# anindex/motion_planning_baselines

Measured on AMD Instinct MI355X. Metric: stomp_trajectory_update_iters_per_sec, higher is better.
Workload: dtype f32

## Files before the change

include/mpb.h:

```cpp
#ifndef MPB_H
#define MPB_H

#include <stddef.h>
#include <stdint.h>

#include "mpb_geom_layout.h"
#include "mpb_rrt_layout.h"
#include "mpb_self_layout.h"
#include "mpb_sdf_layout.h"

#ifdef __cplusplus
extern "C" {
#endif

#define MPB_OK 0
#define MPB_E_INVALID 1
#define MPB_E_UNSUPPORTED 2
#define MPB_E_HIP 3

#define MPB_MAX_H 256

#define MPB_ABI_VERSION 7
#define MPB_VERSION_TUNING_BUILD 0x40000000
int mpb_version(void);
const char *mpb_last_error(void);

int mpb_geom_check(const float *geom_host, int n_words);
int mpb_geom_flags(const float *geom_host, int n_words, int *flags);

int mpb_cost_collision_eval(const float *trajs, const float *geom, float *out, float *per_waypoint,
                            int B, int H, int d, int h_begin, float k_sigma, float weight, void *stream);
int mpb_cost_collision_grad(const float *trajs, const float *geom, int geom_flags, float *out, float *grad,
                            int B, int H, int d, int h_begin, float k_sigma, float weight, void *stream);

#define MPB_TERM_GP 1u
#define MPB_TERM_START 2u
#define MPB_TERM_GOAL 4u
#define MPB_TERM_SMOOTH 8u
#define MPB_TERM_JLIM 16u
#define MPB_TERM_VEL_FD 32u
#define MPB_TERM_ALL 63u
int mpb_cost_terms_eval(const float *trajs, float *out, double *jl_total, const float *start_state,
                        const float *goal_states, const float *q_min, const float *q_max,
                        int B, int H, int d, int n_dof, int trajs_per_goal, uint32_t flags, float dt,
                        float k_gp, float k_start, float k_goal, float k_smooth, float k_jlim, float jl_eps,
                        int accumulate, int broadcast_jlim, void *stream);
int mpb_cost_terms_grad(float *trajs, const float *grad_in, float *grad_out, const float *R,
                        const float *start_state, const float *goal_states, const float *q_min, const float *q_max,
                        int B, int H, int d, int n_dof, int trajs_per_goal, uint32_t flags, float dt,
                        float k_gp, float k_start, float k_goal, float k_smooth, float k_jlim, float jl_eps,
                        float jl_scale, float prior_bw, float lr, float grad_clip, int apply, void *stream);

int mpb_traj_resample(const float *paths, const int *lengths, float *out, int N, int Lmax, int H, int D, float dt,
                      void *stream);
int mpb_traj_interpolate(const float *trajs, float *out, int B, int H, int d, int n_interp, void *stream);
int mpb_gp_factor_error(const float *x, float *out, int B, int H, int D, float dt, void *stream);
int mpb_traj_finite_difference(const float *pos, float *out, int B, int H, int D, float dt, void *stream);

int mpb_fk_collision_points(const float *q, const float *geom, float *pts, int B, int H, int d, void *stream);
int mpb_fk_collision_points_vjp(const float *q, const float *geom, const float *grad_pts, float *grad_q,
                                int B, int H, int d, void *stream);
int mpb_field_cost_points(const float *pts, const float *geom, float *cost, int B, int H, void *stream);
int mpb_field_cost_points_vjp(const float *pts, const float *geom, const float *grad_cost, float *grad_pts,
                              int B, int H, void *stream);

int mpb_stomp_step(float *means, const float *eps, float *samples, float *costs, float *weights,
                   const float *L, const float *Sigma, const float *geom, int geom_flags,
                   int P, int S, int H, int d, int D,
                   float k_sigma, float weight, float lr, float temperature,
                   int n_iters, uint64_t seed, uint32_t iter0, uint32_t particle_offset, void *stream);
int mpb_stomp_step_profile(float *means, float *samples, float *costs, float *weights,
                           const float *L, const float *Sigma, const float *geom, int geom_flags,
                           int P, int S, int H, int d, int D,
                           float k_sigma, float weight, float lr, float temperature,
                           int n_iters, uint64_t seed, uint32_t iter0, uint32_t particle_offset, void *stream,
                           float *sample_kernel_ms, float *update_kernel_ms);
#define MPB_STOMP_WS_HEADER_BYTES 1280
#define MPB_STOMP_PATH_TWO_KERNEL 0
#define MPB_STOMP_PATH_PERSISTENT_EXCHANGE 1
#define MPB_STOMP_PATH_PERSISTENT 2
size_t mpb_stomp_workspace_bytes(int P, int S, int H, int d);
int mpb_stomp_workspace_init(float *workspace, size_t workspace_bytes, void *stream);
int mpb_stomp_run_path(int geom_flags, size_t workspace_bytes, int P, int S, int H, int d);
int mpb_stomp_run(float *means, const float *eps, float *samples, float *costs, float *weights,
                  const float *L, const float *Sigma, const float *geom, int geom_flags,
                  float *workspace, size_t workspace_bytes,
                  int P, int S, int H, int d, int D,
                  float k_sigma, float weight, float lr, float temperature,
                  int n_iters, uint64_t seed, uint32_t iter0, uint32_t particle_offset, void *stream);
int mpb_stomp_run_checked(float *means, const float *eps, float *samples, float *costs, float *weights,
                          const float *L, const float *Sigma, const float *geom, int geom_flags,
                          float *workspace, size_t workspace_bytes,
                          int P, int S, int H, int d, int D,
                          float k_sigma, float weight, float lr, float temperature,
                          int n_iters, uint64_t seed, uint32_t iter0, uint32_t particle_offset,
                          uint32_t *status, uint32_t *tag_out, float *means_copy, void *stream);
int mpb_stomp_run_status(const float *workspace, void *stream, int *timed_out);
int mpb_stomp_run_timed(float *means, const float *eps, float *samples, float *costs, float *weights,
                        const float *L, const float *Sigma, const float *geom, int geom_flags,
                        float *workspace, size_t workspace_bytes,
                        int P, int S, int H, int d, int D,
                        float k_sigma, float weight, float lr, float temperature,
                        int n_iters, uint64_t seed, uint32_t iter0, uint32_t particle_offset,
                        uint32_t *status, uint32_t *tag_out, float *means_copy, void *stream, float *kernel_ms);
typedef struct mpb_stomp_plan_s mpb_stomp_plan;
int mpb_stomp_plan_create(mpb_stomp_plan **plan, float *means, float *samples, float *costs, float *weights,
                          const float *L, const float *Sigma, const float *geom, int geom_flags,
                          float *workspace, size_t workspace_bytes, int P, int S, int H, int d, int D,
                          float k_sigma, float weight, float lr, float temperature, uint64_t seed, uint32_t particle_offset,
                          uint32_t *status);
int mpb_stomp_plan_launch(mpb_stomp_plan *plan, int n_iters, uint32_t iter0, float *means_copy, void *stream, uint32_t *tag_out);
int mpb_stomp_plan_destroy(mpb_stomp_plan *plan);

int mpb_stomp_sample(const float *means, const float *eps, float *samples, const float *L,
                     const float *geom, int geom_flags, float *costs,
                     int P, int S, int H, int d, float k_sigma, float weight,
                     uint64_t seed, uint32_t iter, uint32_t particle_offset, void *stream);
int mpb_stomp_update(float *means, const float *samples, const float *costs, float *weights,
                     const float *Sigma, int P, int S, int H, int d, float lr, float temperature,
                     void *stream);

int mpb_chomp_step(float *means, const float *R, const float *geom, int geom_flags, float *costs_out,
                   int B_local, int B_global, int H, int d, int D,
                   float k_sigma, float weight, float w_prior, float lr, float grad_clip,
                   int n_iters, void *stream);

size_t mpb_gpmp2_workspace_bytes(int B, int H, int D);
int mpb_gpmp2_linearize(const float *x, const float *geom, int geom_flags, void *workspace, int B, int H, int D,
                        int n_interp, void *stream);
int mpb_gpmp2_diag(void *workspace, double *diag_sum_out, int B, int H, int D, int n_fields, float dt,
                   float sigma_start, float sigma_gp, float sigma_goal, float sigma_coll, void *stream);
int mpb_gpmp2_solve(float *x, const float *start, const float *goal, const double *diag_mean, void *workspace,
                    float *costs_out, int B, int H, int D, int n_fields, float dt,
                    float sigma_start, float sigma_gp, float sigma_goal, float sigma_coll,
                    float delta, int trust_region, float step_size, void *stream);
int mpb_gpmp2_step(float *x, const float *start, const float *goal, const float *geom, int geom_flags, void *workspace,
                   float *costs_out, int B, int H, int D, float dt,
                   float sigma_start, float sigma_gp, float sigma_goal, float sigma_coll,
                   float delta, int trust_region, float step_size, int n_iters, int n_interp, int n_fields,
                   void *stream);

int mpb_mppi_step(float *mean, const float *eps, const float *scale_tril, const float *cov_inv,
                  const float *state0, const float *goal, const float *ctrl_min, const float *ctrl_max,
                  const float *discount, const float *c_weights, const float *geom, int geom_flags,
                  float *controls, float *states, float *costs, float *weights,
                  float *best_cost, float *best_states,
                  int NP, int S, int T, int c, int control_type, float dt,
                  float k_sigma, float weight, float temp, float step_size,
                  int n_iters, uint64_t seed, uint32_t iter0, void *stream);
#define MPB_MPPI_NOISE_GLOBAL 0
#define MPB_MPPI_NOISE_LDS 1
#define MPB_MPPI_NOISE_MATRIX 2
int mpb_mppi_plan(int geom_flags, int has_geom, int NP, int S, int T, int c, int has_eps, int n_cu, int *plan);
int mpb_point_dynamics(const float *x, const float *u, const float *ctrl_min, const float *ctrl_max, const float *dyn_std,
                       const float *noise, float *x_next, size_t n, int dim, float dt, void *stream);
int mpb_point_traj_cost(const float *X, const float *U, const float *goal, const float *discount, float w_pos, float w_vel,
                        float w_ctrl, float w_pos_T, float energy, float *costs, int T, int B, int state_dim, int ctrl_dim,
                        void *stream);


int mpb_stoch_gpmp_costs(const float *samples, const float *means, const float *start, const float *goal,
                         const float *geom, float *costs, int P, int S, int H, int D, float dt,
                         float sigma_start, float sigma_gp, float sigma_goal, float sigma_coll,
                         float sigma_start_sample, float sigma_gp_sample, float sigma_goal_sample,
                         float temperature, void *stream);

int mpb_stoch_gpmp_step(float *means, double *means64, float *samples, float *costs, float *weights,
                        const double *Udiag, const double *Uoff, const double *scale_tril,
                        const float *start, const float *goal, const float *geom,
                        int P, int S, int H, int D, float dt,
                        float sigma_start, float sigma_gp, float sigma_goal, float sigma_coll,
                        float sigma_start_sample, float sigma_gp_sample, float sigma_goal_sample,
                        float temperature, float step_size, int n_iters, uint64_t seed, void *stream);

int mpb_gp_prior_sample(float *out, const double *means, const double *eps, const double *Udiag,
                        const double *Uoff, int G, int n, int H, int D, uint64_t seed, void *stream);
int mpb_gp_prior_sample_dense(float *out, const double *means, const double *eps, const double *scale_tril,
                              int G, int n, int H, int D, uint64_t seed, void *stream);
int mpb_mvn_sample_dense(float *out, const double *means, const double *eps, const double *tril_t,
                         int G, int n, int M, uint64_t seed, void *stream);

int mpb_mt19937_normals(float *out, int n, int n_calls, const uint32_t *state_in, int pos, int final_idx, uint32_t *state_out,
                        const uint16_t *jump_idx, const int *jump_cnt, int jump_stride, const int *segs, int n_segs,
                        uint32_t *work, void *stream);

int mpb_collision_check(const float *q, const float *geom, int geom_flags, unsigned char *in_collision, float *gap,
                        int N, int D, void *stream);

int mpb_traj_collision_stats(const float *trajs, size_t row_stride, const float *geom, int geom_flags, int n_interp,
                             int *n_in_collision, int *first_in_collision, float *max_gap, unsigned char *point_in_collision,
                             int N, int H, int D, void *stream);

int mpb_self_check(const float *self_host, int n_words);
int mpb_self_invalidate(const float *self);
int mpb_self_collision_eval(const float *trajs, const float *self, float *out, float *per_waypoint,
                            int B, int H, int d, int h_begin, float k_sigma, float weight, int accumulate, void *stream);
int mpb_self_collision_grad(const float *trajs, const float *self, float *out, float *grad,
                            int B, int H, int d, int h_begin, float k_sigma, float weight, int accumulate, void *stream);
int mpb_self_collision_check(const float *q, const float *self, unsigned char *in_collision, float *gap,
                             int N, int D, int or_into, void *stream);

int mpb_sdf_grid_check(const float *sdf_host, int n_words);
int mpb_sdf_grid_invalidate(const float *sdf);
int mpb_sdf_grid_build(const float *geom, float *sdf, void *stream);
int mpb_sdf_grid_build_occupancy(const unsigned char *occupancy, float *sdf, void *stream);
int mpb_sdf_grid_sample(const float *points, const float *sdf, float *s, float *grad, int N, void *stream);
int mpb_sdf_grid_eval(const float *trajs, const float *sdf, float *out, float *per_waypoint,
                      int B, int H, int d, int h_begin, float k_sigma, float weight, int accumulate, void *stream);
int mpb_sdf_grid_grad(const float *trajs, const float *sdf, float *out, float *grad,
                      int B, int H, int d, int h_begin, float k_sigma, float weight, int accumulate, void *stream);
int mpb_sdf_grid_collision_check(const float *q, const float *sdf, unsigned char *in_collision, float *gap,
                                 int N, int D, int or_into, void *stream);

#define MPB_IK_MAX_ITERS 1024
#define MPB_IK_MIN_DAMPING 1e-2f
int mpb_fk_ee_pose(const float *q, const float *geom, float *pose, float *jac, int N, int D, void *stream);
int mpb_ik_solve(const float *target, const float *q_seed, const float *geom, const float *q_min, const float *q_max,
                 float *q_out, float *pos_err, float *rot_err, unsigned char *converged, int *iters_used,
                 int N, int S, int D, int n_iters, float damping, float pos_tol, float rot_tol, int position_only, void *stream);

int mpb_ee_cost_eval(const float *trajs, const float *geom, const float *target, float *out, float *per_waypoint,
                     int B, int H, int d, int D, int h_begin, int h_end, int group, int stride_g, int stride_h,
                     float k_pos, float k_rot, int use_axis, float ax, float ay, float az, float weight, int accumulate, void *stream);
int mpb_ee_cost_grad(const float *trajs, const float *geom, const float *target, float *out, float *grad,
                     int B, int H, int d, int D, int h_begin, int h_end, int group, int stride_g, int stride_h,
                     float k_pos, float k_rot, int use_axis, float ax, float ay, float az, float weight, int accumulate, void *stream);

size_t mpb_rrt_connect_workspace_bytes(int B, int max_nodes, int n_pre, int D);
int mpb_rrt_connect_init(void *workspace, size_t workspace_bytes, const float *start, const float *goal,
                         const float *geom, int geom_flags, int B, int max_nodes, int n_pre, int D, void *stream);
int mpb_rrt_connect_run(void *workspace, size_t workspace_bytes, const float *geom, int geom_flags,
                        const float *pre_samples, size_t pre_stride, const int *sample_idx, float *paths,
                        int *lengths, int *status, int B, int max_nodes, int n_pre, int D, int Lmax, int iter0,
                        int n_iters, int total_iters, float step_size, float n_radius, uint64_t seed,
                        uint32_t problem_offset, void *stream);

size_t mpb_rrt_star_workspace_bytes(int B, int max_nodes, int n_pre, int D);
int mpb_rrt_star_init(void *workspace, size_t workspace_bytes, const float *start, const float *goal,
                      const float *geom, int geom_flags, int B, int max_nodes, int n_pre, int D, void *stream);
int mpb_rrt_star_run(void *workspace, size_t workspace_bytes, const float *geom, int geom_flags,
                     const float *pre_samples, size_t pre_stride, const int *sample_idx, const int *goal_draw,
                     float *paths, int *lengths, float *costs, int *status, int B, int max_nodes, int n_pre, int D,
                     int Lmax, int iter0, int n_iters, int total_iters, int max_best_cost_iters,
                     int n_iters_after_success, int informed, float step_size, float n_radius, float goal_prob,
                     float cost_eps, float eps, uint64_t seed, uint32_t problem_offset, void *stream);

#ifdef __cplusplus
}
#endif
#endif
```

include/mpb_debug.h:

```cpp
#ifndef MPB_DEBUG_H
#define MPB_DEBUG_H

#include <stddef.h>
#include <stdint.h>

#ifdef __cplusplus
extern "C" {
#endif

const char *mpb_debug_last_error(void);
int mpb_debug_occupy(int n_blocks, uint64_t usec, uint32_t *sink, void *stream);
int mpb_debug_philox(const uint32_t *ctr, const uint32_t *key, uint32_t *out, int n, int rounds, void *stream);
int mpb_debug_stomp_normals(float *out, int P, int S, int d, int n_iters, uint64_t seed, uint32_t iter0,
                            uint32_t particle_offset, void *stream);
int mpb_debug_stomp_normals_h(float *out, int P, int S, int d, int H, int n_iters, uint64_t seed, uint32_t iter0,
                              uint32_t particle_offset, void *stream);
int mpb_debug_mppi_normals(float *out, int NP, int S, int T, int c, int n_iters, uint64_t seed, uint32_t iter0, void *stream);

int mpb_debug_mt19937_uniforms(float *out, int n, int n_calls, const uint32_t *state_in, int pos, int final_idx,
                               uint32_t *state_out, const uint16_t *jump_idx, const int *jump_cnt, int jump_stride,
                               const int *segs, int n_segs, uint32_t *work, void *stream);
int mpb_debug_mt19937_normals_timed(float *out, int n, int n_calls, const uint32_t *state_in, int pos, int final_idx,
                                    uint32_t *state_out, const uint16_t *jump_idx, const int *jump_cnt, int jump_stride,
                                    const int *segs, int n_segs, uint32_t *work, void *events, void *stream);

#ifdef __cplusplus
}
#endif
#endif
```

motion_planning_baselines_amd/_lib.py:

```python
import ctypes
import os

import numpy as np

_HERE = os.path.dirname(os.path.abspath(__file__))
LIB_PATH = os.environ.get('MPB_LIB_PATH') or os.path.join(_HERE, 'csrc', 'libmpb_hip.so')

_f = ctypes.c_float
_i = ctypes.c_int
_p = ctypes.c_void_p
_u64 = ctypes.c_uint64
_u32 = ctypes.c_uint32

SIGNATURES = {
    'mpb_version': [],
    'mpb_last_error': [],
    'mpb_geom_check': [_p, _i],
    'mpb_geom_flags': [_p, _i, _p],
    'mpb_cost_collision_eval': [_p, _p, _p, _p, _i, _i, _i, _i, _f, _f, _p],
    'mpb_cost_collision_grad': [_p, _p, _i, _p, _p, _i, _i, _i, _i, _f, _f, _p],
    'mpb_cost_terms_eval': [_p] * 7 + [_i] * 5 + [_u32] + [_f] * 7 + [_i, _i, _p],
    'mpb_cost_terms_grad': [_p] * 8 + [_i] * 5 + [_u32] + [_f] * 11 + [_i, _p],
    'mpb_traj_resample': [_p, _p, _p, _i, _i, _i, _i, _f, _p],
    'mpb_gp_factor_error': [_p, _p, _i, _i, _i, _f, _p],
    'mpb_traj_interpolate': [_p, _p, _i, _i, _i, _i, _p],
    'mpb_traj_finite_difference': [_p, _p, _i, _i, _i, _f, _p],
    'mpb_fk_collision_points': [_p, _p, _p, _i, _i, _i, _p],
    'mpb_fk_collision_points_vjp': [_p, _p, _p, _p, _i, _i, _i, _p],
    'mpb_field_cost_points': [_p, _p, _p, _i, _i, _p],
    'mpb_field_cost_points_vjp': [_p, _p, _p, _p, _i, _i, _p],
    'mpb_stomp_step': [_p, _p, _p, _p, _p, _p, _p, _p, _i, _i, _i, _i, _i, _i, _f, _f, _f, _f, _i, _u64, _u32, _u32, _p],
    'mpb_stomp_workspace_bytes': [_i, _i, _i, _i],
    'mpb_stomp_run': [_p, _p, _p, _p, _p, _p, _p, _p, _i, _p, ctypes.c_size_t, _i, _i, _i, _i, _i, _f, _f, _f, _f, _i, _u64, _u32, _u32, _p],
    'mpb_stomp_run_checked': [_p, _p, _p, _p, _p, _p, _p, _p, _i, _p, ctypes.c_size_t, _i, _i, _i, _i, _i, _f, _f, _f, _f, _i, _u64, _u32, _u32, _p, _p, _p, _p],
    'mpb_stomp_run_status': [_p, _p, _p],
    'mpb_stomp_run_timed': [_p, _p, _p, _p, _p, _p, _p, _p, _i, _p, ctypes.c_size_t, _i, _i, _i, _i, _i, _f, _f, _f, _f, _i, _u64, _u32, _u32, _p, _p, _p, _p, _p],
    'mpb_stomp_workspace_init': [_p, ctypes.c_size_t, _p],
    'mpb_stomp_run_path': [_i, ctypes.c_size_t, _i, _i, _i, _i],
    'mpb_stomp_step_profile': [_p, _p, _p, _p, _p, _p, _p, _i, _i, _i, _i, _i, _i, _f, _f, _f, _f, _i, _u64, _u32, _u32, _p, _p, _p],
    'mpb_stomp_sample': [_p, _p, _p, _p, _p, _i, _p, _i, _i, _i, _i, _f, _f, _u64, _u32, _u32, _p],
    'mpb_stomp_update': [_p, _p, _p, _p, _p, _i, _i, _i, _i, _f, _f, _p],
    'mpb_chomp_step': [_p, _p, _p, _i, _p, _i, _i, _i, _i, _i, _f, _f, _f, _f, _f, _i, _p],
    'mpb_gpmp2_workspace_bytes': [_i, _i, _i],
    'mpb_gpmp2_linearize': [_p, _p, _i, _p, _i, _i, _i, _i, _p],
    'mpb_gpmp2_diag': [_p, _p, _i, _i, _i, _i, _f, _f, _f, _f, _f, _p],
    'mpb_gpmp2_solve': [_p, _p, _p, _p, _p, _p, _i, _i, _i, _i, _f, _f, _f, _f, _f, _f, _i, _f, _p],
    'mpb_gpmp2_step': [_p, _p, _p, _p, _i, _p, _p, _i, _i, _i, _f, _f, _f, _f, _f, _f, _i, _f, _i, _i, _i, _p],
    'mpb_stoch_gpmp_costs': [_p, _p, _p, _p, _p, _p, _i, _i, _i, _i] + [_f] * 9 + [_p],
    'mpb_stoch_gpmp_step': [_p] * 11 + [_i] * 4 + [_f] * 10 + [_i, _u64, _p],
    'mpb_gp_prior_sample': [_p, _p, _p, _p, _p, _i, _i, _i, _i, _u64, _p],
    'mpb_gp_prior_sample_dense': [_p, _p, _p, _p, _i, _i, _i, _i, _u64, _p],
    'mpb_mvn_sample_dense': [_p, _p, _p, _p, _i, _i, _i, _u64, _p],
    'mpb_stomp_plan_create': [_p] * 8 + [_i, _p, ctypes.c_size_t, _i, _i, _i, _i, _i, _f, _f, _f, _f, _u64, _u32, _p],
    'mpb_stomp_plan_launch': [_p, _i, _u32, _p, _p, _p],
    'mpb_stomp_plan_destroy': [_p],
    'mpb_point_dynamics': [_p, _p, _p, _p, _p, _p, _p, ctypes.c_size_t, _i, _f, _p],
    'mpb_point_traj_cost': [_p, _p, _p, _p, _f, _f, _f, _f, _f, _p, _i, _i, _i, _i, _p],
    'mpb_mppi_step': [_p] * 11 + [_i] + [_p] * 6 + [_i, _i, _i, _i, _i, _f, _f, _f, _f, _f, _i, _u64, _u32, _p],
    'mpb_mppi_plan': [_i, _i, _i, _i, _i, _i, _i, _i, _p],
    'mpb_mt19937_normals': [_p, _i, _i, _p, _i, _i, _p, _p, _p, _i, _p, _i, _p, _p],
    'mpb_collision_check': [_p, _p, _i, _p, _p, _i, _i, _p],
    'mpb_traj_collision_stats': [_p, ctypes.c_size_t, _p, _i, _i, _p, _p, _p, _p, _i, _i, _i, _p],
    'mpb_self_check': [_p, _i],
    'mpb_self_invalidate': [_p],
    'mpb_self_collision_eval': [_p, _p, _p, _p, _i, _i, _i, _i, _f, _f, _i, _p],
    'mpb_self_collision_grad': [_p, _p, _p, _p, _i, _i, _i, _i, _f, _f, _i, _p],
    'mpb_self_collision_check': [_p, _p, _p, _p, _i, _i, _i, _p],
    'mpb_sdf_grid_check': [_p, _i],
    'mpb_sdf_grid_invalidate': [_p],
    'mpb_sdf_grid_build': [_p, _p, _p],
    'mpb_sdf_grid_build_occupancy': [_p, _p, _p],
    'mpb_sdf_grid_sample': [_p, _p, _p, _p, _i, _p],
    'mpb_sdf_grid_eval': [_p, _p, _p, _p, _i, _i, _i, _i, _f, _f, _i, _p],
    'mpb_sdf_grid_grad': [_p, _p, _p, _p, _i, _i, _i, _i, _f, _f, _i, _p],
    'mpb_sdf_grid_collision_check': [_p, _p, _p, _p, _i, _i, _i, _p],
    'mpb_fk_ee_pose': [_p, _p, _p, _p, _i, _i, _p],
    'mpb_ik_solve': [_p] * 10 + [_i] * 4 + [_f] * 3 + [_i, _p],
    'mpb_ee_cost_eval': [_p] * 5 + [_i] * 9 + [_f, _f, _i] + [_f] * 4 + [_i, _p],
    'mpb_ee_cost_grad': [_p] * 5 + [_i] * 9 + [_f, _f, _i] + [_f] * 4 + [_i, _p],
    'mpb_rrt_connect_workspace_bytes': [_i, _i, _i, _i],
    'mpb_rrt_connect_init': [_p, ctypes.c_size_t, _p, _p, _p, _i, _i, _i, _i, _i, _p],
    'mpb_rrt_connect_run': [_p, ctypes.c_size_t, _p, _i, _p, ctypes.c_size_t, _p, _p, _p, _p] + [_i] * 8 + [_f, _f, _u64, _u32, _p],
    'mpb_rrt_star_workspace_bytes': [_i, _i, _i, _i],
    'mpb_rrt_star_init': [_p, ctypes.c_size_t, _p, _p, _p, _i, _i, _i, _i, _i, _p],
    'mpb_rrt_star_run': [_p, ctypes.c_size_t, _p, _i, _p, ctypes.c_size_t] + [_p] * 6 + [_i] * 11 + [_f] * 5 + [_u64, _u32, _p],
}

DEBUG_SIGNATURES = {
    'mpb_debug_last_error': [],
    'mpb_debug_occupy': [_i, _u64, _p, _p],
    'mpb_debug_philox': [_p, _p, _p, _i, _i, _p],
    'mpb_debug_stomp_normals': [_p, _i, _i, _i, _i, _u64, _u32, _u32, _p],
    'mpb_debug_stomp_normals_h': [_p, _i, _i, _i, _i, _i, _u64, _u32, _u32, _p],
    'mpb_debug_mppi_normals': [_p, _i, _i, _i, _i, _i, _u64, _u32, _p],
    'mpb_debug_mt19937_uniforms': [_p, _i, _i, _p, _i, _i, _p, _p, _p, _i, _p, _i, _p, _p],
    'mpb_debug_mt19937_normals_timed': [_p, _i, _i, _p, _i, _i, _p, _p, _p, _i, _p, _i, _p, _p, _p],
}
ABI_VERSION = 7

_lib = None
_debug_lib = None


class MPBError(RuntimeError):
    pass


def lib():
    global _lib
    if _lib is not None:
        return _lib
    if not os.path.exists(LIB_PATH):
        raise MPBError(
            f'{LIB_PATH} not found: the HIP extension is not built. Run '
            f'`python -c "import __graft_entry__ as g; g.build()"` (or motion_planning_baselines_amd/build.py). '
            f'There is no CPU fallback.')
    import torch
    h = ctypes.CDLL(LIB_PATH)
    for name, argtypes in SIGNATURES.items():
        try:
            fn = getattr(h, name)
        except AttributeError as e:
            raise MPBError(f'{LIB_PATH} does not export {name} (declared in include/mpb.h)') from e
        fn.argtypes = argtypes
        fn.restype = (ctypes.c_char_p if name == 'mpb_last_error' else
                      ctypes.c_size_t if name in ('mpb_gpmp2_workspace_bytes', 'mpb_stomp_workspace_bytes', 'mpb_rrt_connect_workspace_bytes',
                                                         'mpb_rrt_star_workspace_bytes') else ctypes.c_int)
    if (h.mpb_version() & 0xFFFF) != ABI_VERSION:
        raise MPBError(f'{LIB_PATH} reports ABI version {h.mpb_version() & 0xFFFF}, this binding is written for {ABI_VERSION} '
                       f'(include/mpb.h MPB_ABI_VERSION); rebuild with motion_planning_baselines_amd.build.build(force=True)')
    if (h.mpb_version() & 0x40000000) and not os.environ.get('MPB_LIB_PATH'):
        raise MPBError(f'{LIB_PATH} is a tuning build (compiled with wrong-result timing switches); rebuild with '
                       f'motion_planning_baselines_amd.build.build(force=True)')
    _lib = h
    return h


def debug_lib():
    global _debug_lib
    if _debug_lib is not None:
        return _debug_lib
    path = os.path.join(_HERE, 'csrc', 'libmpb_hip_debug.so')
    if not os.path.exists(path):
        raise MPBError(f'{path} not found: run motion_planning_baselines_amd.build.build()')
    lib()
    h = ctypes.CDLL(path)
    for name, argtypes in DEBUG_SIGNATURES.items():
        fn = getattr(h, name)
        fn.argtypes = argtypes
        fn.restype = ctypes.c_char_p if name == 'mpb_debug_last_error' else ctypes.c_int
    _debug_lib = h
    return h


def debug_check(code, what=''):
    if code != 0:
        msg = debug_lib().mpb_debug_last_error()
        raise MPBError(f'{what} failed with code {code}: {msg.decode() if msg else "?"}')


def check(code, what=''):
    if code != 0:
        msg = lib().mpb_last_error()
        raise MPBError(f'{what} failed with code {code}: {msg.decode() if msg else "?"}')


def geom_check(buf):
    buf = np.ascontiguousarray(buf, dtype=np.float32)
    check(lib().mpb_geom_check(buf.ctypes.data_as(ctypes.c_void_p), int(buf.size)), 'mpb_geom_check')


def self_check(buf):
    buf = np.ascontiguousarray(buf, dtype=np.float32)
    check(lib().mpb_self_check(buf.ctypes.data_as(ctypes.c_void_p), int(buf.size)), 'mpb_self_check')


def sdf_grid_check(buf, n_words=None):
    buf = np.ascontiguousarray(buf, dtype=np.float32)
    check(lib().mpb_sdf_grid_check(buf.ctypes.data_as(ctypes.c_void_p), int(buf.size if n_words is None else n_words)), 'mpb_sdf_grid_check')


def geom_flags(buf):
    buf = np.ascontiguousarray(buf, dtype=np.float32)
    out = ctypes.c_int(0)
    check(lib().mpb_geom_flags(buf.ctypes.data_as(ctypes.c_void_p), int(buf.size), ctypes.cast(ctypes.pointer(out), ctypes.c_void_p)),
          'mpb_geom_flags')
    return int(out.value)
```

motion_planning_baselines_amd/build.py:

```python
import os
import subprocess
import sys
import tempfile

HERE = os.path.dirname(os.path.abspath(__file__))
CSRC = os.path.join(HERE, 'csrc')
SOURCES = ['mpb_lib.hip', 'mpb_stomp_api.hip', 'mpb_kernels.hip', 'mpb_stomp_fused.hip', 'mpb_stomp_fused_hx.hip', 'mpb_chomp.hip', 'mpb_gpmp2.hip', 'mpb_gpmp2_lr.hip', 'mpb_mppi.hip', 'mpb_prior.hip', 'mpb_stoch_gpmp.hip', 'mpb_costs.hip', 'mpb_points.hip', 'mpb_mt19937.hip', 'mpb_rrt_connect.hip', 'mpb_rrt_star.hip', 'mpb_traj_validate.hip', 'mpb_self_collision.hip', 'mpb_sdf_grid.hip', 'mpb_ik.hip', 'mpb_ee_cost.hip']
DEBUG_SOURCES = ['mpb_debug.hip']
MAX_ILP = ['-mllvm', '-amdgpu-sched-strategy=max-ilp']
EXTRA = {'mpb_chomp.hip': MAX_ILP, 'mpb_gpmp2.hip': MAX_ILP, 'mpb_gpmp2_lr.hip': MAX_ILP, 'mpb_mppi.hip': MAX_ILP,
         'mpb_kernels.hip': ['-mllvm', '-amdgpu-sched-strategy=iterative-ilp'],
         'mpb_stomp_fused.hip': ['-mllvm', '-amdgpu-sched-strategy=iterative-ilp'],
         'mpb_stomp_fused_hx.hip': ['-mllvm', '-amdgpu-sched-strategy=iterative-ilp']}
OUT = os.path.join(CSRC, 'libmpb_hip.so')
DEBUG_OUT = os.path.join(CSRC, 'libmpb_hip_debug.so')
FLAGS = ['--offload-arch=gfx950', '-O3', '-std=c++17', '-fPIC', '-Wall', '-Wno-unused-function',
         '-ffinite-math-only', '-fno-signed-zeros', '-fno-slp-vectorize']
RESOURCES = os.path.join(CSRC, 'kernel_resources.json')
REMARKS = ['-Rpass-analysis=kernel-resource-usage']


def parse_resource_remarks(text):
    import re
    out, cur = {}, None
    keys = {'VGPRs': 'vgprs', 'AGPRs': 'agprs', 'ScratchSize [bytes/lane]': 'scratch', 'Occupancy [waves/SIMD]': 'occupancy',
            'SGPRs Spill': 'sgpr_spill', 'VGPRs Spill': 'vgpr_spill', 'LDS Size [bytes/block]': 'lds', 'TotalSGPRs': 'sgprs'}
    for line in text.splitlines():
        m = re.search(r'remark: Function Name: (\S+)', line)
        if m:
            cur = out.setdefault(m.group(1), {})
            continue
        m = re.search(r'remark:\s+([A-Za-z \[\]/]+): (\d+) \[-Rpass-analysis', line)
        if m and cur is not None and m.group(1).strip() in keys:
            cur[keys[m.group(1).strip()]] = int(m.group(2))
    return out


_LAYOUT = '../../include/mpb_geom_layout.h'
PMC_SOURCES = {
    'stomp': ['mpb_stomp_fused.hip', 'mpb_stomp_fused.h', 'mpb_stomp_noise.h', 'mpb_geom.h', _LAYOUT, 'mpb_common.h', 'mpb_model_panda.h'],
    'stomp_c5': ['mpb_stomp_fused.hip', 'mpb_stomp_fused.h', 'mpb_stomp_noise.h', 'mpb_geom.h', _LAYOUT, 'mpb_common.h', 'mpb_model_panda.h'],
    'stomp_h128': ['mpb_stomp_fused_hx.hip', 'mpb_stomp_fused.h', 'mpb_stomp_noise.h', 'mpb_geom.h', _LAYOUT, 'mpb_common.h', 'mpb_model_panda.h'],
    'kernelA': ['mpb_kernels.hip', 'mpb_stomp_noise.h', 'mpb_geom.h', _LAYOUT, 'mpb_common.h', 'mpb_model_panda.h'],
    'solve': ['mpb_gpmp2.hip', 'mpb_gpmp2_lr.hip', 'mpb_gpmp2.h', 'mpb_geom.h', _LAYOUT, 'mpb_common.h'],
    'chomp': ['mpb_chomp.hip', 'mpb_geom.h', _LAYOUT, 'mpb_common.h', 'mpb_model_panda.h'],
    'mppi': ['mpb_mppi.hip', 'mpb_geom.h', _LAYOUT, 'mpb_common.h'],
}


def sources_sha1(files):
    import hashlib
    h = hashlib.sha1()
    for f in files:
        h.update(f.encode())
        with open(os.path.join(CSRC, f), 'rb') as fh:
            h.update(fh.read())
    return h.hexdigest()


def pmc_fingerprint(kind):
    files = PMC_SOURCES[kind]
    return {'sources': files, 'sources_sha1': sources_sha1(files), 'flags': FLAGS + EXTRA.get(files[0], [])}


def _stale():
    if not os.path.exists(OUT) or not os.path.exists(DEBUG_OUT) or not os.path.exists(RESOURCES):
        return True
    t = min(os.path.getmtime(OUT), os.path.getmtime(DEBUG_OUT))
    deps = [os.path.join(CSRC, f) for f in os.listdir(CSRC) if f.endswith(('.hip', '.h'))]
    deps += [os.path.join(os.path.dirname(HERE), 'include', h) for h in ('mpb.h', 'mpb_geom_layout.h', 'mpb_rrt_layout.h', 'mpb_self_layout.h', 'mpb_sdf_layout.h', 'mpb_debug.h')]
    return any(os.path.getmtime(d) > t for d in deps)


def build_variant(out, extra_flags, verbose=False):
    if os.path.abspath(out) == os.path.abspath(OUT):
        raise ValueError('build_variant must not overwrite the product library')
    extra_flags = list(extra_flags)
    if any('_T_' in f for f in extra_flags) and '-DMPB_TUNING_BUILD' not in extra_flags:
        extra_flags.append('-DMPB_TUNING_BUILD')
    hipcc = os.environ.get('HIPCC', '/opt/rocm/bin/hipcc')
    objs = []
    tmp = out + '.objs'
    os.makedirs(tmp, exist_ok=True)
    for src in SOURCES:
        obj = os.path.join(tmp, src.replace('.hip', '.o'))
        cmd = [hipcc, *FLAGS, *EXTRA.get(src, []), *extra_flags, '-c', os.path.join(CSRC, src), '-o', obj]
        if verbose:
            print(' '.join(cmd), flush=True)
        subprocess.check_call(cmd)
        objs.append(obj)
    subprocess.check_call([hipcc, '--offload-arch=gfx950', '-shared', '-fPIC', *objs, '-o', out])
    return out


def build(force=False, verbose=True):
    from . import model_gen
    stale = force or _stale() or bool(model_gen.stale_headers())
    if not stale:
        return OUT
    for path in model_gen.write_headers():
        if verbose:
            print('regenerated', path, flush=True)
    if any('MPB_TUNING_BUILD' in f or '_T_' in f for f in FLAGS + [x for v in EXTRA.values() for x in v]):
        raise RuntimeError('the product build must not carry tuning switches')
    hipcc = os.environ.get('HIPCC', '/opt/rocm/bin/hipcc')
    objs = []
    procs = []
    for src in SOURCES + DEBUG_SOURCES:
        obj = os.path.join(CSRC, src.replace('.hip', '.o'))
        objs.append(obj)
        cmd = [hipcc, *FLAGS, *EXTRA.get(src, []), *REMARKS, '-c', os.path.join(CSRC, src), '-o', obj]
        if verbose:
            print(' '.join(cmd), flush=True)
        log = tempfile.TemporaryFile(mode='w+')
        procs.append((cmd, subprocess.Popen(cmd, stderr=log, text=True), log))
    resources = {}
    for cmd, p, log in procs:
        p.wait()
        log.seek(0)
        err = log.read()
        log.close()
        rest = '\n'.join(l for l in err.splitlines() if 'kernel-resource-usage' not in l and not l.lstrip().startswith(('|', '^')) and l.strip()
                         and not __import__('re').match(r'^\s*\d+ \|', l))
        if p.returncode != 0:
            raise RuntimeError('hipcc failed: ' + ' '.join(cmd) + '\n' + err[-4000:])
        if verbose and rest:
            print(rest, file=sys.stderr, flush=True)
        resources.update(parse_resource_remarks(err))
    import json
    with open(RESOURCES, 'w') as fh:
        json.dump(resources, fh, indent=0, sort_keys=True)
    n = len(SOURCES)
    for out, o in ((OUT, objs[:n]), (DEBUG_OUT, objs[n:])):
        cmd = [hipcc, '--offload-arch=gfx950', '-shared', '-fPIC', *o, '-o', out]
        if verbose:
            print(' '.join(cmd), flush=True)
        subprocess.check_call(cmd)
    return OUT


if __name__ == '__main__':
    build(force='--force' in sys.argv)
```

motion_planning_baselines_amd/csrc/mpb_debug.hip:

```cpp
#include <hip/hip_runtime.h>

#include "mpb_common.h"
#include "mpb_host.h"
#include "mpb_stomp_noise.h"
#include "mpb_mt19937.h"
#include "../../include/mpb_debug.h"

static thread_local char g_debug_err[512] = "";
char* mpb_err_buf() { return g_debug_err; }
extern "C" const char* mpb_debug_last_error(void) { return g_debug_err; }

__global__ void debug_philox_kernel(const uint32_t* __restrict__ ctr, const uint32_t* __restrict__ key, uint32_t* __restrict__ out,
                                    int n, int rounds) {
    const int i = blockIdx.x * blockDim.x + threadIdx.x;
    if (i >= n) return;
    const uint4 c = make_uint4(ctr[4 * i], ctr[4 * i + 1], ctr[4 * i + 2], ctr[4 * i + 3]);
    const uint2 k = make_uint2(key[2 * i], key[2 * i + 1]);
    const uint4 r = (rounds == 7) ? philox4x32<7>(c, k) : philox4x32<10>(c, k);
    out[4 * i] = r.x; out[4 * i + 1] = r.y; out[4 * i + 2] = r.z; out[4 * i + 3] = r.w;
}

extern "C" int mpb_debug_philox(const uint32_t* ctr, const uint32_t* key, uint32_t* out, int n, int rounds, void* stream) {
    if (!ctr || !key || !out || n < 1) return mpb_fail(MPB_E_INVALID, "mpb_debug_philox: bad argument");
    if (rounds != 7 && rounds != 10) return mpb_fail(MPB_E_INVALID, "mpb_debug_philox: rounds must be 7 or 10");
    hipLaunchKernelGGL(debug_philox_kernel, dim3((n + 255) / 256), dim3(256), 0, (hipStream_t)stream, ctr, key, out, n, rounds);
    return mpb_check_launch("mpb_debug_philox");
}

#ifdef MPB_DEBUG_RAW_NORMALS
#define DBGQ(x) (x)
#else
#define DBGQ(x) stomp_eps_quantise(x)
#endif
__global__ void debug_stomp_normals_kernel(float* __restrict__ out, int P, int S, int d, int HC, int n_iters, uint32_t seed_lo,
                                           uint32_t seed_hi, uint32_t iter0, uint32_t particle_offset) {
    const size_t n = (size_t)n_iters * P * S * d * HC * 4;
    const size_t i = (size_t)blockIdx.x * blockDim.x + threadIdx.x;
    if (i >= n) return;
    const uint32_t g = i & 3;
    size_t r = i >> 2;
    const uint32_t kc = r % HC; r /= HC;
    const uint32_t j = r % d; r /= d;
    const uint32_t s = r % S; r /= S;
    const uint32_t p = r % P; r /= P;
    const uint32_t it = (uint32_t)r;
    float lo[8], hi[8];
    uint32_t carry[2];
    stomp_normals_lo<STOMP_PRIO_NONE>(particle_offset + p, s, j, g, kc << 4, iter0 + it, seed_lo, seed_hi, lo, carry);
    stomp_normals_hi<STOMP_PRIO_NONE>(particle_offset + p, s, j, g, kc << 4, iter0 + it, seed_lo, seed_hi, carry, hi);
    float* o = out + (((((size_t)it * P + p) * S + s) * d + j) * HC + kc) * 64;
#pragma unroll
    for (int u = 0; u < 8; ++u) {
        o[stomp_eps_column((int)g, u >> 2, u & 3)] = DBGQ(lo[u]);
        o[stomp_eps_column((int)g, 2 + (u >> 2), u & 3)] = DBGQ(hi[u]);
    }
}

extern "C" int mpb_debug_stomp_normals_h(float* out, int P, int S, int d, int H, int n_iters, uint64_t seed, uint32_t iter0,
                                         uint32_t particle_offset, void* stream) {
    if (!out || P < 1 || S < 1 || d < 1 || d > 16 || n_iters < 1 || H < 1 || H > 256)
        return mpb_fail(MPB_E_INVALID, "mpb_debug_stomp_normals: bad argument");
    const int HC = (H + 63) / 64;
    const size_t n = (size_t)n_iters * P * S * d * HC * 4;
    if (n > 0x7FFFFFFFull * 256ull) return mpb_fail(MPB_E_INVALID, "mpb_debug_stomp_normals: too many draws for one launch");
    hipLaunchKernelGGL(debug_stomp_normals_kernel, dim3((unsigned)((n + 255) / 256)), dim3(256), 0, (hipStream_t)stream, out, P, S,
                       d, HC, n_iters, (uint32_t)seed, (uint32_t)(seed >> 32), iter0, particle_offset);
    return mpb_check_launch("mpb_debug_stomp_normals");
}
extern "C" int mpb_debug_stomp_normals(float* out, int P, int S, int d, int n_iters, uint64_t seed, uint32_t iter0,
                                       uint32_t particle_offset, void* stream) {
    return mpb_debug_stomp_normals_h(out, P, S, d, 64, n_iters, seed, iter0, particle_offset, stream);
}

__global__ void debug_mppi_normals_kernel(float* __restrict__ out, int NP, int S, int T, int c, int n_iters, uint32_t seed_lo,
                                          uint32_t seed_hi, uint32_t iter0) {
    const int G4 = (T + 3) >> 2;
    const size_t n = (size_t)n_iters * NP * c * S * G4;
    const size_t idx = (size_t)blockIdx.x * blockDim.x + threadIdx.x;
    if (idx >= n) return;
    size_t r = idx;
    const uint32_t g4 = r % G4; r /= G4;
    const uint32_t s = r % S; r /= S;
    const uint32_t i = r % c; r /= c;
    const uint32_t prob = r % NP; r /= NP;
    const uint32_t it = (uint32_t)r;
    const uint4 w = philox4x32<7>(make_uint4(prob, s, g4 | (i << 16), iter0 + it), make_uint2(seed_lo, seed_hi));
    float nrm[4];
    box_muller_m23(w.x, w.y, nrm[0], nrm[1]);
    box_muller_m23(w.z, w.w, nrm[2], nrm[3]);
    float* o = out + ((((size_t)it * NP + prob) * c + i) * S + s) * T;
#pragma unroll
    for (int q = 0; q < 4; ++q)
        if ((int)(4 * g4 + q) < T) o[4 * g4 + q] = nrm[q];
}

extern "C" int mpb_debug_mppi_normals(float* out, int NP, int S, int T, int c, int n_iters, uint64_t seed, uint32_t iter0, void* stream) {
    if (!out || NP < 1 || S < 1 || T < 1 || c < 1 || n_iters < 1) return mpb_fail(MPB_E_INVALID, "mpb_debug_mppi_normals: bad argument");
    const size_t n = (size_t)n_iters * NP * c * S * ((T + 3) >> 2);
    if (n > 0x7FFFFFFFull * 256ull) return mpb_fail(MPB_E_INVALID, "mpb_debug_mppi_normals: too many draws for one launch");
    hipLaunchKernelGGL(debug_mppi_normals_kernel, dim3((unsigned)((n + 255) / 256)), dim3(256), 0, (hipStream_t)stream, out, NP, S, T, c,
                       n_iters, (uint32_t)seed, (uint32_t)(seed >> 32), iter0);
    return mpb_check_launch("mpb_debug_mppi_normals");
}

__global__ __launch_bounds__(64) void occupy_kernel(unsigned long long ticks, unsigned* sink) {
    __shared__ unsigned pad[150 * 256];
    pad[threadIdx.x] = threadIdx.x;
    const unsigned long long t0 = __builtin_amdgcn_s_memrealtime();
    while (__builtin_amdgcn_s_memrealtime() - t0 < ticks) __builtin_amdgcn_s_sleep(32);
    if (pad[(threadIdx.x + 1) & 63] == 0xFFFFFFFFu) sink[0] = 1u;
}

extern "C" int mpb_debug_occupy(int n_blocks, uint64_t usec, uint32_t* sink, void* stream) {
    if (n_blocks < 1 || !sink) return mpb_fail(MPB_E_INVALID, "mpb_debug_occupy: bad argument");
    hipLaunchKernelGGL(occupy_kernel, dim3(n_blocks), dim3(64), 0, (hipStream_t)stream, usec * 100ull, sink);
    return mpb_check_launch("mpb_debug_occupy");
}

extern "C" int mpb_debug_mt19937_uniforms(float* out, int n, int n_calls, const uint32_t* state_in, int pos, int final_idx,
                                          uint32_t* state_out, const uint16_t* jump_idx, const int* jump_cnt, int jump_stride,
                                          const int* segs, int n_segs, uint32_t* work, void* stream) {
    if (!out || !state_in || !state_out || !jump_idx || !jump_cnt || !segs || !work)
        return mpb_fail(MPB_E_INVALID, "mpb_debug_mt19937_uniforms: null pointer");
    if (const char* why = mt19937_bad_args(n, n_calls, pos, final_idx, jump_stride, n_segs)) return mpb_fail(MPB_E_INVALID, why);
    if (((uintptr_t)jump_idx & 15u) || ((uintptr_t)work & 15u)) return mpb_fail(MPB_E_INVALID, "mpb_debug_mt19937_uniforms: misaligned");
    if (mt19937_launch<true>(out, n, state_in, pos, final_idx, state_out, jump_idx, jump_cnt, jump_stride, segs, n_segs, work, nullptr,
                             (hipStream_t)stream) != hipSuccess)
        return mpb_fail(MPB_E_HIP, "mpb_debug_mt19937_uniforms: HIP launch failed");
    return MPB_OK;
}

extern "C" int mpb_debug_mt19937_normals_timed(float* out, int n, int n_calls, const uint32_t* state_in, int pos, int final_idx,
                                               uint32_t* state_out, const uint16_t* jump_idx, const int* jump_cnt, int jump_stride,
                                               const int* segs, int n_segs, uint32_t* work, void* events, void* stream) {
    if (!out || !state_in || !state_out || !jump_idx || !jump_cnt || !segs || !work || !events)
        return mpb_fail(MPB_E_INVALID, "mpb_debug_mt19937_normals_timed: null pointer");
    if (const char* why = mt19937_bad_args(n, n_calls, pos, final_idx, jump_stride, n_segs)) return mpb_fail(MPB_E_INVALID, why);
    if (((uintptr_t)jump_idx & 15u) || ((uintptr_t)work & 15u)) return mpb_fail(MPB_E_INVALID, "mpb_debug_mt19937_normals_timed: misaligned");
    if (mt19937_launch<false>(out, n, state_in, pos, final_idx, state_out, jump_idx, jump_cnt, jump_stride, segs, n_segs, work,
                              (hipEvent_t*)events, (hipStream_t)stream) != hipSuccess)
        return mpb_fail(MPB_E_HIP, "mpb_debug_mt19937_normals_timed: HIP launch failed");
    return MPB_OK;
}
```

motion_planning_baselines_amd/csrc/mpb_stomp_api.hip:

```cpp
#include <hip/hip_runtime.h>
#include <stdlib.h>

#include <atomic>
#include <chrono>

#include "mpb_stomp_host.h"
#include "mpb_stomp_fused.h"

struct StompCheck {
    const char* who;
    int n_iters;
    bool two_kernel;
    bool profile;
    const char* aligned;
    const void *extra0 = nullptr, *extra1 = nullptr;
};

static int stomp_check(const StompCall& c, const StompCheck& k) {
    if (!c.means || !c.samples || !c.costs || !c.weights || !c.L || !c.Sigma || !c.geom) return mpb_failf(MPB_E_INVALID, "%s: null pointer", k.who);
    bool bad = c.P < (k.profile ? 1 : 0) || c.S < 1 || !(c.d == c.D || c.d == 2 * c.D) || k.n_iters < (k.profile ? 1 : 0) || (k.profile && k.n_iters > 1024);
    if (k.two_kernel) bad = bad || c.H < 3 || c.H > MPB_MAX_H || c.D < 1 || c.D > MPB_MAX_DOF;
    if (bad) return mpb_failf(MPB_E_INVALID, "%s: bad shape", k.who);
    if (!(c.temperature > 0.f)) return mpb_failf(MPB_E_INVALID, "%s: temperature must be > 0", k.who);
    if (k.aligned && (mpb_misaligned16(c.means, c.eps, c.samples, c.L, c.Sigma, c.geom) || mpb_misaligned16(k.extra0, k.extra1)))
        return mpb_failf(MPB_E_INVALID, "%s: %s must be 16-byte aligned", k.who, k.aligned);
    return k.two_kernel ? mpb_update_envelope(c.S, c.H, c.d, k.who) : MPB_OK;
}

extern "C" int mpb_stomp_sample(const float* means, const float* eps, float* samples, const float* L,
                                const float* geom, int geom_flags, float* costs, int P, int S, int H, int d, float k_sigma,
                                float weight, uint64_t seed, uint32_t iter, uint32_t particle_offset, void* stream) {
    if (P == 0) return MPB_OK;
    if (!means || !samples || !L) return mpb_failf(MPB_E_INVALID, "%s: null pointer", __func__);
    if ((geom == nullptr) != (costs == nullptr)) return mpb_failf(MPB_E_INVALID, "%s: geom and costs must be given together", __func__);
    if (P < 0 || S < 1 || H < 3 || H > MPB_MAX_H || d < 1 || d > MPB_MAX_D) return mpb_failf(MPB_E_INVALID, "%s: bad shape", __func__);
    if (mpb_misaligned16(means, eps, samples, L, geom)) return mpb_failf(MPB_E_INVALID, "%s: means / eps / samples / L / geom must be 16-byte aligned", __func__);
    StompCall c = {};
    c.means = const_cast<float*>(means); c.eps = eps; c.samples = samples; c.costs = costs; c.L = L; c.geom = geom;
    c.P = P; c.S = S; c.H = H; c.d = d; c.seed = seed; c.particle_offset = particle_offset;
    if (geom) { c.geom_flags = geom_flags; c.k_sigma = k_sigma; c.weight = weight; }
    mpb_stomp_launch_sample(c, eps, iter, (hipStream_t)stream, nullptr);
    return mpb_check_launch(__func__);
}

extern "C" int mpb_stomp_update(float* means, const float* samples, const float* costs, float* weights,
                                const float* Sigma, int P, int S, int H, int d, float lr, float temperature,
                                void* stream) {
    if (P == 0) return MPB_OK;
    if (!means || !samples || !costs || !weights) return mpb_failf(MPB_E_INVALID, "%s: null pointer", __func__);
    if (P < 0) return mpb_failf(MPB_E_INVALID, "%s: bad shape", __func__);
    if (const int rc = mpb_update_envelope(S, H, d, __func__)) return rc;
    if (!(temperature > 0.f)) return mpb_failf(MPB_E_INVALID, "%s: temperature must be > 0", __func__);
    if (mpb_misaligned16(means, samples, Sigma)) return mpb_failf(MPB_E_INVALID, "%s: means / samples / Sigma must be 16-byte aligned", __func__);
    StompCall c = {};
    c.means = means; c.samples = const_cast<float*>(samples); c.costs = const_cast<float*>(costs); c.weights = weights; c.Sigma = Sigma;
    c.P = P; c.S = S; c.H = H; c.d = d; c.lr = lr; c.temperature = temperature;
    mpb_stomp_launch_update(c, (hipStream_t)stream, nullptr);
    return mpb_check_launch(__func__);
}

static int stomp_step(const StompCall& c, const StompLaunch& l) {
    if (c.P == 0) return MPB_OK;
    if (const int rc = stomp_check(c, {"mpb_stomp_step", l.n_iters, true, false, "means / eps / samples / L / Sigma / geom"})) return rc;
    const size_t eps_stride = (size_t)c.S * c.d * c.P * c.H;
    constexpr int MPB_CHUNK = 128;
    hipEvent_t ev[2] = {nullptr, nullptr};
    hipStreamCaptureStatus cap = hipStreamCaptureStatusNone;
    const bool throttle = l.n_iters > 2 * MPB_CHUNK &&
                          hipStreamIsCapturing(l.stream, &cap) == hipSuccess && cap == hipStreamCaptureStatusNone;
    for (int it = 0; it < l.n_iters; ++it) {
        if (throttle && it % MPB_CHUNK == 0) {
            const int k = (it / MPB_CHUNK) & 1;
            if (ev[k]) (void)hipEventSynchronize(ev[k]);
            else (void)hipEventCreateWithFlags(&ev[k], hipEventDisableTiming);
        }
        mpb_stomp_launch_sample(c, c.eps ? c.eps + (size_t)it * eps_stride : nullptr, l.iter0 + (uint32_t)it, l.stream, nullptr);
        mpb_stomp_launch_update(c, l.stream, nullptr);
        if (throttle && it % MPB_CHUNK == MPB_CHUNK - 1) (void)hipEventRecord(ev[(it / MPB_CHUNK) & 1], l.stream);
    }
    for (int k = 0; k < 2; ++k)
        if (ev[k]) (void)hipEventDestroy(ev[k]);
    return mpb_check_launch("mpb_stomp_step");
}

extern "C" int mpb_stomp_step(float* means, const float* eps, float* samples, float* costs, float* weights,
                              const float* L, const float* Sigma, const float* geom, int geom_flags, int P, int S, int H, int d, int D,
                              float k_sigma, float weight, float lr, float temperature, int n_iters, uint64_t seed,
                              uint32_t iter0, uint32_t particle_offset, void* stream) {
    const StompCall c = {means, eps, samples, costs, weights, L, Sigma, geom, geom_flags, P, S, H, d, D,
                         k_sigma, weight, lr, temperature, seed, particle_offset};
    return stomp_step(c, {n_iters, iter0, nullptr, (hipStream_t)stream, nullptr});
}

extern "C" int mpb_stomp_step_profile(float* means, float* samples, float* costs, float* weights, const float* L,
                                      const float* Sigma, const float* geom, int geom_flags, int P, int S, int H, int d, int D,
                                      float k_sigma, float weight, float lr, float temperature, int n_iters, uint64_t seed,
                                      uint32_t iter0, uint32_t particle_offset, void* stream, float* sample_kernel_ms,
                                      float* update_kernel_ms) {
    const StompCall c = {means, nullptr, samples, costs, weights, L, Sigma, geom, geom_flags, P, S, H, d, D,
                         k_sigma, weight, lr, temperature, seed, particle_offset};
    if (!sample_kernel_ms || !update_kernel_ms) return mpb_failf(MPB_E_INVALID, "%s: null pointer", __func__);
    if (const int rc = stomp_check(c, {__func__, n_iters, true, true, nullptr})) return rc;
    hipStream_t st = (hipStream_t)stream;
    StompEvents* ev = new StompEvents[2 * (size_t)n_iters]();
    int rc = MPB_OK;
    for (int i = 0; i < 2 * n_iters && rc == MPB_OK; ++i)
        if (hipEventCreate(&ev[i].start) != hipSuccess || hipEventCreate(&ev[i].stop) != hipSuccess)
            rc = mpb_failf(MPB_E_HIP, "%s: hipEventCreate failed", __func__);
    if (rc == MPB_OK) {
        for (int it = 0; it < n_iters; ++it) {
            mpb_stomp_launch_sample(c, nullptr, iter0 + (uint32_t)it, st, &ev[2 * it]);
            mpb_stomp_launch_update(c, st, &ev[2 * it + 1]);
        }
        rc = mpb_check_launch(__func__);
    }
    if (rc == MPB_OK && hipStreamSynchronize(st) != hipSuccess) rc = mpb_failf(MPB_E_HIP, "%s: synchronize failed", __func__);
    double sa = 0.0, sb = 0.0;
    for (int it = 0; it < n_iters && rc == MPB_OK; ++it) {
        float ma = 0.f, mb = 0.f;
        if (hipEventElapsedTime(&ma, ev[2 * it].start, ev[2 * it].stop) != hipSuccess ||
            hipEventElapsedTime(&mb, ev[2 * it + 1].start, ev[2 * it + 1].stop) != hipSuccess)
            rc = mpb_failf(MPB_E_HIP, "%s: hipEventElapsedTime failed", __func__);
        sa += ma;
        sb += mb;
    }
    for (int i = 0; i < 2 * n_iters; ++i) {
        if (ev[i].start) (void)hipEventDestroy(ev[i].start);
        if (ev[i].stop) (void)hipEventDestroy(ev[i].stop);
    }
    delete[] ev;
    if (rc != MPB_OK) return rc;
    *sample_kernel_ms = (float)(sa / n_iters);
    *update_kernel_ms = (float)(sb / n_iters);
    return MPB_OK;
}

struct FusedPlan {
    int path;
    int nc;
    bool hx;
    int nb;
    size_t ws_bytes;
};
static FusedPlan fused_plan(int geom_flags, int P, int S, int H, int d) {
    FusedPlan f = {MPB_STOMP_PATH_TWO_KERNEL, 1, false, 1, 0};
    if (P < 1 || S < 1) return f;
    const int n_cu = mpb_device_cu_count();
    const char* hx_env = getenv("MPB_STOMP_HX");
    const int force_hx = hx_env ? atoi(hx_env) : 0;
    const bool v1 = !force_hx && H == 64 && S <= FUSED_WAVES * FUSED_MAX_CHUNKS && mpb_flags_all_grids(geom_flags) &&
                    (d == 2 || d == 3 || d == 4 || d == 6 || d == 7 || d == 14);
    if (!v1) {
        if (!mpb_fused_hx_plan(geom_flags, n_cu, P, S, H, d, &f.nc, &f.nb, &f.ws_bytes)) return f;
        f.hx = true;
        f.path = f.nc > 1 ? MPB_STOMP_PATH_PERSISTENT_EXCHANGE : MPB_STOMP_PATH_PERSISTENT;
        return f;
    }
    f.nc = (S + FUSED_WAVES - 1) / FUSED_WAVES;
    static const int force_nb = [] { const char* e = getenv("MPB_STOMP_BATCHES"); return e ? atoi(e) : 0; }();
    const long r1 = (2L * P + n_cu - 1) / n_cu, r2 = ((long)P + n_cu - 1) / n_cu;
    const bool two_batches = f.nc == 2 && force_nb != 1 && (force_nb == 2 || 188 * r2 < 100 * r1);
    f.nb = two_batches ? 2 : 1;
    const bool exchange = f.nc > 1 && !two_batches;
    f.path = exchange ? MPB_STOMP_PATH_PERSISTENT_EXCHANGE : MPB_STOMP_PATH_PERSISTENT;
    f.ws_bytes = (exchange ? mpb_fused_ws_floats(P, f.nc) : FUSED_HDR_WORDS) * sizeof(float);
    return f;
}

extern "C" size_t mpb_stomp_workspace_bytes(int P, int S, int H, int d) {
    if (P < 1 || S < 1) return 0;
    const FusedPlan f = fused_plan(MPB_GEOM_FLAG_ALL_GRIDS, P, S, H, d);
    const FusedPlan fl = fused_plan(MPB_GEOM_FLAG_ALL_LISTS, P, S, H, d);
    size_t b = f.path == MPB_STOMP_PATH_TWO_KERNEL ? FUSED_HDR_WORDS * sizeof(float) : f.ws_bytes;
    if (fl.path != MPB_STOMP_PATH_TWO_KERNEL && fl.ws_bytes > b) b = fl.ws_bytes;
    return b;
}

extern "C" int mpb_stomp_workspace_init(float* workspace, size_t workspace_bytes, void* stream) {
    if (!workspace || workspace_bytes < FUSED_HDR_WORDS * sizeof(float)) return mpb_fail(MPB_E_INVALID, "mpb_stomp_workspace_init: workspace too small");
    if (hipMemsetAsync(workspace, 0, FUSED_HDR_WORDS * sizeof(float), (hipStream_t)stream) != hipSuccess) return mpb_fail(MPB_E_HIP, "mpb_stomp_workspace_init: memset failed");
    return MPB_OK;
}

extern "C" int mpb_stomp_run_path(int geom_flags, size_t workspace_bytes, int P, int S, int H, int d) {
    const FusedPlan f = fused_plan(geom_flags, P, S, H, d);
    return (f.path != MPB_STOMP_PATH_TWO_KERNEL && workspace_bytes >= f.ws_bytes) ? f.path : MPB_STOMP_PATH_TWO_KERNEL;
}

static int stomp_run(const StompCall& c, float* workspace, size_t workspace_bytes, uint32_t* status, const StompLaunch& l, uint32_t* tag_out) {
    if (tag_out) *tag_out = 0u;
    if (c.P == 0) return MPB_OK;
    const FusedPlan f = fused_plan(c.geom_flags, c.P, c.S, c.H, c.d);
    if (l.n_iters == 0 || !workspace || f.path == MPB_STOMP_PATH_TWO_KERNEL || workspace_bytes < f.ws_bytes) {
        const int rc = l.n_iters == 0 ? MPB_OK : stomp_step(c, l);
        if (rc == MPB_OK && l.means_copy && c.means &&
            hipMemcpyAsync(l.means_copy, c.means, sizeof(float) * (size_t)c.P * c.H * c.d, hipMemcpyDeviceToDevice, l.stream) != hipSuccess)
            return mpb_fail(MPB_E_HIP, "mpb_stomp_run: copy of the means failed");
        return rc;
    }
    if (const int rc = stomp_check(c, {"mpb_stomp_run", l.n_iters, false, false, "means / eps / samples / L / Sigma / geom / workspace / means_copy",
                                       workspace, l.means_copy}))
        return rc;
    StompFusedGrid g = {workspace, f.nc, f.nb, 0u, 0ull, nullptr};
    if (status) {
        static thread_local uint32_t* seen_host = nullptr;
        static thread_local unsigned* seen_dev = nullptr;
        if (status != seen_host) {
            unsigned* dp = nullptr;
            if (hipHostGetDevicePointer(reinterpret_cast<void**>(&dp), status, 0) != hipSuccess) {
                (void)hipGetLastError();
                return mpb_fail(MPB_E_INVALID, "mpb_stomp_run: status is not pinned, device-mapped host memory");
            }
            seen_host = status;
            seen_dev = dp;
        }
        g.status_dev = seen_dev;
    }
    static std::atomic<uint32_t> epoch{(uint32_t)std::chrono::steady_clock::now().time_since_epoch().count()};
    g.tag0 = (epoch.fetch_add(1u) + 1u) * 0x9E3779B9u;
    if (g.tag0 == 0u) g.tag0 = 0x9E3779B9u;
    if (tag_out) *tag_out = g.tag0;
    g.timeout = FUSED_TIMEOUT_TICKS + FUSED_TIMEOUT_PER_ITER * (unsigned long long)l.n_iters;
    if (const char* e = getenv("MPB_STOMP_TIMEOUT_US")) { const long long us = atoll(e); if (us > 0) g.timeout = 100ull * (unsigned long long)us; }
    return f.hx ? mpb_fused_hx_launch(c, l, g) : mpb_fused_launch(c, l, g);
}

extern "C" int mpb_stomp_run_checked(float* means, const float* eps, float* samples, float* costs, float* weights,
                                     const float* L, const float* Sigma, const float* geom, int geom_flags, float* workspace,
                                     size_t workspace_bytes, int P, int S, int H, int d, int D, float k_sigma, float weight, float lr,
                                     float temperature, int n_iters, uint64_t seed, uint32_t iter0, uint32_t particle_offset,
                                     uint32_t* status, uint32_t* tag_out, float* means_copy, void* stream) {
    const StompCall c = {means, eps, samples, costs, weights, L, Sigma, geom, geom_flags, P, S, H, d, D,
                         k_sigma, weight, lr, temperature, seed, particle_offset};
    return stomp_run(c, workspace, workspace_bytes, status, {n_iters, iter0, means_copy, (hipStream_t)stream, nullptr}, tag_out);
}

extern "C" int mpb_stomp_run(float* means, const float* eps, float* samples, float* costs, float* weights,
                             const float* L, const float* Sigma, const float* geom, int geom_flags, float* workspace,
                             size_t workspace_bytes, int P, int S, int H, int d, int D, float k_sigma, float weight, float lr,
                             float temperature, int n_iters, uint64_t seed, uint32_t iter0, uint32_t particle_offset,
                             void* stream) {
    const StompCall c = {means, eps, samples, costs, weights, L, Sigma, geom, geom_flags, P, S, H, d, D,
                         k_sigma, weight, lr, temperature, seed, particle_offset};
    return stomp_run(c, workspace, workspace_bytes, nullptr, {n_iters, iter0, nullptr, (hipStream_t)stream, nullptr}, nullptr);
}

struct mpb_stomp_plan_s {
    StompCall call;
    float* workspace;
    size_t workspace_bytes;
    uint32_t* status;
};

extern "C" int mpb_stomp_plan_create(mpb_stomp_plan** plan, float* means, float* samples, float* costs, float* weights, const float* L,
                                     const float* Sigma, const float* geom, int geom_flags, float* workspace, size_t workspace_bytes,
                                     int P, int S, int H, int d, int D, float k_sigma, float weight, float lr, float temperature,
                                     uint64_t seed, uint32_t particle_offset, uint32_t* status) {
    if (!plan) return mpb_failf(MPB_E_INVALID, "%s: null pointer", __func__);
    *plan = nullptr;
    const StompCall c = {means, nullptr, samples, costs, weights, L, Sigma, geom, geom_flags, P, S, H, d, D,
                         k_sigma, weight, lr, temperature, seed, particle_offset};
    if (const int rc = stomp_check(c, {__func__, 0, false, false, "means / samples / L / Sigma / geom / workspace", workspace})) return rc;
    mpb_stomp_plan_s* q = static_cast<mpb_stomp_plan_s*>(malloc(sizeof(mpb_stomp_plan_s)));
    if (!q) return mpb_failf(MPB_E_HIP, "%s: out of host memory", __func__);
    *q = mpb_stomp_plan_s{c, workspace, workspace_bytes, status};
    *plan = q;
    return MPB_OK;
}

extern "C" int mpb_stomp_plan_launch(mpb_stomp_plan* plan, int n_iters, uint32_t iter0, float* means_copy, void* stream, uint32_t* tag_out) {
    if (!plan) return mpb_fail(MPB_E_INVALID, "mpb_stomp_plan_launch: null plan");
    return stomp_run(plan->call, plan->workspace, plan->workspace_bytes, plan->status, {n_iters, iter0, means_copy, (hipStream_t)stream, nullptr}, tag_out);
}

extern "C" int mpb_stomp_plan_destroy(mpb_stomp_plan* plan) {
    free(plan);
    return MPB_OK;
}

extern "C" int mpb_stomp_run_timed(float* means, const float* eps, float* samples, float* costs, float* weights,
                                   const float* L, const float* Sigma, const float* geom, int geom_flags, float* workspace,
                                   size_t workspace_bytes, int P, int S, int H, int d, int D, float k_sigma, float weight, float lr,
                                   float temperature, int n_iters, uint64_t seed, uint32_t iter0, uint32_t particle_offset,
                                   uint32_t* status, uint32_t* tag_out, float* means_copy, void* stream, float* kernel_ms) {
    if (!kernel_ms) return mpb_failf(MPB_E_INVALID, "%s: null pointer", __func__);
    *kernel_ms = 0.f;
    StompEvents ev = {nullptr, nullptr};
    if (hipEventCreate(&ev.start) != hipSuccess || hipEventCreate(&ev.stop) != hipSuccess) {
        if (ev.start) (void)hipEventDestroy(ev.start);
        return mpb_failf(MPB_E_HIP, "%s: hipEventCreate failed", __func__);
    }
    const StompCall c = {means, eps, samples, costs, weights, L, Sigma, geom, geom_flags, P, S, H, d, D,
                         k_sigma, weight, lr, temperature, seed, particle_offset};
    uint32_t tag = 0;
    int rc = stomp_run(c, workspace, workspace_bytes, status, {n_iters, iter0, means_copy, (hipStream_t)stream, &ev}, &tag);
    if (tag_out) *tag_out = tag;
    if (rc == MPB_OK && hipStreamSynchronize((hipStream_t)stream) != hipSuccess) rc = mpb_failf(MPB_E_HIP, "%s: synchronize failed", __func__);
    if (rc == MPB_OK && tag != 0u && hipEventElapsedTime(kernel_ms, ev.start, ev.stop) != hipSuccess) {
        (void)hipGetLastError();
        rc = mpb_failf(MPB_E_HIP, "%s: hipEventElapsedTime failed", __func__);
    }
    (void)hipEventDestroy(ev.start);
    (void)hipEventDestroy(ev.stop);
    return rc;
}

extern "C" int mpb_stomp_run_status(const float* workspace, void* stream, int* timed_out) {
    if (!workspace || !timed_out) return mpb_failf(MPB_E_INVALID, "%s: null pointer", __func__);
    uint32_t w[4] = {0u};
    if (hipMemcpyAsync(w, workspace, sizeof(w), hipMemcpyDeviceToHost, (hipStream_t)stream) != hipSuccess ||
        hipStreamSynchronize((hipStream_t)stream) != hipSuccess)
        return mpb_failf(MPB_E_HIP, "%s: copy failed", __func__);
    *timed_out = (w[FUSED_HDR_ERR] == w[FUSED_HDR_TAG] && w[FUSED_HDR_TAG] != 0u) ? (w[FUSED_HDR_WHY] == 2u ? 2 : 1) : 0;
    return MPB_OK;
}
```

motion_planning_baselines_amd/csrc/mpb_stomp_fused.hip:

```cpp
#include <hip/hip_runtime.h>

#include <type_traits>

#include "mpb_common.h"
#include "mpb_stomp_host.h"
#include "mpb_geom.h"
#include "mpb_stomp_noise.h"
#include "mpb_stomp_fused.h"

static inline size_t fused_ws_floats(int P, int nc) { return FUSED_HDR_WORDS + 2 * 2 * (size_t)P * nc * FUSED_XCHG; }

#ifdef MPB_STAMPS
__device__ unsigned long long g_fstamps[256 * FUSED_WAVES * 12];
#define FSTAMP(k)                                                                                   \
    do {                                                                                            \
        if (it == 2 && blockIdx.x < 256) {                                                          \
            __builtin_amdgcn_sched_barrier(0);                                                      \
            unsigned long long t_;                                                                  \
            asm volatile("s_memtime %0\n\ts_waitcnt lgkmcnt(0)" : "=s"(t_)::"memory");           \
            __builtin_amdgcn_sched_barrier(0);                                                      \
            if ((k) == 0) {           \
                unsigned hw_;                                                                       \
                asm volatile("s_getreg_b32 %0, hwreg(HW_REG_HW_ID, 4, 2)" : "=s"(hw_));             \
                t_ = (t_ & 0x00FFFFFFFFFFFFFFull) | ((unsigned long long)hw_ << 56);                \
            }                                                                                       \
            if ((threadIdx.x & 63) == 0) g_fstamps[(blockIdx.x * FUSED_WAVES + (threadIdx.x >> 6)) * 12 + (k)] = t_; \
        }                                                                                           \
    } while (0)
extern "C" int mpb_debug_read_fstamps(unsigned long long* dst, int n) {
    return hipMemcpyFromSymbol(dst, HIP_SYMBOL(g_fstamps), sizeof(unsigned long long) * n) == hipSuccess ? 0 : 3;
}
__device__ unsigned long long g_lstamps[1024 * 8];
#define LSTAMP(k)                                                                                   \
    do {                                                                                            \
        if (blockIdx.x < 1024 && threadIdx.x == 0) g_lstamps[blockIdx.x * 8 + (k)] = __builtin_amdgcn_s_memrealtime(); \
    } while (0)
extern "C" int mpb_debug_read_lstamps(unsigned long long* dst, int n) {
    return hipMemcpyFromSymbol(dst, HIP_SYMBOL(g_lstamps), sizeof(unsigned long long) * n) == hipSuccess ? 0 : 3;
}
#else
#define FSTAMP(k)
#define LSTAMP(k)
#endif

#ifdef FUSED_T_PRE_STATS
__device__ unsigned g_pre_miss[FUSED_WAVES];
extern "C" int mpb_debug_read_pre_miss(unsigned* dst) {
    if (hipMemcpyFromSymbol(dst, HIP_SYMBOL(g_pre_miss), sizeof(unsigned) * FUSED_WAVES) != hipSuccess) return 3;
    unsigned z[FUSED_WAVES] = {};
    return hipMemcpyToSymbol(HIP_SYMBOL(g_pre_miss), z, sizeof(z)) == hipSuccess ? 0 : 3;
}
#endif
template <int DCH, bool PRE>
struct FusedSmem {
    float4 otab[MPB_GRID_MAX_SPH + 1];
    unsigned gridw[MPB_GRID_MAX_CELLS];
    unsigned Limg[STOMP_LIMG_WORDS];
    float sig_l[64 * FUSED_LD];
    float mean_l[64 * DCH];
    float delta[DCH * FUSED_LD];
    float cst[FUSED_WAVES];
    int s_abort;
    unsigned s_ticket;
    unsigned pad_[2];
    float tiles[FUSED_WAVES * 64 * NT_STRIDE];
    __attribute__((aligned(16))) granule_t pre[PRE ? FUSED_WAVES * 128 : 2];
    __attribute__((aligned(16))) granule_t premz[PRE ? FUSED_WAVES * 4 : 2];
};

template <int DCH, int MODEL, int NB, bool INJ, bool CHAIN>
__global__ __launch_bounds__(FUSED_THREADS, 4) void stomp_fused_kernel(
    float* __restrict__ means, const float* __restrict__ eps, float* __restrict__ samples, float* __restrict__ costs,
    float* __restrict__ weights, const float* __restrict__ Lmat, const float* __restrict__ Sigma,
    const float* __restrict__ geom, float* __restrict__ ws, int P, int S, int nc, float k_sigma, float weight, float lr,
    float temperature, int n_iters, uint32_t seed_lo, uint32_t seed_hi, uint32_t iter0, uint32_t particle_offset,
    uint32_t tag0, unsigned long long timeout_ticks, unsigned* __restrict__ status_host, float* __restrict__ means_copy) {
    constexpr int H = 64;
    constexpr int N = H * DCH;
    static_assert(N <= FUSED_THREADS && N + 2 <= FUSED_XCHG, "one thread per trajectory element");
    if (!INJ) eps = nullptr;
#ifdef FUSED_NO_PRE
    constexpr bool PRE = false;
#else
    constexpr bool PRE = NB == 1 && 2 * DCH > 16 && MODEL != 0 && !INJ;
#endif
    __shared__ __attribute__((aligned(16))) FusedSmem<DCH, PRE> sm;
    float4 (&otab)[MPB_GRID_MAX_SPH + 1] = sm.otab;
    unsigned (&gridw)[MPB_GRID_MAX_CELLS] = sm.gridw;
    unsigned (&Limg)[STOMP_LIMG_WORDS] = sm.Limg;
    float (&sig_l)[64 * FUSED_LD] = sm.sig_l;
    float (&mean_l)[64 * DCH] = sm.mean_l;
    float (&delta)[DCH * FUSED_LD] = sm.delta;
    float (&cst)[FUSED_WAVES] = sm.cst;
    float (&tiles)[FUSED_WAVES * 64 * NT_STRIDE] = sm.tiles;
    int& s_abort = sm.s_abort;
    unsigned& s_ticket = sm.s_ticket;

    const int tid = threadIdx.x, lane = tid & 63, wave = __builtin_amdgcn_readfirstlane(tid >> 6);
    LSTAMP(0);
    unsigned* wsu = reinterpret_cast<unsigned*>(ws);
    const bool exchange = NB == 1 && nc > 1;
    if (tid == 0) {
        s_abort = 0;
        fused_stamp_begin(wsu, status_host);
        unsigned u = blockIdx.x;
        if (exchange) {
            int why;
            u = fused_draw_unit(wsu, P, nc, tag0, why);
            s_abort = why;
        }
        s_ticket = u;
    }
    LSTAMP(1);
    const int j = lane & 15, g = lane >> 4;
    granule_t* xch = reinterpret_cast<granule_t*>(ws + FUSED_HDR_WORDS);

    GeomView G0 = geom_view(geom);
    if (!CHAIN && G0.next != 0) G0.model = 0;
    {
        const int g_rounds = (G0.n_cells + 4 * FUSED_THREADS - 1) / (4 * FUSED_THREADS);
        const uint4* g4 = reinterpret_cast<const uint4*>(G0.grid);
        const int n_pad16 = (G0.n_cells + MPB_GRID_PAD - 1) / MPB_GRID_PAD * (MPB_GRID_PAD / 4);
        for (int u = 0; u < (MPB_GRID_MAX_CELLS / 4 + FUSED_THREADS - 1) / FUSED_THREADS; ++u) {
            const int i = tid + FUSED_THREADS * u;
            if (u < g_rounds && i < n_pad16) {
                const uint4 gw = g4[i];
                const unsigned ns = (unsigned)G0.n_sph;
                reinterpret_cast<uint4*>(gridw)[i] = make_uint4(grid_offset_word(gw.x, ns), grid_offset_word(gw.y, ns),
                                                                grid_offset_word(gw.z, ns), grid_offset_word(gw.w, ns));
            }
        }
        for (int i = tid; i <= G0.n_sph && i <= MPB_GRID_MAX_SPH; i += FUSED_THREADS)
            otab[i] = (i < G0.n_sph) ? reinterpret_cast<const float4*>(G0.sph)[i] : make_float4(-1.0e9f, -1.0e9f, -1.0e9f, 0.f);
        const f32x4 lv = reinterpret_cast<const f32x4*>(Lmat)[tid];
        const f32x4 sv = reinterpret_cast<const f32x4*>(Sigma)[tid];
        const int row = tid >> 4, col0 = (tid & 15) << 2;
        const bool edge_row = row == 0 || row == H - 1;
        stomp_l_image_store(Limg, row, col0, edge_row ? f32x4{0.f, 0.f, 0.f, 0.f} : lv);
        *reinterpret_cast<f32x4*>(sig_l + row * FUSED_LD + col0) = sv;
    }
    __syncthreads();
    const int ticket = __builtin_amdgcn_readfirstlane((int)s_ticket);
    const int p = exchange ? ticket / nc : ticket;
    const int chunk = exchange ? ticket - p * nc : 0;
    int s = chunk * FUSED_WAVES + wave;
    bool live = s < S;
    float mean_reg = 0.f;
    if (NB == 1) mean_reg = (tid < N) ? means[(size_t)p * N + tid] : 0.f;
    else if (tid < N) mean_l[tid] = means[(size_t)p * N + tid];
    if (ticket == 0 && tid == 0) st_agent_u(wsu + FUSED_HDR_TAG, tag0);
    LSTAMP(2);

    const size_t eps_stride = (size_t)S * DCH * P * H;
    const float inv_temperature = 1.0f / temperature;

#ifdef FUSED_NO_PAIR
    constexpr bool PAIRED = false;
#else
    constexpr bool PAIRED = 2 * DCH <= 16;
#endif
    constexpr int PAIR_STRIDE = FUSED_WAVES / 2;
    float* nt = tiles + wave * (H * NT_STRIDE);
    if constexpr (PAIRED) {
        if (wave < PAIR_STRIDE) {
            f32x4 acc[4];
            stomp_noise_bf16_pair<DCH>(Limg, acc, eps, P, S, p, j, g, particle_offset + (uint32_t)p, (uint32_t)s, (uint32_t)(s + PAIR_STRIDE),
                                       iter0, seed_lo, seed_hi);
            stomp_noise_to_tile_pair<DCH>(nt, nt + PAIR_STRIDE * (H * NT_STRIDE), acc, lane);
        }
    } else {
        f32x4 acc[4];
        stomp_noise_bf16<DCH>(Limg, acc, eps ? eps + (size_t)(live ? s : 0) * DCH * P * H : nullptr, P, p, j, g,
                              particle_offset + (uint32_t)p, (uint32_t)s, iter0, seed_lo, seed_hi);
        stomp_noise_to_tile(nt, acc, lane);
    }
    if (NB == 1 && tid < N) mean_l[tid] = mean_reg;
    __syncthreads();

    LSTAMP(3);
    const int n_run = s_abort ? 0 : n_iters;
#ifdef FUSED_T_PRE_STATS
    int pre_miss_ = 0;
#endif
    float w_out = 0.f;
    for (int it = 0; it < n_run; ++it) {
        const bool last_it = it + 1 == n_run;
        float pm0 = -3.0e38f, pz0 = 0.f, pe0 = 0.f, pm1 = -3.0e38f, pz1 = 0.f, pe1 = 0.f;
        f32x4 sd0 = {0.f, 0.f, 0.f, 0.f}, sd1 = {0.f, 0.f, 0.f, 0.f};
        float mb = 0.f, zb = 0.f, ex = 0.f, dpart = 0.f;
        int tq = 0, hh = 0, cc = 0, sl = 0;
        auto sigma_times_delta = [&](int li, int lg) {
            const float* arow = sig_l + (16 * wave + li) * FUSED_LD + 16 * lg;
            const float* brow = delta + (li < DCH ? li : 0) * FUSED_LD + 16 * lg;
            f32x4 acc = {0.f, 0.f, 0.f, 0.f};
#pragma unroll
            for (int q = 0; q < 4; ++q) {
                const f32x4 av = *reinterpret_cast<const f32x4*>(arow + 4 * q);
                f32x4 bv = *reinterpret_cast<const f32x4*>(brow + 4 * q);
                if (li >= DCH) bv = f32x4{0.f, 0.f, 0.f, 0.f};
#pragma unroll
                for (int e = 0; e < 4; ++e) acc = __builtin_amdgcn_mfma_f32_16x16x4f32(av[e], bv[e], acc, 0, 0, 0);
            }
            return acc;
        };
#pragma nounroll
        for (int bt = 0; bt < NB; ++bt) {
        if (NB > 1) { s = bt * FUSED_WAVES + wave; live = s < S; }
        FSTAMP(0);
        float nz[16];
        stomp_noise_row<DCH>(nt, lane, nz);
        const int h = lane;
        float x[DCH];
        if (DCH % 2 == 0) {
#pragma unroll
            for (int c = 0; c < DCH; c += 2) {
#ifdef FUSED_T_A_NOMEAN
                const float2 mv = make_float2(0.f, 0.f);
#else
                const float2 mv = *reinterpret_cast<const float2*>(mean_l + h * DCH + c);
#endif
                x[c] = mv.x + nz[c];
                x[c + 1] = mv.y + nz[c + 1];
            }
#pragma unroll
            for (int c = 0; c < DCH; c += 2) *reinterpret_cast<float2*>(nt + h * DCH + c) = make_float2(x[c], x[c + 1]);
        } else {
#pragma unroll
            for (int c = 0; c < DCH; ++c) x[c] = mean_l[h * DCH + c] + nz[c];
#pragma unroll
            for (int c = 0; c < DCH; ++c) nt[h * DCH + c] = x[c];
        }
        __builtin_amdgcn_wave_barrier();
        if (NB > 1 && last_it && live) {
            const f32x4* pk4 = reinterpret_cast<const f32x4*>(nt);
            f32x4* out4 = reinterpret_cast<f32x4*>(samples + ((size_t)p * S + s) * N);
#pragma unroll
            for (int k = 0; k < (16 * DCH + 63) / 64; ++k) {
                const unsigned idx = (unsigned)lane + 64u * k;
                if (idx < 16u * DCH) out4[idx] = pk4[idx];
            }
        }
        FSTAMP(1);
        {
            float q[MPB_MAX_DOF];
            constexpr int DQ_ = (DCH > MPB_MAX_DOF) ? DCH / 2 : DCH;
#pragma unroll
            for (int i = 0; i < MPB_MAX_DOF; ++i) q[i] = (i < DQ_) ? x[i < DQ_ ? i : 0] : 0.f;
            float c = 0.f;
            bool bad = false;
            GeomView G = G0;
            for (const float* gp = geom;;) {
                if (gp != geom) {
                    __syncthreads();
                    grid_stage_offsets(G, gridw, otab, tid, FUSED_THREADS);
                    __syncthreads();
                }
#ifdef FUSED_T_SKIP_COST
                if (false) {
#else
                if (live && h >= 1) {
#endif
                    if (MODEL == PandaModel::ID) {
                        if (G.model == PandaModel::ID) c = fmaf(G.fscale, waypoint_cost_grid_model<PandaModel, true, false, !CHAIN>(G, gridw, otab, q), c);
                    } else {
                        c = fmaf(G.fscale, waypoint_cost_grid<true>(G, gridw, otab, q), c);
                    }
                }
                if (MODEL != 0 && G.model != MODEL) bad = true;
                if (!CHAIN) break;
                if (G.next == 0) break;
                gp += G.next;
                G = geom_view(gp);
            }
            if (CHAIN && G0.next != 0) {
                __syncthreads();
                int tid_o = tid;
                asm volatile("" : "+v"(tid_o));
                grid_stage_offsets(G0, gridw, otab, tid_o, FUSED_THREADS);
            }
            const double csum = wave_sum_f64((double)c);
            const float cw = weight * (k_sigma * (float)csum);
            if (lane == 0) {
                cst[wave] = cw;
                if (NB > 1 && last_it && live) {
                    if (bad) reinterpret_cast<unsigned*>(costs)[(size_t)p * S + s] = 0x7FC00000u;
                    else costs[(size_t)p * S + s] = cw;
                }
            }
        }
        FSTAMP(2);
        __syncthreads();
        FSTAMP(3);
        tq = tid;
        asm volatile("" : "+v"(tq));
        const int lq = tq & 63;
        hh = (tq < N) ? tq / DCH : 0; cc = (tq < N) ? tq - hh * DCH : 0;
        sl = (NB > 1 ? bt : chunk) * FUSED_WAVES + (lq & 15);
        const float xs = (sl < S) ? -cst[lq & 15] * inv_temperature : -3.0e38f;
        mb = row_max_f32(xs);
        ex = (sl < S) ? fast_expf(xs - mb) : 0.f;
        zb = row_sum_f32(ex);
        dpart = 0.f;
        if (tq < N) {
            const float mu = mean_l[tq];
            float df[FUSED_WAVES];
#pragma unroll
            for (int w = 0; w < FUSED_WAVES; ++w) df[w] = tiles[w * (H * NT_STRIDE) + tq] - mu;
            fmac_row_bcast_seq(dpart, ex, df);
        }
        if (NB > 1) {
            if (bt == 0) { pm0 = mb; pz0 = zb; pe0 = ex; } else { pm1 = mb; pz1 = zb; pe1 = ex; }
        }
        FSTAMP(4);
        const unsigned tag = tag0 + (unsigned)it;
        if (NB == 1 && nc > 1 && tq == 0) {
            granule_t* mine = xch + ((size_t)(it & 1) * P * nc + (size_t)p * nc + chunk) * FUSED_XCHG;
            st_granule(mine + 0, mb, tag);
            st_granule(mine + 1, zb, tag);
        }
        if (tq < N) delta[cc * FUSED_LD + hh] = dpart;
        __syncthreads();
        if (wave < 4) {
#ifndef FUSED_NO_PUBPRIO
            if (NB == 1) __builtin_amdgcn_s_setprio(3);
#endif
            const int li = tq & 15, lg = (tq >> 4) & 3;
            const f32x4 sd = sigma_times_delta(li, lg);
            if (NB == 1 && nc > 1) {
                granule_t* mine = xch + ((size_t)(it & 1) * P * nc + (size_t)p * nc + chunk) * FUSED_XCHG;
                if (li < DCH) {
#pragma unroll
                    for (int r = 0; r < 4; ++r) st_granule(mine + 2 + (16 * wave + 4 * lg + r) * DCH + li, sd[r], tag);
                }
            } else if (NB > 1 && bt > 0) {
                sd1 = sd;
            } else {
                sd0 = sd;
            }
        }
        FSTAMP(5);
        const bool more_batches = NB > 1 && bt + 1 < NB;
        const int it_n = more_batches ? it : it + 1;
        const int s_n = NB > 1 ? (more_batches ? bt + 1 : 0) * FUSED_WAVES + wave : s;
#ifdef FUSED_T_SKIP_NOISE
        if (false) {
#else
        if (it_n < n_run) {
#endif
            f32x4 acc[4];
            int jv = j, gv = g;
            asm volatile("" : "+v"(jv), "+v"(gv));
            uint32_t slo = seed_lo, shi = seed_hi;
            asm volatile("" : "+s"(slo), "+s"(shi));
            uint32_t pg = particle_offset + (uint32_t)p;
            if (NB > 1) asm volatile("" : "+s"(pg));
#ifndef FUSED_NOISE_PRIO
#define FUSED_NOISE_PRIO STOMP_PRIO_PROGRESS
#endif
            int lane_w = lane;
            asm volatile("" : "+v"(lane_w));
            if constexpr (PAIRED) {
                if (wave < PAIR_STRIDE) {
                    stomp_noise_bf16_pair<DCH, FUSED_NOISE_PRIO>(Limg, acc, eps ? eps + (size_t)it_n * eps_stride : nullptr, P, S, p, jv, gv,
                                                                 pg, (uint32_t)s_n, (uint32_t)(s_n + PAIR_STRIDE),
                                                                 iter0 + (uint32_t)it_n, slo, shi, 3 - (wave >> 1));
                    stomp_noise_to_tile_pair<DCH>(nt, nt + PAIR_STRIDE * (H * NT_STRIDE), acc, lane_w);
                }
            } else {
                auto prefetch = [&]() {
                    if (PRE && nc == 2) {
                        int lp = lane;
                        asm volatile("" : "+v"(lp));
                        const granule_t* slot0 = xch + ((size_t)(it & 1) * P * nc + (size_t)p * nc) * FUSED_XCHG;
                        const int wv = wave < DCH ? wave : DCH - 1;
                        const granule_t* gsrc = slot0 + (size_t)(lp >> 5) * FUSED_XCHG + 2 + 64 * wv + 2 * (lp & 31);
                        __builtin_amdgcn_global_load_lds((const __attribute__((address_space(1))) void*)gsrc,
                                                         (__attribute__((address_space(3))) void*)(sm.pre + wave * 128), 16, 0, 16);
                        if (lp < 2)
                            __builtin_amdgcn_global_load_lds((const __attribute__((address_space(1))) void*)(slot0 + (size_t)lp * FUSED_XCHG),
                                                             (__attribute__((address_space(3))) void*)(sm.premz + wave * 4), 16, 0, 16);
                    }
                };
                if constexpr (PRE)
                    stomp_noise_bf16<DCH, FUSED_NOISE_PRIO>(Limg, acc, eps ? eps + (size_t)it_n * eps_stride + (size_t)(s_n < S ? s_n : 0) * DCH * P * H : nullptr,
                                                            P, p, jv, gv, pg, (uint32_t)s_n, iter0 + (uint32_t)it_n,
                                                            slo, shi, 3 - (wave >> 2), prefetch);
                else
                    stomp_noise_bf16<DCH, FUSED_NOISE_PRIO>(Limg, acc, eps ? eps + (size_t)it_n * eps_stride + (size_t)(s_n < S ? s_n : 0) * DCH * P * H : nullptr,
                                                            P, p, jv, gv, pg, (uint32_t)s_n, iter0 + (uint32_t)it_n,
                                                            slo, shi, 3 - (wave >> 2));
                stomp_noise_to_tile(nt, acc, lane_w);
            }
            if (FUSED_NOISE_PRIO == STOMP_PRIO_STAGGER) __builtin_amdgcn_s_setprio(0);
        }
        if (PAIRED && more_batches) __syncthreads();
        }
        float m_all = mb, z_all = zb, f_own = 1.f, f_own0 = 1.f, f_sd0 = 1.f, f_sd1 = 0.f;
        const unsigned tag = tag0 + (unsigned)it;
        float dsum = 0.f;
        FSTAMP(6);
        if (NB > 1) {
            m_all = fmaxf(pm0, pm1);
            const float f0 = fast_expf(pm0 - m_all), f1 = fast_expf(pm1 - m_all);
            z_all = fmaf(f1, pz1, fmaf(f0, pz0, 0.f));
            f_own0 = f0;
            f_own = f1;
            f_sd0 = f0;
            f_sd1 = f1;
        }
        if (NB == 1 && nc > 1) {
            float mk[FUSED_MAX_CHUNKS], zk[FUSED_MAX_CHUNKS], dk[FUSED_MAX_CHUNKS];
            const granule_t* slot0 = xch + ((size_t)(it & 1) * P * nc + (size_t)p * nc) * FUSED_XCHG;
            bool have = false;
            if (PRE && nc == 2 && it + 1 < n_run) {
                asm volatile("s_waitcnt vmcnt(0)" ::: "memory");
                const granule_t* mine = sm.pre + wave * 128;
                const granule_t* mz = sm.premz + wave * 4;
                const granule_t g0 = mine[tq & 63], g1 = mine[64 + (tq & 63)];
                const granule_t gm0 = mz[0], gz0 = mz[1], gm1 = mz[2], gz1 = mz[3];
                have = (unsigned)(g0 >> 32) == tag && (unsigned)(g1 >> 32) == tag && (unsigned)(gm0 >> 32) == tag && (unsigned)(gz0 >> 32) == tag &&
                       (unsigned)(gm1 >> 32) == tag && (unsigned)(gz1 >> 32) == tag;
#pragma unroll
                for (int k = 2; k < FUSED_MAX_CHUNKS; ++k) { mk[k] = -3.0e38f; zk[k] = 0.f; dk[k] = 0.f; }
                mk[0] = __uint_as_float((unsigned)gm0); zk[0] = __uint_as_float((unsigned)gz0);
                mk[1] = __uint_as_float((unsigned)gm1); zk[1] = __uint_as_float((unsigned)gz1);
                dk[0] = (tq < N) ? __uint_as_float((unsigned)g0) : 0.f;
                dk[1] = (tq < N) ? __uint_as_float((unsigned)g1) : 0.f;
            }
#ifdef FUSED_T_PRE_STATS
            if (!have) ++pre_miss_;
#endif
            const unsigned long long t0 = __builtin_amdgcn_s_memrealtime();
            for (;;) {
                if (have) break;
                bool ok = true;
                auto poll_chunk = [&](auto kc) {
                    constexpr int k = decltype(kc)::value;
                    mk[k] = -3.0e38f; zk[k] = 0.f; dk[k] = 0.f;
                    if (k < nc) {
                        const granule_t* theirs = slot0 + (size_t)k * FUSED_XCHG;
                        const granule_t gm = ld_granule(theirs + 0), gz = ld_granule(theirs + 1);
                        const granule_t gd = ld_granule(theirs + 2 + (tq < N ? tq : 0));
                        ok = ok && (unsigned)(gm >> 32) == tag && (unsigned)(gz >> 32) == tag && (unsigned)(gd >> 32) == tag;
                        mk[k] = __uint_as_float((unsigned)gm);
                        zk[k] = __uint_as_float((unsigned)gz);
                        dk[k] = (tq < N) ? __uint_as_float((unsigned)gd) : 0.f;
                    }
                };
                static_assert(FUSED_MAX_CHUNKS == 4, "poll_chunk is called once per chunk");
                poll_chunk(std::integral_constant<int, 0>{});
                poll_chunk(std::integral_constant<int, 1>{});
                poll_chunk(std::integral_constant<int, 2>{});
                poll_chunk(std::integral_constant<int, 3>{});
                if (ok) break;
                __builtin_amdgcn_s_sleep(2);
                if (__builtin_amdgcn_s_memrealtime() - t0 > timeout_ticks) { s_abort = 1; break; }
            }
            FSTAMP(7);
            m_all = mk[0];
#pragma unroll
            for (int k = 1; k < FUSED_MAX_CHUNKS; ++k) m_all = fmaxf(m_all, mk[k]);
            z_all = 0.f;
            dsum = 0.f;
#pragma unroll
            for (int k = 0; k < FUSED_MAX_CHUNKS; ++k) {
                if (k < nc) {
                    const float f = fast_expf(mk[k] - m_all);
                    z_all = fmaf(f, zk[k], z_all);
                    dsum = fmaf(f, dk[k], dsum);
                }
            }
            f_own = fast_expf(mb - m_all);
        }
        FSTAMP(8);
        const float rz = fast_rcpf(z_all);
        if (NB > 1) {
            const int sl0 = tq & 15;
            if (last_it && tq < FUSED_WAVES && sl0 < S) weights[(size_t)p * S + sl0] = pe0 * f_own0 * rz;
            if (last_it && tq < FUSED_WAVES && sl < S) weights[(size_t)p * S + sl] = pe1 * f_own * rz;
        } else {
            w_out = ex * f_own * rz;
        }
        if (NB == 1 && nc > 1) {
            if (tq < N) mean_l[tq] += lr * (dsum * rz);
        } else if (wave < 4) {
            const int li = tq & 15, lg = (tq >> 4) & 3;
            if (li < DCH) {
#pragma unroll
                for (int r = 0; r < 4; ++r) {
                    float ds = fmaf(f_sd0, sd0[r], 0.f);
                    if (NB > 1) ds = fmaf(f_sd1, sd1[r], ds);
                    mean_l[(16 * wave + 4 * lg + r) * DCH + li] += lr * (ds * rz);
                }
            }
        }
        FSTAMP(9);
        FSTAMP(10);
        __syncthreads();
        FSTAMP(11);
        if (s_abort) break;
        if (it < 3) LSTAMP(4 + it);
    }
#ifdef FUSED_T_PRE_STATS
    if (pre_miss_ > 1) atomicAdd(&g_pre_miss[wave], (unsigned)(pre_miss_ - 1));
#endif
    const int aborted = s_abort;
    if (NB == 1 && !aborted && n_run > 0) {
        if (live) {
            const f32x4* pk4 = reinterpret_cast<const f32x4*>(nt);
            f32x4* out4 = reinterpret_cast<f32x4*>(samples + ((size_t)p * S + s) * N);
#pragma unroll
            for (int k = 0; k < (16 * DCH + 63) / 64; ++k) {
                const unsigned idx = (unsigned)lane + 64u * k;
                if (idx < 16u * DCH) out4[idx] = pk4[idx];
            }
            if (lane == 0) {
                bool bad = false;
                if (MODEL != 0) {
                    for (const float* gp = geom;;) {
                        const GeomView G = geom_view(gp);
                        if (G.model != MODEL || (!CHAIN && G.next != 0)) bad = true;
                        if (!CHAIN || G.next == 0) break;
                        gp += G.next;
                    }
                }
                if (bad) reinterpret_cast<unsigned*>(costs)[(size_t)p * S + s] = 0x7FC00000u;
                else costs[(size_t)p * S + s] = cst[wave];
            }
        }
        const int sl = chunk * FUSED_WAVES + (tid & 15);
        if (tid < FUSED_WAVES && sl < S) weights[(size_t)p * S + sl] = w_out;
    }
    if (!aborted && chunk == 0 && tid < N) {
        const float m = mean_l[tid];
        means[(size_t)p * N + tid] = m;
        if (means_copy) means_copy[(size_t)p * N + tid] = m;
    }
    if (aborted == 1 && chunk == 0 && tid < N && means_copy) means_copy[(size_t)p * N + tid] = means[(size_t)p * N + tid];
    if (aborted == 2 && (int)blockIdx.x < P && tid < N && means_copy) means_copy[(size_t)blockIdx.x * N + tid] = means[(size_t)blockIdx.x * N + tid];
    asm volatile("s_waitcnt vmcnt(0)" ::: "memory");
    __syncthreads();
    if (tid == 0) {
        LSTAMP(7);
        fused_leave(wsu, status_host, tag0, aborted);
    }
}

size_t mpb_fused_ws_floats(int P, int nc) { return fused_ws_floats(P, nc); }

int mpb_fused_launch(const StompCall& c, const StompLaunch& l, const StompFusedGrid& g) {
    const bool two_batches = g.nb == 2;
    const dim3 grid(two_batches ? c.P : c.P * g.nc), block(FUSED_THREADS);
    const int nc_k = two_batches ? 1 : g.nc;
    const int model = mpb_flags_model_on_grids(c.geom_flags, PandaModel::ID) ? PandaModel::ID : 0, d = c.d;
    const uint32_t lo = (uint32_t)c.seed, hi = (uint32_t)(c.seed >> 32);
#define MPB_F_LAUNCH_(DCH, MODEL, NB, INJ, CHAIN)                                                                                       \
    MPB_LAUNCH(l.events, (stomp_fused_kernel<DCH, MODEL, NB, INJ, CHAIN>), grid, block, 0, l.stream, c.means, c.eps, c.samples, c.costs, \
               c.weights, c.L, c.Sigma, c.geom, g.workspace, c.P, c.S, nc_k, c.k_sigma, c.weight, c.lr, c.temperature, l.n_iters, lo,   \
               hi, l.iter0, c.particle_offset, g.tag0, g.timeout, g.status_dev, l.means_copy)
    const bool one_field = mpb_flags_one_field(c.geom_flags);
#define MPB_F_LAUNCH(DCH, MODEL, NB, INJ)                                              \
    do {                                                                               \
        if ((MODEL) != 0 && one_field) MPB_F_LAUNCH_(DCH, MODEL, NB, INJ, (MODEL) == 0); \
        else MPB_F_LAUNCH_(DCH, MODEL, NB, INJ, true);                                 \
    } while (0)
#define MPB_F_CASE(DCH, MODEL)                                             \
    do {                                                                   \
        if (two_batches && c.eps) MPB_F_LAUNCH(DCH, MODEL, 2, true);       \
        else if (two_batches) MPB_F_LAUNCH(DCH, MODEL, 2, false);          \
        else if (c.eps) MPB_F_LAUNCH(DCH, MODEL, 1, true);                 \
        else MPB_F_LAUNCH(DCH, MODEL, 1, false);                           \
    } while (0)
    if (model == PandaModel::ID && d == 7) MPB_F_CASE(7, PandaModel::ID);
    else if (model == PandaModel::ID && d == 14) MPB_F_CASE(14, PandaModel::ID);
    else if (d == 2) MPB_F_CASE(2, 0);
    else if (d == 3) MPB_F_CASE(3, 0);
    else if (d == 4) MPB_F_CASE(4, 0);
    else if (d == 6) MPB_F_CASE(6, 0);
    else if (d == 7) MPB_F_CASE(7, 0);
    else MPB_F_CASE(14, 0);
#undef MPB_F_CASE
#undef MPB_F_LAUNCH
#undef MPB_F_LAUNCH_
    return mpb_check_launch("mpb_stomp_run");
}
```

motion_planning_baselines_amd/csrc/mpb_stomp_host.h:

```cpp
#pragma once
#include <hip/hip_runtime.h>
#include <hip/hip_ext.h>
#include <stdint.h>

#include "mpb_host.h"

#define MPB_MAX_D 16

struct StompCall {
    float* means;
    const float* eps;
    float *samples, *costs, *weights;
    const float *L, *Sigma, *geom;
    int geom_flags;
    int P, S, H, d, D;
    float k_sigma, weight, lr, temperature;
    uint64_t seed;
    uint32_t particle_offset;
};

struct StompEvents { hipEvent_t start, stop; };
#define MPB_LAUNCH(ev, kernel, grid, block, lds, st, ...)                                                                   \
    do {                                                                                                                    \
        if ((ev) != nullptr) hipExtLaunchKernelGGL(kernel, grid, block, lds, st, (ev)->start, (ev)->stop, 0, __VA_ARGS__);  \
        else hipLaunchKernelGGL(kernel, grid, block, lds, st, __VA_ARGS__);                                                 \
    } while (0)

struct StompLaunch {
    int n_iters;
    uint32_t iter0;
    float* means_copy;
    hipStream_t stream;
    const StompEvents* events;
};

struct StompFusedGrid {
    float* workspace;
    int nc;
    int nb;
    uint32_t tag0;
    unsigned long long timeout;
    unsigned* status_dev;
};

void mpb_stomp_launch_sample(const StompCall& c, const float* eps_it, uint32_t iter, hipStream_t st, const StompEvents* ev);
bool mpb_stomp_launch_update(const StompCall& c, hipStream_t st, const StompEvents* ev);
size_t mpb_fused_ws_floats(int P, int nc);
int mpb_fused_launch(const StompCall& c, const StompLaunch& l, const StompFusedGrid& g);
bool mpb_fused_hx_plan(int geom_flags, int n_cu, int P, int S, int H, int d, int* nc_out, int* nb_out, size_t* ws_bytes);
int mpb_fused_hx_launch(const StompCall& c, const StompLaunch& l, const StompFusedGrid& g);
```

motion_planning_baselines_amd/ops.py:

```python
import collections
import ctypes
import functools
import math
import warnings

import numpy as np
import torch

from . import _lib, rrt_layout
from .geometry import KIND_CHAIN, MAX_FIELDS, CollisionField, count_fields, occupancy_bytes, pack_geometry, pack_sdf_grid, pack_self_collision
from .geometry import header as geometry_header


_raw_stream = getattr(torch._C, '_cuda_getCurrentRawStream', None)


def raw_stream(device_index):
    if _raw_stream is not None:
        return _raw_stream(device_index)
    return torch.cuda.current_stream(device_index).cuda_stream


def _stream():
    return ctypes.c_void_p(torch.cuda.current_stream().cuda_stream)
# ... 262 lines not shown
        gap = torch.empty(N, device=q.device, dtype=torch.float32) if with_gap else None
    _lib.check(_lib.lib().mpb_sdf_grid_collision_check(_ptr(q), _ptr(sdf.buf), _ptr(flag), _ptr(gap), N, D, int(or_into), _stream()),
               'mpb_sdf_grid_collision_check')
    return (flag, gap) if (with_gap or gap is not None) else flag


@_on_tensor_device
def cost_collision_eval(trajs, geom, k_sigma, weight=1.0, h_begin=1, per_waypoint=False):
    B, H, d = trajs.shape
    _chk(trajs, (B, H, d), 'trajs')
    out = torch.empty(B, device=trajs.device, dtype=torch.float32)
    pw = torch.empty(B, H, device=trajs.device, dtype=torch.float32) if per_waypoint else None
    _lib.check(_lib.lib().mpb_cost_collision_eval(_ptr(trajs), _ptr(geom.buf), _ptr(out), _ptr(pw), B, H, d, h_begin,
                                                 float(k_sigma), float(weight), _stream()), 'mpb_cost_collision_eval')
    return (out, pw) if per_waypoint else out


@_on_tensor_device
def cost_collision_grad(trajs, geom, k_sigma, weight=1.0, h_begin=1, grad=None):
    B, H, d = trajs.shape
    _chk(trajs, (B, H, d), 'trajs')
    out = torch.empty(B, device=trajs.device, dtype=torch.float32)
    if grad is None:
        grad = torch.empty_like(trajs)
    else:
        _chk(grad, (B, H, d), 'grad')
    _lib.check(_lib.lib().mpb_cost_collision_grad(_ptr(trajs), _ptr(geom.buf), int(geom.flags), _ptr(out), _ptr(grad), B, H, d, h_begin,
                                                 float(k_sigma), float(weight), _stream()), 'mpb_cost_collision_grad')
    return out, grad


TERM_GP, TERM_START, TERM_GOAL, TERM_SMOOTH, TERM_JLIM, TERM_VEL_FD = 1, 2, 4, 8, 16, 32


def _term_flags(terms, B, n_dof, vel_fd, start_state, goal_states, trajs_per_goal, q_min, q_max):
    terms = set(terms or ())
    unknown = terms - {'gp', 'start', 'goal', 'smooth', 'jlim'}
    if unknown:
        raise ValueError(f'unknown cost terms {sorted(unknown)}')
    flags = 0
    if 'gp' in terms:
        flags |= TERM_GP | (TERM_VEL_FD if vel_fd else 0)
    if 'start' in terms:
        flags |= TERM_START
        _chk(start_state, (2 * n_dof,), 'start_state')
    if 'goal' in terms:
        flags |= TERM_GOAL
        if goal_states is None or goal_states.ndim != 2:
            raise ValueError('goal_states (G, 2*n_dof) is required')
        _chk(goal_states, (goal_states.shape[0], 2 * n_dof), 'goal_states')
        if trajs_per_goal < 1 or goal_states.shape[0] * trajs_per_goal < B:
            raise ValueError(f'{goal_states.shape[0]} goals x {trajs_per_goal} trajectories do not cover B={B}')
    if 'smooth' in terms:
        flags |= TERM_SMOOTH
    if 'jlim' in terms:
        flags |= TERM_JLIM
        _chk(q_min, (n_dof,), 'q_min')
        _chk(q_max, (n_dof,), 'q_max')
    return flags


@_on_tensor_device
def cost_terms_eval(trajs, n_dof, dt=0.0, k_gp=0.0, vel_fd=False, k_start=0.0, start_state=None, k_goal=0.0,
                    goal_states=None, trajs_per_goal=1, k_smooth=0.0, k_jlim=0.0, q_min=None, q_max=None, jl_eps=0.0,
                    out=None, accumulate=False, broadcast_jlim=True, terms=None):
    B, H, d = trajs.shape
    _chk(trajs, (B, H, d), 'trajs')
    flags = _term_flags(terms, B, n_dof, vel_fd, start_state, goal_states, trajs_per_goal, q_min, q_max)
    jl_total = torch.zeros((), device=trajs.device, dtype=torch.float64) if flags & TERM_JLIM else None
    if out is None:
        if accumulate:
            raise ValueError('accumulate needs an existing out buffer')
        out = torch.empty(B, device=trajs.device, dtype=torch.float32)
    else:
        if out.numel() != B:
            raise ValueError(f'out has {out.numel()} elements, expected {B}')
        _chk(out, out.shape, 'out')
    _lib.check(_lib.lib().mpb_cost_terms_eval(
        _ptr(trajs), _ptr(out), _ptr(jl_total), _ptr(start_state), _ptr(goal_states), _ptr(q_min), _ptr(q_max),
        B, H, d, int(n_dof), int(trajs_per_goal), flags, float(dt), float(k_gp), float(k_start), float(k_goal),
        float(k_smooth), float(k_jlim), float(jl_eps), int(bool(accumulate)), int(bool(broadcast_jlim)), _stream()),
        'mpb_cost_terms_eval')
    return out, jl_total


def _need_all_links(geom):
    if not getattr(geom, 'all_links', True):
        raise ValueError('this geometry leaves out collision spheres that cannot reach an obstacle; the per-sphere entry '
                         'points need DeviceGeometry(..., keep_all_links=True)')


@_on_tensor_device
def fk_collision_points(q, geom):
    B, H, d = q.shape
    _chk(q, (B, H, d), 'q')
    _need_all_links(geom)
    L = geom.n_links
    pts = torch.empty(B, H, L, 3, device=q.device, dtype=torch.float32)
    _lib.check(_lib.lib().mpb_fk_collision_points(_ptr(q), _ptr(geom.buf), _ptr(pts), B, H, d, _stream()), 'mpb_fk_collision_points')
    return pts


@_on_tensor_device
def fk_collision_points_vjp(q, geom, grad_pts):
    B, H, d = q.shape
    _need_all_links(geom)
    L = geom.n_links
    _chk(q, (B, H, d), 'q')
    _chk(grad_pts, (B, H, L, 3), 'grad_pts')
    gq = torch.empty(B, H, geom.n_dof, device=q.device, dtype=torch.float32)
    _lib.check(_lib.lib().mpb_fk_collision_points_vjp(_ptr(q), _ptr(geom.buf), _ptr(grad_pts), _ptr(gq), B, H, d, _stream()),
               'mpb_fk_collision_points_vjp')
    return gq


@_on_tensor_device
def field_cost_points(pts, geom):
    B, H, L, _ = pts.shape
    _need_all_links(geom)
    _chk(pts, (B, H, geom.n_links, 3), 'pts')
    cost = torch.empty(B, H, device=pts.device, dtype=torch.float32)
    _lib.check(_lib.lib().mpb_field_cost_points(_ptr(pts), _ptr(geom.buf), _ptr(cost), B, H, _stream()), 'mpb_field_cost_points')
    return cost


@_on_tensor_device
def field_cost_points_vjp(pts, geom, grad_cost):
    B, H, L, _ = pts.shape
    _need_all_links(geom)
    _chk(pts, (B, H, geom.n_links, 3), 'pts')
    _chk(grad_cost, (B, H), 'grad_cost')
    gp = torch.empty_like(pts)
    _lib.check(_lib.lib().mpb_field_cost_points_vjp(_ptr(pts), _ptr(geom.buf), _ptr(grad_cost), _ptr(gp), B, H, _stream()),
               'mpb_field_cost_points_vjp')
    return gp


@_on_tensor_device
def gp_factor_error(x, D, dt):
    B, H, dim = x.shape
    _chk(x, (B, H, 2 * D), 'x')
    out = torch.empty(B, H - 1, dim, device=x.device, dtype=torch.float32)
    _lib.check(_lib.lib().mpb_gp_factor_error(_ptr(x), _ptr(out), B, H, D, float(dt), _stream()), 'mpb_gp_factor_error')
    return out


@_on_tensor_device
def cost_terms_grad(trajs, n_dof, grad_in=None, grad_out=None, apply=False, R=None, prior_bw=0.0, lr=0.0, grad_clip=0.0,
                    jl_scale=1.0, dt=0.0, k_gp=0.0, vel_fd=False, k_start=0.0, start_state=None, k_goal=0.0,
                    goal_states=None, trajs_per_goal=1, k_smooth=0.0, k_jlim=0.0, q_min=None, q_max=None, jl_eps=0.0,
                    terms=None):
    B, H, d = trajs.shape
    _chk(trajs, (B, H, d), 'trajs')
    flags = _term_flags(terms, B, n_dof, vel_fd, start_state, goal_states, trajs_per_goal, q_min, q_max)
    if grad_in is not None:
        _chk(grad_in, (B, H, d), 'grad_in')
    if not apply:
        if grad_out is None:
            grad_out = torch.empty(B, H, d, device=trajs.device, dtype=torch.float32)
        _chk(grad_out, (B, H, d), 'grad_out')
    if prior_bw != 0.0:
        _chk(R, (H, H), 'R')
    _lib.check(_lib.lib().mpb_cost_terms_grad(
        _ptr(trajs), _ptr(grad_in), _ptr(grad_out), _ptr(R), _ptr(start_state), _ptr(goal_states), _ptr(q_min), _ptr(q_max),
        B, H, d, int(n_dof), int(trajs_per_goal), flags, float(dt), float(k_gp), float(k_start), float(k_goal),
        float(k_smooth), float(k_jlim), float(jl_eps), float(jl_scale), float(prior_bw), float(lr), float(grad_clip),
        int(bool(apply)), _stream()), 'mpb_cost_terms_grad')
    return grad_out


@_on_tensor_device
def traj_interpolate(trajs, n_interp):
    B, H, d = trajs.shape
    _chk(trajs, (B, H, d), 'trajs')
    n = int(n_interp)
    out = torch.empty(B, (H - 1) * (n + 1) + 1, d, device=trajs.device, dtype=torch.float32)
    _lib.check(_lib.lib().mpb_traj_interpolate(_ptr(trajs), _ptr(out), B, H, d, n, _stream()), 'mpb_traj_interpolate')
    return out


@_on_tensor_device
def traj_resample(paths, lengths, H, dt):
    N, Lmax, D = paths.shape
    _chk(paths, (N, Lmax, D), 'paths')
    if not (lengths.is_cuda and lengths.dtype == torch.int32 and lengths.is_contiguous() and tuple(lengths.shape) == (N,)):
        raise ValueError('lengths must be a contiguous int32 GPU tensor of shape (N,)')
    out = torch.empty(N, H, 2 * D, device=paths.device, dtype=torch.float32)
    _lib.check(_lib.lib().mpb_traj_resample(_ptr(paths), _ptr(lengths), _ptr(out), N, Lmax, int(H), D, float(dt), _stream()),
               'mpb_traj_resample')
    return out


@_on_tensor_device
def traj_finite_difference(pos, dt):
    B, H, D = pos.shape
    _chk(pos, (B, H, D), 'pos')
    out = torch.empty(B, H, 2 * D, device=pos.device, dtype=torch.float32)
    _lib.check(_lib.lib().mpb_traj_finite_difference(_ptr(pos), _ptr(out), B, H, D, float(dt), _stream()),
               'mpb_traj_finite_difference')
    return out


def _stomp_shapes(means, samples, costs, weights, L, Sigma, S):
    P, H, d = means.shape
    _chk(means, (P, H, d), 'means')
    _chk(samples, (P, S, H, d), 'samples')
    _chk(costs, (P, S), 'costs')
    _chk(weights, (P, S), 'weights')
    _chk(L, (H, H), 'L')
    _chk(Sigma, (H, H), 'Sigma')
    return P, H, d


def _stomp_head(eps, means, samples, costs, weights, L, Sigma, geom, S, D, k_sigma, weight, lr, temperature, workspace=False):
    P, H, d = means.shape
    bufs = (means,) + (() if eps is False else (eps,)) + (samples, costs, weights, L, Sigma, geom.buf)
    ws = () if workspace is False else (_ptr(workspace), 0 if workspace is None else workspace.numel() * 4)
    return (*map(_ptr, bufs), int(geom.flags), *ws, P, S, H, d, D, float(k_sigma), float(weight), float(lr), float(temperature))


@_on_tensor_device
def stomp_step(means, eps, samples, costs, weights, L, Sigma, geom, S, D, k_sigma, weight, lr, temperature,
               n_iters=1, seed=0, iter0=0, particle_offset=0):
    P, H, d = _stomp_shapes(means, samples, costs, weights, L, Sigma, S)
    if eps is not None:
        _chk(eps, (n_iters, S, d, P, H), 'eps')
    _lib.check(_lib.lib().mpb_stomp_step(
        *_stomp_head(eps, means, samples, costs, weights, L, Sigma, geom, S, D, k_sigma, weight, lr, temperature),
        int(n_iters), _seed64(seed), int(iter0), int(particle_offset), _stream()), 'mpb_stomp_step')


def stomp_workspace(P, S, H, d, device):
    n = int(_lib.lib().mpb_stomp_workspace_bytes(int(P), int(S), int(H), int(d)))
    ws = torch.empty((n + 3) // 4, device=device, dtype=torch.float32)
    with torch.cuda.device(ws.device):
        _lib.check(_lib.lib().mpb_stomp_workspace_init(_ptr(ws), ws.numel() * 4, _stream()), 'mpb_stomp_workspace_init')
    return ws


STOMP_PATH_TWO_KERNEL, STOMP_PATH_PERSISTENT_EXCHANGE, STOMP_PATH_PERSISTENT = 0, 1, 2


def stomp_run_path(geom, workspace, P, S, H, d):
    nbytes = 0 if workspace is None else workspace.numel() * 4
    with torch.cuda.device(geom.buf.device):
        return int(_lib.lib().mpb_stomp_run_path(int(geom.flags), nbytes, int(P), int(S), int(H), int(d)))


class StompRunStatus:

    def __init__(self):
        self.buf = torch.zeros(8, dtype=torch.int32).pin_memory()
        self._view = self.buf.numpy().view(np.uint32)
        self.issued = []
        self.tag_c = ctypes.c_uint32(0)

    def ptr(self):
        return ctypes.c_void_p(self.buf.data_ptr())

    def note_launch(self):
        tag = int(self.tag_c.value)
        if tag:
            self.issued.append(tag)
        return tag

    def lost(self):
        lost, done = int(self._view[1]), int(self._view[0])
        if lost and lost in self.issued:
            return lost, int(self._view[2])
        if done in self.issued:
            del self.issued[:self.issued.index(done) + 1]
        return None

    def device_span_ms(self):
        v = self._view
        if int(v[0]) == 0:
            return None
        t0, t1 = int(v[4]) | (int(v[5]) << 32), int(v[6]) | (int(v[7]) << 32)
        return (t1 - t0) * 1e-5 if t1 > t0 else None

    def acknowledge(self, tag):
        if tag in self.issued:
            del self.issued[:self.issued.index(tag) + 1]


@_on_tensor_device
def stomp_run(means, eps, samples, costs, weights, L, Sigma, geom, S, D, k_sigma, weight, lr, temperature, workspace,
              n_iters=1, seed=0, iter0=0, particle_offset=0, status=None, means_copy=None):
    P, H, d = _stomp_shapes(means, samples, costs, weights, L, Sigma, S)
    if eps is not None:
        _chk(eps, (n_iters, S, d, P, H), 'eps')
    if workspace is not None:
        _chk(workspace, tuple(workspace.shape), 'workspace')
    if means_copy is not None:
        _chk(means_copy, (P, H, d), 'means_copy')
    _lib.check(_lib.lib().mpb_stomp_run_checked(
        *_stomp_head(eps, means, samples, costs, weights, L, Sigma, geom, S, D, k_sigma, weight, lr, temperature, workspace),
        int(n_iters), _seed64(seed), int(iter0), int(particle_offset),
        None if status is None else status.ptr(), None if status is None else ctypes.byref(status.tag_c), _ptr(means_copy),
        _stream()), 'mpb_stomp_run')
    return 0 if status is None else status.note_launch()


class StompRunPlan:

    def __init__(self, means, samples, costs, weights, L, Sigma, geom, S, D, k_sigma, weight, lr, temperature, workspace,
                 seed, particle_offset, status):
        P, H, d = _stomp_shapes(means, samples, costs, weights, L, Sigma, S)
        _chk(workspace, tuple(workspace.shape), 'workspace')
        devs = {t.device for t in (means, samples, costs, weights, L, Sigma, geom.buf, workspace)}
        if len(devs) != 1:
            raise ValueError(f'StompRunPlan: tensors live on different devices ({devs})')
        self.device = means.device
        self.shape = (P, H, d)
        self.key = (means.data_ptr(), samples.data_ptr(), costs.data_ptr(), weights.data_ptr(), L.data_ptr(),
                    Sigma.data_ptr(), geom.buf.data_ptr(), workspace.data_ptr(), S, D, float(k_sigma), float(weight),
                    float(lr), float(temperature), int(seed), int(particle_offset))
        self._call = (means, samples, costs, weights, L, Sigma, geom, S, D, k_sigma, weight, lr, temperature, workspace)
        self._seed, self._poff = _seed64(seed), int(particle_offset)
        self._status = status
        self._status_ptr = status.ptr()
        self._tag_ref = ctypes.byref(status.tag_c)
        h = ctypes.c_void_p(0)
        _lib.check(_lib.lib().mpb_stomp_plan_create(
            ctypes.byref(h), *_stomp_head(False, *self._call), self._seed, self._poff, self._status_ptr),
            'mpb_stomp_plan_create')
        self._handle = h
        self._launch = _lib.lib().mpb_stomp_plan_launch
        self._destroy = _lib.lib().mpb_stomp_plan_destroy

    def __del__(self):
        h = getattr(self, '_handle', None)
        if h is not None and h.value:
            self._destroy(h)
            self._handle = None

    def launch_timed(self, n_iters, iter0, means_copy=None):
        ms = ctypes.c_float(0.0)
        rc = _lib.lib().mpb_stomp_run_timed(*_stomp_head(None, *self._call), int(n_iters), self._seed,
                                            int(iter0), self._poff, self._status_ptr,
                                            self._tag_ref, None if means_copy is None else means_copy.data_ptr(),
                                            torch.cuda.current_stream(self.device).cuda_stream, ctypes.byref(ms))
        if rc != 0:
            _lib.check(rc, 'mpb_stomp_run_timed')
        self._status.note_launch()
        return float(ms.value)

    def launch(self, n_iters, iter0, means_copy=None):
        rc = self._launch(self._handle, n_iters, iter0, None if means_copy is None else means_copy.data_ptr(),
                          raw_stream(self.device.index), self._tag_ref)
        if rc != 0:
            _lib.check(rc, 'mpb_stomp_run')
        return self._status.note_launch()


def stomp_run_state(workspace):
    out = ctypes.c_int(0)
    with torch.cuda.device(workspace.device):
        _lib.check(_lib.lib().mpb_stomp_run_status(_ptr(workspace), _stream(), ctypes.cast(ctypes.pointer(out), ctypes.c_void_p)),
                   'mpb_stomp_run_status')
    return int(out.value)


def stomp_run_timed_out(workspace):
    return stomp_run_state(workspace) != 0


def debug_philox(ctr, key, rounds):
    ctr = np.ascontiguousarray(np.asarray(ctr, dtype=np.uint32).reshape(-1, 4))
    key = np.ascontiguousarray(np.asarray(key, dtype=np.uint32).reshape(-1, 2))
    n = ctr.shape[0]
    dev = torch.device('cuda', torch.cuda.current_device())
    c = torch.from_numpy(ctr.view(np.int32)).to(dev)
    k = torch.from_numpy(key.view(np.int32)).to(dev)
    out = torch.empty(n, 4, dtype=torch.int32, device=dev)
    _lib.debug_check(_lib.debug_lib().mpb_debug_philox(_ptr(c), _ptr(k), _ptr(out), n, int(rounds), _stream()), 'mpb_debug_philox')
    return out.cpu().numpy().view(np.uint32)


def debug_stomp_normals(P, S, d, n_iters, device, seed=0, iter0=0, particle_offset=0, H=64):
    Hp = 64 * ((int(H) + 63) // 64)
    out = torch.empty(n_iters, P, S, d, Hp, device=device, dtype=torch.float32)
    with torch.cuda.device(out.device):
        _lib.debug_check(_lib.debug_lib().mpb_debug_stomp_normals_h(_ptr(out), int(P), int(S), int(d), int(H), int(n_iters),
                                                                    _seed64(seed), int(iter0), int(particle_offset), _stream()),
                         'mpb_debug_stomp_normals_h')
    return out


def debug_mppi_normals(NP, S, T, c, n_iters, device, seed=0, iter0=0):
    out = torch.empty(n_iters, NP, c, S, T, device=device, dtype=torch.float32)
    with torch.cuda.device(out.device):
        _lib.debug_check(_lib.debug_lib().mpb_debug_mppi_normals(_ptr(out), int(NP), int(S), int(T), int(c), int(n_iters),
                                                                 _seed64(seed), int(iter0), _stream()), 'mpb_debug_mppi_normals')
    return out


def debug_occupy(n_blocks, usec, device):
    sink = torch.zeros(1, dtype=torch.int32, device=device)
    with torch.cuda.device(sink.device):
        _lib.debug_check(_lib.debug_lib().mpb_debug_occupy(int(n_blocks), int(usec), _ptr(sink), _stream()), 'mpb_debug_occupy')
    return sink


@_on_tensor_device
def stomp_step_profile(means, samples, costs, weights, L, Sigma, geom, S, D, k_sigma, weight, lr, temperature,
                       n_iters=50, seed=0, iter0=0, particle_offset=0):
    _stomp_shapes(means, samples, costs, weights, L, Sigma, S)
    ka, kb = ctypes.c_float(0.0), ctypes.c_float(0.0)
    _lib.check(_lib.lib().mpb_stomp_step_profile(
        *_stomp_head(False, means, samples, costs, weights, L, Sigma, geom, S, D, k_sigma, weight, lr, temperature),
        int(n_iters), _seed64(seed), int(iter0), int(particle_offset), _stream(),
        ctypes.cast(ctypes.pointer(ka), ctypes.c_void_p), ctypes.cast(ctypes.pointer(kb), ctypes.c_void_p)),
        'mpb_stomp_step_profile')
    return float(ka.value), float(kb.value)


@_on_tensor_device
def stomp_sample(means, eps, samples, L, S, seed=0, it=0, particle_offset=0, geom=None, costs=None, k_sigma=0.0,
                 weight=1.0):
    P, H, d = means.shape
    _chk(means, (P, H, d), 'means')
    _chk(samples, (P, S, H, d), 'samples')
    _chk(L, (H, H), 'L')
    if eps is not None:
        _chk(eps, (S, d, P, H), 'eps')
    if (geom is None) != (costs is None):
        raise ValueError('geom and costs must be given together')
    if costs is not None:
        _chk(costs, (P, S), 'costs')
    _lib.check(_lib.lib().mpb_stomp_sample(_ptr(means), _ptr(eps), _ptr(samples), _ptr(L),
                                          _ptr(None if geom is None else geom.buf),
                                          0 if geom is None else int(geom.flags), _ptr(costs), P, S, H, d,
                                          float(k_sigma), float(weight), _seed64(seed), int(it),
                                          int(particle_offset), _stream()), 'mpb_stomp_sample')


@_on_tensor_device
def stomp_update(means, samples, costs, weights, Sigma, lr, temperature):
    P, S, H, d = samples.shape
    _chk(means, (P, H, d), 'means')
    _chk(samples, (P, S, H, d), 'samples')
    _chk(costs, (P, S), 'costs')
    _chk(weights, (P, S), 'weights')
    _chk(Sigma, (H, H), 'Sigma', allow_none=True)
    _lib.check(_lib.lib().mpb_stomp_update(_ptr(means), _ptr(samples), _ptr(costs), _ptr(weights), _ptr(Sigma),
                                          P, S, H, d, float(lr), float(temperature), _stream()), 'mpb_stomp_update')


@_on_tensor_device
def chomp_step(means, R, geom, D, k_sigma, weight, w_prior, lr, grad_clip, n_iters=1, B_global=None, costs_out=None):
    B, H, d = means.shape
    _chk(means, (B, H, d), 'means')
    _chk(R, (H, H), 'R')
    _chk(costs_out, (B,), 'costs_out', allow_none=True)
    _lib.check(_lib.lib().mpb_chomp_step(_ptr(means), _ptr(R), _ptr(geom.buf), int(geom.flags), _ptr(costs_out), B,
                                        B if B_global is None else int(B_global), H, d, D, float(k_sigma), float(weight),
                                        float(w_prior), float(lr), float(grad_clip), int(n_iters), _stream()),
               'mpb_chomp_step')


@_on_tensor_device
def gpmp2_workspace(B, H, D, device):
    n = int(_lib.lib().mpb_gpmp2_workspace_bytes(B, H, D))
    if n == 0:
        raise ValueError(f'unsupported GPMP2 shape B={B} H={H} D={D}')
    return torch.empty(n, dtype=torch.uint8, device=device)


@_on_tensor_device
def gpmp2_step(x, start, goal, geom, workspace, sigmas, dt, delta, trust_region, step_size, n_iters=1, costs_out=None,
               n_interp=0):
    B, H, dim = x.shape
    D = dim // 2
    _chk(x, (B, H, dim), 'x')
    _chk(start, (B, dim), 'start')
    _chk(goal, (B, dim), 'goal')
    _chk(costs_out, (B,), 'costs_out', allow_none=True)
    assert workspace.numel() >= _lib.lib().mpb_gpmp2_workspace_bytes(B, H, D)
    _lib.check(_lib.lib().mpb_gpmp2_step(
        _ptr(x), _ptr(start), _ptr(goal), _ptr(geom.buf), int(geom.flags), _ptr(workspace), _ptr(costs_out), B, H, D, float(dt),
        float(sigmas[0]), float(sigmas[1]), float(sigmas[2]), float(sigmas[3]), float(delta), int(bool(trust_region)),
        float(step_size), int(n_iters), int(n_interp or 0), int(geom.n_fields), _stream()), 'mpb_gpmp2_step')


@_on_tensor_device
def gpmp2_linearize(x, geom, workspace, n_interp=0):
    B, H, dim = x.shape
    _chk(x, (B, H, dim), 'x')
    _lib.check(_lib.lib().mpb_gpmp2_linearize(_ptr(x), _ptr(geom.buf), int(geom.flags), _ptr(workspace), B, H, dim // 2,
                                              int(n_interp or 0), _stream()), 'mpb_gpmp2_linearize')


@_on_tensor_device
def gpmp2_collision_rows(x, geom, n_interp=0):
    B, H, dim = x.shape
    D = dim // 2
    _chk(x, (B, H, dim), 'x')
    if _lib.lib().mpb_gpmp2_workspace_bytes(B, H, D) == 0:
        raise ValueError(f'unsupported GPMP2 shape B={B} H={H} D={D}')
    jac = torch.zeros(MAX_FIELDS, B, H, D + 1, device=x.device, dtype=torch.float32)
    _lib.check(_lib.lib().mpb_gpmp2_linearize(_ptr(x), _ptr(geom.buf), int(geom.flags), _ptr(jac), B, H, D, int(n_interp or 0), _stream()),
               'mpb_gpmp2_linearize')
    return jac[:geom.n_fields]


@_on_tensor_device
def gpmp2_diag(workspace, B, H, D, sigmas, dt, n_fields=1):
    out = torch.empty(H * 2 * D, dtype=torch.float64, device=workspace.device)
    _lib.check(_lib.lib().mpb_gpmp2_diag(_ptr(workspace), _ptr(out), B, H, D, int(n_fields), float(dt), float(sigmas[0]),
                                        float(sigmas[1]), float(sigmas[2]), float(sigmas[3]), _stream()), 'mpb_gpmp2_diag')
    return out


@_on_tensor_device
def gpmp2_solve(x, start, goal, diag_mean, workspace, sigmas, dt, delta, trust_region, step_size, costs_out=None,
                n_fields=1):
    B, H, dim = x.shape
    _chk(x, (B, H, dim), 'x')
    _chk(start, (B, dim), 'start')
    _chk(goal, (B, dim), 'goal')
    _chk(diag_mean, (H * dim,), 'diag_mean', allow_none=True, dtype=torch.float64)
    _lib.check(_lib.lib().mpb_gpmp2_solve(
        _ptr(x), _ptr(start), _ptr(goal), _ptr(diag_mean), _ptr(workspace), _ptr(costs_out), B, H, dim // 2, int(n_fields),
        float(dt), float(sigmas[0]), float(sigmas[1]), float(sigmas[2]), float(sigmas[3]), float(delta), int(bool(trust_region)),
        float(step_size), _stream()), 'mpb_gpmp2_solve')


@_on_tensor_device
def mppi_step(mean, eps, scale_tril, cov_inv, state0, goal, ctrl_min, ctrl_max, discount, c_weights, geom, controls,
              states, costs, weights, dt, k_sigma=0.0, weight=1.0, temp=1.0, step_size=1.0, n_iters=1, seed=0, iter0=0,
              best_cost=None, best_states=None):
    NP, T, c = mean.shape
    S = controls.shape[1]
    _chk(mean, (NP, T, c), 'mean')
    if eps is not None:
        _chk(eps, (n_iters, NP, c, S, T), 'eps')
    _chk(scale_tril, (c, T, T), 'scale_tril')
    _chk(cov_inv, (c, T, T), 'cov_inv')
    _chk(state0, (NP, c), 'state0')
    _chk(goal, (NP, c), 'goal')
    _chk(ctrl_min, (c,), 'ctrl_min')
    _chk(ctrl_max, (c,), 'ctrl_max')
    _chk(discount, (T,), 'discount')
    _chk(c_weights, (4,), 'c_weights')
    _chk(controls, (NP, S, T, c), 'controls')
    _chk(states, (NP, S, T, c), 'states')
    _chk(costs, (NP, S), 'costs')
    _chk(weights, (NP, S), 'weights')
    if (best_cost is None) != (best_states is None):
        raise ValueError('best_cost and best_states must be given together')
    _chk(best_cost, (NP,), 'best_cost', allow_none=True)
    _chk(best_states, (NP, T, c), 'best_states', allow_none=True)
    _lib.check(_lib.lib().mpb_mppi_step(
        _ptr(mean), _ptr(eps), _ptr(scale_tril), _ptr(cov_inv), _ptr(state0), _ptr(goal), _ptr(ctrl_min), _ptr(ctrl_max),
        _ptr(discount), _ptr(c_weights), _ptr(None if geom is None else geom.buf), 0 if geom is None else int(geom.flags),
        _ptr(controls), _ptr(states),
        _ptr(costs), _ptr(weights), _ptr(best_cost), _ptr(best_states), NP, S, T, c, 0, float(dt), float(k_sigma),
        float(weight), float(temp),
        float(step_size), int(n_iters), _seed64(seed), int(iter0), _stream()), 'mpb_mppi_step')


MPPI_NOISE_GLOBAL, MPPI_NOISE_LDS, MPPI_NOISE_MATRIX = 0, 1, 2
MppiPlan = collections.namedtuple('MppiPlan', 'noise_mode waves grid_words lds_bytes')


def mppi_plan(geom, NP, S, T, c, has_eps=False, n_cu=0):
    out = (ctypes.c_int * 4)()
    flags = 0 if geom is None else int(geom.flags if isinstance(geom, DeviceGeometry) else geom)
    args = (flags, int(geom is not None), int(NP), int(S), int(T), int(c), int(bool(has_eps)), int(n_cu), ctypes.cast(out, ctypes.c_void_p))
    if isinstance(geom, DeviceGeometry):
        with torch.cuda.device(geom.buf.device):
            rc = _lib.lib().mpb_mppi_plan(*args)
    else:
        rc = _lib.lib().mpb_mppi_plan(*args)
    _lib.check(rc, 'mpb_mppi_plan')
    return MppiPlan(*[int(v) for v in out])


@_on_tensor_device
def point_dynamics(x, u, ctrl_min, ctrl_max, dt, dyn_std=None, noise=None):
    dim = x.shape[-1]
    _chk(x, tuple(x.shape), 'x')
    _chk(u, tuple(x.shape), 'u')
    _chk(ctrl_min, (dim,), 'ctrl_min')
    _chk(ctrl_max, (dim,), 'ctrl_max')
    if noise is not None:
        _chk(noise, tuple(x.shape), 'noise')
        _chk(dyn_std, (dim,), 'dyn_std')
    out = torch.empty_like(x)
    _lib.check(_lib.lib().mpb_point_dynamics(_ptr(x), _ptr(u), _ptr(ctrl_min), _ptr(ctrl_max), _ptr(dyn_std if noise is not None else None),
                                            _ptr(noise), _ptr(out), x.numel() // dim, dim, float(dt), _stream()), 'mpb_point_dynamics')
    return out


@_on_tensor_device
def point_traj_cost(X, U, goal, discount, w_pos, w_vel, w_ctrl, w_pos_T, energy=0.0):
    T, B, sd = X.shape
    cd = U.shape[-1]
    _chk(X, (T, B, sd), 'X')
    _chk(U, (T, B, cd), 'U')
    _chk(goal, (sd,), 'goal')
    _chk(discount, (T,), 'discount')
    out = torch.empty(B, device=X.device, dtype=torch.float32)
    _lib.check(_lib.lib().mpb_point_traj_cost(_ptr(X), _ptr(U), _ptr(goal), _ptr(discount), float(w_pos), float(w_vel), float(w_ctrl),
                                             float(w_pos_T), float(energy), _ptr(out), T, B, sd, cd, _stream()), 'mpb_point_traj_cost')
    return out


@_on_tensor_device
def mvn_sample_dense(means, eps, tril_t, n, seed=0):
    G, M = means.shape
    _chk(means, (G, M), 'means', dtype=torch.float64)
    _chk(tril_t, (M, M), 'tril_t', dtype=torch.float64)
    _chk(eps, (n, G, M), 'eps', allow_none=True, dtype=torch.float64)
    out = torch.empty(G * n, M, device=means.device, dtype=torch.float32)
    _lib.check(_lib.lib().mpb_mvn_sample_dense(_ptr(out), _ptr(means), _ptr(eps), _ptr(tril_t), G, n, M,
                                              _seed64(seed), _stream()), 'mpb_mvn_sample_dense')
    return out


@_on_tensor_device
def gp_prior_sample(means, eps, Udiag, Uoff, n, D, seed=0, scale_tril=None, out=None):
    G, H, dim = means.shape
    _chk(means, (G, H, 2 * D), 'means', dtype=torch.float64)
    _chk(Udiag, (H, 3), 'Udiag', dtype=torch.float64)
    _chk(Uoff, (H - 1, 4), 'Uoff', dtype=torch.float64)
    _chk(eps, (n, G, H * dim), 'eps', allow_none=True, dtype=torch.float64)
    if out is None:
        out = torch.empty(G * n, H, dim, device=means.device, dtype=torch.float32)
    else:
        _chk(out, (G * n, H, dim), 'out')
    if scale_tril is not None and H <= 128:
        _chk(scale_tril, (2 * H, 2 * H), 'scale_tril', dtype=torch.float64)
        _lib.check(_lib.lib().mpb_gp_prior_sample_dense(_ptr(out), _ptr(means), _ptr(eps), _ptr(scale_tril), G, n, H, D,
                                                       _seed64(seed), _stream()), 'mpb_gp_prior_sample_dense')
        return out
    _lib.check(_lib.lib().mpb_gp_prior_sample(_ptr(out), _ptr(means), _ptr(eps), _ptr(Udiag), _ptr(Uoff), G, n, H, D,
                                             _seed64(seed), _stream()), 'mpb_gp_prior_sample')
    return out


@_on_tensor_device
def stoch_gpmp_step(means, means64, samples, costs, weights, Udiag, Uoff, scale_tril, start, goal, geom, S, sig_cost,
                    sig_sample, dt, temperature, step_size, n_iters=1, seed=0):
    P, H, dim = means.shape
    _chk(means, (P, H, dim), 'means')
# ... 448 lines not shown
```

motion_planning_baselines_amd/planners/stomp.py:

```python
import time

import torch

from .. import ops
from .._lib import MPBError
from .base import OptimizationPlanner
from .costs.cost_functions import device_plan, fusable_collision


def stomp_precision_matrix(n_support_points, dt, sigma_spectral, tensor_args):
    H = n_support_points
    inner = -2 * torch.eye(H) + torch.diag(torch.ones(H - 1), 1) + torch.diag(torch.ones(H - 1), -1)
    A = torch.cat((torch.zeros(1, H), inner, torch.zeros(1, H)), dim=0)
    A[0, 0] = 1.
    A[-1, -1] = 1.
    A = A * 1. / dt ** 2 * sigma_spectral
    return (A.t() @ A).to(**tensor_args)


def precision_to_scale_tril(P):
    Lf = torch.linalg.cholesky(torch.flip(P, (-2, -1)))
    L_inv = torch.transpose(torch.flip(Lf, (-2, -1)), -2, -1)
    Id = torch.eye(P.shape[-1], dtype=P.dtype, device=P.device)
    return torch.linalg.solve_triangular(L_inv, Id, upper=False).contiguous()


_current_device = getattr(torch._C, '_cuda_getDevice', torch.cuda.current_device)
_perf_counter = time.perf_counter
_SYNC_SPIN_S = 1e-3


class PersistentLaunchLost(MPBError):
    """A persistent (one-launch) optimisation loop was abandoned by the device side: see STOMP's `check` argument."""


class STOMP(OptimizationPlanner):

    def __init__(self, n_dof, n_support_points, num_particles_per_goal, num_samples, opt_iters, dt, start_state,
                 cost=None, initial_particle_means=None, multi_goal_states=None, sigma_start_init=0.001,
                 sigma_goal_init=0.001, sigma_gp_init=10., temperature=1., step_size=1., sigma_spectral=0.1,
                 goal_state=None, pos_only=True, tensor_args=None, noise='philox', seed=0, particle_offset=0,
                 persistent=True, check='sync', **kwargs):
        super().__init__(name='STOMP', n_dof=n_dof, n_support_points=n_support_points,
                         num_particles_per_goal=num_particles_per_goal, opt_iters=opt_iters, dt=dt,
                         start_state=start_state, cost=cost, initial_particle_means=initial_particle_means,
                         multi_goal_states=multi_goal_states, sigma_start_init=sigma_start_init,
                         sigma_goal_init=sigma_goal_init, sigma_gp_init=sigma_gp_init, pos_only=pos_only,
                         tensor_args=tensor_args)
        assert noise in ('philox', 'torch', 'torch_cpu', 'mt19937')
        assert check in ('deferred', 'sync')
        self.check = check
        self._status = None
        self._plan = None
        self._last_tag = 0
        self._spare_copy = None
        self._eps_ring = None
        self._eps_dev = None
        self._traj_out = None
        self.lr = step_size
        self.sigma_spectral = sigma_spectral
        self.start_state = start_state
        self.goal_state = goal_state
        self.num_samples = num_samples
        self.temperature = temperature
        self.noise = noise
        self.seed = int(seed)
        self.particle_offset = int(particle_offset)
        self._iter = 0
        self._weights = None
        self._run_ws = None
        self.persistent = bool(persistent)
        cpu = dict(device='cpu', dtype=torch.float32)
        R = stomp_precision_matrix(n_support_points, dt, sigma_spectral, cpu)
        self.Sigma_inv = R.to(self.device)
        self.Sigma = torch.inverse(R).to(self.device).contiguous()
        self.scale_tril = precision_to_scale_tril(R).to(self.device).contiguous()
        P, S, H, d = self.num_particles, num_samples, n_support_points, self.d_state_opt
        self.state_particles = torch.empty(P, S, H, d, device=self.device, dtype=torch.float32)
        self.costs = torch.zeros(P, S, device=self.device, dtype=torch.float32)
        self._weights_buf = torch.empty(P, S, device=self.device, dtype=torch.float32)
        self.reset(initial_particle_means=initial_particle_means)
        self.best_cost = torch.inf

    def _get_R_mat(self):
        return stomp_precision_matrix(self.n_support_points, self.dt, self.sigma_spectral,
                                      dict(device='cpu', dtype=torch.float32)).to(self.device)

    def set_noise_dist(self):
        self.scale_tril = precision_to_scale_tril(self.Sigma_inv.detach().cpu().float()).to(self.device).contiguous()

    def const_vel_trajectory(self, start_state, goal_state):
        H, D = self.n_support_points, self.n_dof
        start_state, goal_state = start_state.detach().cpu().float(), goal_state.detach().cpu().float()
        n = H - 1
        traj = torch.zeros(H, self.d_state_opt)
        for i in range(H):
            traj[i, :D] = start_state[:D] * (n - i) * 1. / n + goal_state[:D] * i * 1. / n
        if not self.pos_only:
            traj[:, D:] = ((goal_state[:D] - start_state[:D]) / (n * self.dt)).unsqueeze(0)
        return traj.to(self.device)

    def _calc_sample_weights(self, costs):
        costs = costs.reshape(self.num_particles, self.num_samples).to(torch.float32).contiguous()
        w = torch.empty_like(costs)
        ops.stomp_update(self._particle_means, self.state_particles, costs, w, self.Sigma, 0.0, self.temperature)
        return w.reshape(self.num_particles, self.num_samples, 1, 1)

    def _draw_eps(self, n_iters):
        if self.noise == 'philox':
            return None
        S, d, P, H = self.num_samples, self.d_state_opt, self.num_particles, self.n_support_points
        if self.noise == 'mt19937':
            return ops.torch_cpu_normal_(torch.empty(n_iters, S, d, P, H, device=self.device, dtype=torch.float32), n_iters)
        dev = 'cpu' if self.noise == 'torch_cpu' else self.device
        blocks = [torch.empty(S, d, P, H, device=dev, dtype=torch.float32).normal_() for _ in range(n_iters)]
        return torch.stack(blocks).to(self.device).contiguous()

    def sample(self):
        self._raise_if_lost()
        eps = self._draw_eps(1)
        ops.stomp_sample(self._particle_means, None if eps is None else eps[0], self.state_particles,
                         self.scale_tril, self.num_samples, seed=self.seed, it=self._iter,
                         particle_offset=self.particle_offset)
        self._iter += 1
        return self.state_particles

    def reset(self, initial_particle_means=None):
        self._raise_if_lost()
        if initial_particle_means is not None:
            m = initial_particle_means.clone()
        else:
            m = self.get_random_trajs()
        self._particle_means = m.to(device=self.device, dtype=torch.float32).contiguous()
        self.state_particles = self.sample()

    def optimize(self, opt_iters=None, **observation):
        self._traj_out = None
        self._last_tag = 0
        self._run_optimization(opt_iters, **observation)
        if self.check == 'sync':
            self._raise_if_lost(synchronize=True, tag=self._last_tag)
        if self._traj_out is not None:
            out, self._traj_out = self._traj_out, None
            return out
        return self._get_traj()

    def get_traj(self):
        self._raise_if_lost()
        return self._get_traj()

    def _raise_if_lost(self, synchronize=False, tag=0):
        if self._status is None:
            return
        if synchronize:
            t_end = _perf_counter() + _SYNC_SPIN_S
            stream = torch.cuda.current_stream(self.device)
            if tag:
                view = self._status._view
                while int(view[0]) != tag and int(view[1]) != tag:
                    if _perf_counter() > t_end:
                        stream.synchronize()
                        break
            else:
                while not stream.query():
                    if _perf_counter() > t_end:
                        stream.synchronize()
                        break
        lost = self._status.lost()
        if lost is not None:
            tag, why = lost
            self._status.acknowledge(tag)
            raise PersistentLaunchLost(
                'the persistent STOMP launch (tag 0x%08x) was abandoned: %s.  The means of the particles it did not finish '
                'are unchanged from before that optimize() call; samples, costs and weights are undefined.  reset() the '
                'planner (or restore saved means) and run again; persistent=False selects the two-kernel path, which '
                'has no inter-workgroup waits.' % (tag, {
                    1: 'a workgroup waited longer than the bound for the partner workgroups of its particle (the device did '
                       'not start them: is another context or stream holding the whole GPU?)',
                    2: 'the workspace header was not zero before the first call'}.get(why, 'reason %d' % why)))

    def _run_optimization(self, opt_iters, **observation):
        if opt_iters is None:
            opt_iters = self.opt_iters
        self._raise_if_lost()
        fused = fusable_collision(self.cost)
        if fused is not None and not observation:
            cc, weight = fused
            geom = cc.device_geometry(self.device)
            if self.persistent and self._run_ws is None:
                self._run_ws = ops.stomp_workspace(self.num_particles, self.num_samples, self.n_support_points,
                                                   self.d_state_opt, self.device)
                self._status = ops.StompRunStatus()
            copy = None
            if not self.pos_only:
                copy, self._spare_copy = self._spare_copy, None
                m = self._particle_means
                if copy is None or copy.shape != m.shape or copy.device != m.device or copy.dtype != m.dtype:
                    copy = torch.empty_like(m)
            if (self.persistent and self.noise == 'philox' and self._particle_means.is_cuda
                    and _current_device() == self._particle_means.device.index):
                key = (self._particle_means.data_ptr(), self.state_particles.data_ptr(), self.costs.data_ptr(),
                       self._weights_buf.data_ptr(), self.scale_tril.data_ptr(), self.Sigma.data_ptr(), geom.buf.data_ptr(),
                       self._run_ws.data_ptr(), self.num_samples, self.n_dof, float(cc.k_sigma), float(weight), float(self.lr),
                       float(self.temperature), self.seed, self.particle_offset)
                plan = self._plan
                if plan is None or plan.key != key:
                    plan = self._plan = ops.StompRunPlan(
                        self._particle_means, self.state_particles, self.costs, self._weights_buf, self.scale_tril,
                        self.Sigma, geom, self.num_samples, self.n_dof, cc.k_sigma, weight, self.lr, self.temperature,
                        self._run_ws, self.seed, self.particle_offset, self._status)
                self._last_tag = plan.launch(opt_iters, self._iter, copy)
                if copy is not None:
                    self._spare_copy = torch.empty_like(copy)
            else:
                self._last_tag = self._run_fused_injected(opt_iters, geom, cc, weight, copy)
            self._traj_out = copy
            self._iter += opt_iters
        elif not observation and device_plan(self.cost, self.device) is not None:
            plan = device_plan(self.cost, self.device)
            cc, weight, groups = plan
            flat = self.state_particles.view(-1, self.n_support_points, self.d_state_opt)
            flat_costs = self.costs.view(-1)
            for _ in range(opt_iters):
                eps = self._draw_eps(1)
                ops.stomp_sample(self._particle_means, None if eps is None else eps[0], self.state_particles,
                                 self.scale_tril, self.num_samples, seed=self.seed, it=self._iter,
                                 particle_offset=self.particle_offset,
                                 geom=None if cc is None else cc.device_geometry(self.device),
                                 costs=None if cc is None else self.costs,
                                 k_sigma=0.0 if cc is None else cc.k_sigma, weight=weight)
                self._iter += 1
                have = cc is not None
                for om, w in plan.own:
                    om.own_eval(flat, weight=w, out=flat_costs, accumulate=have)
                    have = True
                for spec in groups:
                    ops.cost_terms_eval(flat, self.n_dof, out=self.costs, accumulate=have, **spec)
                    have = True
                ops.stomp_update(self._particle_means, self.state_particles, self.costs, self._weights_buf,
                                 self.Sigma, self.lr, self.temperature)
        else:
            for _ in range(opt_iters):
                self.costs = self._sample_and_eval(**observation)
                self._update_distribution(self.costs, self.state_particles)
        self._weights = self._weights_buf.reshape(self.num_particles, self.num_samples, 1, 1)

    def _run_fused_injected(self, opt_iters, geom, cc, weight, copy):
        run = lambda eps, n, it0, cp: ops.stomp_run(
            self._particle_means, eps, self.state_particles, self.costs, self._weights_buf, self.scale_tril, self.Sigma, geom,
            self.num_samples, self.n_dof, cc.k_sigma, weight, self.lr, self.temperature, self._run_ws if self.persistent else None,
            n_iters=n, seed=self.seed, iter0=it0, particle_offset=self.particle_offset,
            status=self._status if self.persistent else None, means_copy=cp)
        if self.noise == 'philox' or opt_iters <= 0:
            return run(None, opt_iters, self._iter, copy)
        S, d, P, H = self.num_samples, self.d_state_opt, self.num_particles, self.n_support_points
        tag = 0
        if self.noise in ('torch', 'mt19937'):
            chunk = min(opt_iters, 16)
            buf = self._eps_dev
            if buf is None or buf.shape != (chunk, S, d, P, H) or buf.device != self.device:
                buf = self._eps_dev = torch.empty(chunk, S, d, P, H, device=self.device, dtype=torch.float32)
            gen = ops.TorchCpuGeneratorOnDevice(self.device) if self.noise == 'mt19937' else None
            done = 0
            try:
                while done < opt_iters:
                    n = min(chunk, opt_iters - done)
                    if gen is not None:
                        gen.normal_(buf[:n], n)
                        if done + n == opt_iters:
                            gen.stage()
                    else:
                        for i in range(n):
                            buf[i].normal_()
                    tag = run(buf[:n], n, self._iter + done, copy if done + n == opt_iters else None)
                    done += n
            finally:
                if gen is not None:
                    gen.store()
            return tag
        ring = self._eps_ring
        if ring is None or ring['host'][0].shape != (1, S, d, P, H) or ring['dev'][0].device != self.device:
            ring = self._eps_ring = dict(
                host=[torch.empty(1, S, d, P, H, dtype=torch.float32).pin_memory() for _ in range(2)],
                dev=[torch.empty(1, S, d, P, H, device=self.device, dtype=torch.float32) for _ in range(2)],
                copied=[torch.cuda.Event() for _ in range(2)])
        for it in range(opt_iters):
            k = it & 1
            ring['copied'][k].synchronize()
            ring['host'][k].normal_()
            ring['dev'][k].copy_(ring['host'][k], non_blocking=True)
            ring['copied'][k].record()
            tag = run(ring['dev'][k], 1, self._iter + it, copy if it == opt_iters - 1 else None)
        return tag

    def persistent_timed_out(self):
        if self._run_ws is None or not self.persistent:
            return False
        lost = ops.stomp_run_timed_out(self._run_ws)
        if lost and self._status is not None:
            hit = self._status.lost()
            if hit is not None:
                self._status.acknowledge(hit[0])
        return lost

    def optimize_timed(self, opt_iters):
        self._run_optimization(0)
        if self._plan is None:
            return None
        ms = self._plan.launch_timed(opt_iters, self._iter)
        self._iter += opt_iters
        return ms if ms > 0.0 else None

    def run_path(self):
        fused = fusable_collision(self.cost)
        if fused is None or not self.persistent:
            return ops.STOMP_PATH_TWO_KERNEL
        ws = self._run_ws if self._run_ws is not None else ops.stomp_workspace(
            self.num_particles, self.num_samples, self.n_support_points, self.d_state_opt, self.device)
        return ops.stomp_run_path(fused[0].device_geometry(self.device), ws, self.num_particles, self.num_samples,
                                  self.n_support_points, self.d_state_opt)

    def _sample_and_eval(self, **observation):
        self.state_particles = self.sample()
        costs = self._get_costs(self.state_particles.flatten(0, 1), **observation)
        return costs.reshape(self.num_particles, self.num_samples).to(torch.float32).contiguous()

    def _update_distribution(self, costs, traj_particles):
        ops.stomp_update(self._particle_means, traj_particles, costs, self._weights_buf, self.Sigma, self.lr,
                         self.temperature)
        self._weights = self._weights_buf.reshape(self.num_particles, self.num_samples, 1, 1)
```

Before: 89420.

## Prebuild STOMP kernel constant image once per plan and copy it into LDS

Moves the per-launch staging of the collision grid, sphere table, L image and Sigma into a device-side image block that is built once when a plan is created or refreshed. The fused kernel then copies this block into LDS instead of recomputing the grid offset words and L layout on every launch. The plan key now tracks tensor versions so the image is rebuilt if L, Sigma or geometry change. This saves per-launch setup work but adds a device allocation and a risk of stale constants if invalidation is missed.

```diff
diff --git a/include/mpb.h b/include/mpb.h
--- a/include/mpb.h
+++ b/include/mpb.h
@@ -110,6 +110,10 @@
                           float k_sigma, float weight, float lr, float temperature, uint64_t seed, uint32_t particle_offset,
                           uint32_t *status);
 int mpb_stomp_plan_launch(mpb_stomp_plan *plan, int n_iters, uint32_t iter0, float *means_copy, void *stream, uint32_t *tag_out);
+int mpb_stomp_plan_refresh(mpb_stomp_plan *plan, void *stream);
+int mpb_stomp_plan_image_copy(mpb_stomp_plan *plan, void *out, size_t out_bytes, void *stream);
+int mpb_stomp_plan_launch_timed(mpb_stomp_plan *plan, int n_iters, uint32_t iter0, float *means_copy, void *stream,
+                                uint32_t *tag_out, float *kernel_ms);
 int mpb_stomp_plan_destroy(mpb_stomp_plan *plan);
 
 int mpb_stomp_sample(const float *means, const float *eps, float *samples, const float *L,
diff --git a/include/mpb_debug.h b/include/mpb_debug.h
--- a/include/mpb_debug.h
+++ b/include/mpb_debug.h
@@ -15,6 +15,7 @@
                             uint32_t particle_offset, void *stream);
 int mpb_debug_stomp_normals_h(float *out, int P, int S, int d, int H, int n_iters, uint64_t seed, uint32_t iter0,
                               uint32_t particle_offset, void *stream);
+int mpb_debug_stomp_image(void *out, const float *L, const float *Sigma, const float *geom, void *stream);
 int mpb_debug_mppi_normals(float *out, int NP, int S, int T, int c, int n_iters, uint64_t seed, uint32_t iter0, void *stream);
 
 int mpb_debug_mt19937_uniforms(float *out, int n, int n_calls, const uint32_t *state_in, int pos, int final_idx,
diff --git a/motion_planning_baselines_amd/_lib.py b/motion_planning_baselines_amd/_lib.py
--- a/motion_planning_baselines_amd/_lib.py
+++ b/motion_planning_baselines_amd/_lib.py
@@ -53,6 +53,9 @@
     'mpb_mvn_sample_dense': [_p, _p, _p, _p, _i, _i, _i, _u64, _p],
     'mpb_stomp_plan_create': [_p] * 8 + [_i, _p, ctypes.c_size_t, _i, _i, _i, _i, _i, _f, _f, _f, _f, _u64, _u32, _p],
     'mpb_stomp_plan_launch': [_p, _i, _u32, _p, _p, _p],
+    'mpb_stomp_plan_refresh': [_p, _p],
+    'mpb_stomp_plan_image_copy': [_p, _p, ctypes.c_size_t, _p],
+    'mpb_stomp_plan_launch_timed': [_p, _i, _u32, _p, _p, _p, _p],
     'mpb_stomp_plan_destroy': [_p],
     'mpb_point_dynamics': [_p, _p, _p, _p, _p, _p, _p, ctypes.c_size_t, _i, _f, _p],
     'mpb_point_traj_cost': [_p, _p, _p, _p, _f, _f, _f, _f, _f, _p, _i, _i, _i, _i, _p],
@@ -92,6 +95,7 @@
     'mpb_debug_philox': [_p, _p, _p, _i, _i, _p],
     'mpb_debug_stomp_normals': [_p, _i, _i, _i, _i, _u64, _u32, _u32, _p],
     'mpb_debug_stomp_normals_h': [_p, _i, _i, _i, _i, _i, _u64, _u32, _u32, _p],
+    'mpb_debug_stomp_image': [_p, _p, _p, _p, _p],
     'mpb_debug_mppi_normals': [_p, _i, _i, _i, _i, _i, _u64, _u32, _p],
     'mpb_debug_mt19937_uniforms': [_p, _i, _i, _p, _i, _i, _p, _p, _p, _i, _p, _i, _p, _p],
     'mpb_debug_mt19937_normals_timed': [_p, _i, _i, _p, _i, _i, _p, _p, _p, _i, _p, _i, _p, _p, _p],
diff --git a/motion_planning_baselines_amd/build.py b/motion_planning_baselines_amd/build.py
--- a/motion_planning_baselines_amd/build.py
+++ b/motion_planning_baselines_amd/build.py
@@ -38,8 +38,8 @@
 
 _LAYOUT = '../../include/mpb_geom_layout.h'
 PMC_SOURCES = {
-    'stomp': ['mpb_stomp_fused.hip', 'mpb_stomp_fused.h', 'mpb_stomp_noise.h', 'mpb_geom.h', _LAYOUT, 'mpb_common.h', 'mpb_model_panda.h'],
-    'stomp_c5': ['mpb_stomp_fused.hip', 'mpb_stomp_fused.h', 'mpb_stomp_noise.h', 'mpb_geom.h', _LAYOUT, 'mpb_common.h', 'mpb_model_panda.h'],
+    'stomp': ['mpb_stomp_fused.hip', 'mpb_stomp_fused.h', 'mpb_stomp_image.h', 'mpb_stomp_noise.h', 'mpb_geom.h', _LAYOUT, 'mpb_common.h', 'mpb_model_panda.h'],
+    'stomp_c5': ['mpb_stomp_fused.hip', 'mpb_stomp_fused.h', 'mpb_stomp_image.h', 'mpb_stomp_noise.h', 'mpb_geom.h', _LAYOUT, 'mpb_common.h', 'mpb_model_panda.h'],
     'stomp_h128': ['mpb_stomp_fused_hx.hip', 'mpb_stomp_fused.h', 'mpb_stomp_noise.h', 'mpb_geom.h', _LAYOUT, 'mpb_common.h', 'mpb_model_panda.h'],
     'kernelA': ['mpb_kernels.hip', 'mpb_stomp_noise.h', 'mpb_geom.h', _LAYOUT, 'mpb_common.h', 'mpb_model_panda.h'],
     'solve': ['mpb_gpmp2.hip', 'mpb_gpmp2_lr.hip', 'mpb_gpmp2.h', 'mpb_geom.h', _LAYOUT, 'mpb_common.h'],
diff --git a/motion_planning_baselines_amd/csrc/mpb_debug.hip b/motion_planning_baselines_amd/csrc/mpb_debug.hip
--- a/motion_planning_baselines_amd/csrc/mpb_debug.hip
+++ b/motion_planning_baselines_amd/csrc/mpb_debug.hip
@@ -4,6 +4,7 @@
 #include "mpb_host.h"
 #include "mpb_stomp_noise.h"
 #include "mpb_mt19937.h"
+#include "mpb_stomp_image.h"
 #include "../../include/mpb_debug.h"
 
 static thread_local char g_debug_err[512] = "";
@@ -103,6 +104,26 @@
     return mpb_check_launch("mpb_debug_mppi_normals");
 }
 
+__global__ __launch_bounds__(FUSED_THREADS) void debug_stomp_image_kernel(uint4* __restrict__ out, const float* __restrict__ Lmat,
+                                                                          const float* __restrict__ Sigma, const float* __restrict__ geom) {
+    __shared__ __attribute__((aligned(16))) FusedImage im;
+    uint4* im4 = reinterpret_cast<uint4*>(&im);
+    constexpr int N16 = (int)(sizeof(FusedImage) / 16);
+    for (int i = threadIdx.x; i < N16; i += FUSED_THREADS) im4[i] = make_uint4(0u, 0u, 0u, 0u);
+    __syncthreads();
+    const GeomView G0 = geom_view(geom);
+    fused_stage_image(im.otab, im.gridw, im.Limg, im.sig_l, G0, Lmat, Sigma, (int)threadIdx.x);
+    __syncthreads();
+    for (int i = threadIdx.x; i < N16; i += FUSED_THREADS) out[i] = im4[i];
+}
+
+extern "C" int mpb_debug_stomp_image(void* out, const float* L, const float* Sigma, const float* geom, void* stream) {
+    if (!out || !L || !Sigma || !geom) return mpb_fail(MPB_E_INVALID, "mpb_debug_stomp_image: null pointer");
+    if (mpb_misaligned16(out, L, Sigma, geom)) return mpb_fail(MPB_E_INVALID, "mpb_debug_stomp_image: out / L / Sigma / geom must be 16-byte aligned");
+    hipLaunchKernelGGL(debug_stomp_image_kernel, dim3(1), dim3(FUSED_THREADS), 0, (hipStream_t)stream, static_cast<uint4*>(out), L, Sigma, geom);
+    return mpb_check_launch("mpb_debug_stomp_image");
+}
+
 __global__ __launch_bounds__(64) void occupy_kernel(unsigned long long ticks, unsigned* sink) {
     __shared__ unsigned pad[150 * 256];
     pad[threadIdx.x] = threadIdx.x;
diff --git a/motion_planning_baselines_amd/csrc/mpb_stomp_api.hip b/motion_planning_baselines_amd/csrc/mpb_stomp_api.hip
--- a/motion_planning_baselines_amd/csrc/mpb_stomp_api.hip
+++ b/motion_planning_baselines_amd/csrc/mpb_stomp_api.hip
@@ -187,7 +187,8 @@
     return (f.path != MPB_STOMP_PATH_TWO_KERNEL && workspace_bytes >= f.ws_bytes) ? f.path : MPB_STOMP_PATH_TWO_KERNEL;
 }
 
-static int stomp_run(const StompCall& c, float* workspace, size_t workspace_bytes, uint32_t* status, const StompLaunch& l, uint32_t* tag_out) {
+static int stomp_run(const StompCall& c, float* workspace, size_t workspace_bytes, uint32_t* status, const StompLaunch& l, uint32_t* tag_out,
+                     const void* image = nullptr) {
     if (tag_out) *tag_out = 0u;
     if (c.P == 0) return MPB_OK;
     const FusedPlan f = fused_plan(c.geom_flags, c.P, c.S, c.H, c.d);
@@ -201,7 +202,7 @@
     if (const int rc = stomp_check(c, {"mpb_stomp_run", l.n_iters, false, false, "means / eps / samples / L / Sigma / geom / workspace / means_copy",
                                        workspace, l.means_copy}))
         return rc;
-    StompFusedGrid g = {workspace, f.nc, f.nb, 0u, 0ull, nullptr};
+    StompFusedGrid g = {workspace, f.nc, f.nb, 0u, 0ull, nullptr, image};
     if (status) {
         static thread_local uint32_t* seen_host = nullptr;
         static thread_local unsigned* seen_dev = nullptr;
@@ -250,6 +251,8 @@
     float* workspace;
     size_t workspace_bytes;
     uint32_t* status;
+    void* image;
+    bool image_built;
 };
 
 extern "C" int mpb_stomp_plan_create(mpb_stomp_plan** plan, float* means, float* samples, float* costs, float* weights, const float* L,
@@ -263,19 +266,68 @@
     if (const int rc = stomp_check(c, {__func__, 0, false, false, "means / samples / L / Sigma / geom / workspace", workspace})) return rc;
     mpb_stomp_plan_s* q = static_cast<mpb_stomp_plan_s*>(malloc(sizeof(mpb_stomp_plan_s)));
     if (!q) return mpb_failf(MPB_E_HIP, "%s: out of host memory", __func__);
-    *q = mpb_stomp_plan_s{c, workspace, workspace_bytes, status};
+    *q = mpb_stomp_plan_s{c, workspace, workspace_bytes, status, nullptr, false};
+    if (P > 0 && mpb_fused_takes_image(c) && hipMalloc(&q->image, mpb_fused_image_bytes()) != hipSuccess) {
+        (void)hipGetLastError();
+        free(q);
+        return mpb_failf(MPB_E_HIP, "%s: out of device memory (the image block)", __func__);
+    }
     *plan = q;
+    return MPB_OK;
+}
+
+extern "C" int mpb_stomp_plan_refresh(mpb_stomp_plan* plan, void* stream) {
+    if (!plan) return mpb_fail(MPB_E_INVALID, "mpb_stomp_plan_refresh: null plan");
+    if (!plan->image) return MPB_OK;
+    plan->image_built = true;
+    return mpb_fused_image_build(plan->call, plan->image, (hipStream_t)stream);
+}
+
+extern "C" int mpb_stomp_plan_image_copy(mpb_stomp_plan* plan, void* out, size_t out_bytes, void* stream) {
+    if (!plan || !out) return mpb_failf(MPB_E_INVALID, "%s: null pointer", __func__);
+    if (!plan->image) return mpb_failf(MPB_E_INVALID, "%s: the plan has no image block (its kernel stages the constants itself)", __func__);
+    if (out_bytes < mpb_fused_image_bytes()) return mpb_failf(MPB_E_INVALID, "%s: out holds %zu bytes, the block has %zu", __func__, out_bytes, mpb_fused_image_bytes());
+    if (!plan->image_built)
+        if (const int rc = mpb_stomp_plan_refresh(plan, stream)) return rc;
+    if (hipMemcpyAsync(out, plan->image, mpb_fused_image_bytes(), hipMemcpyDeviceToDevice, (hipStream_t)stream) != hipSuccess)
+        return mpb_failf(MPB_E_HIP, "%s: copy failed", __func__);
     return MPB_OK;
 }
 
 extern "C" int mpb_stomp_plan_launch(mpb_stomp_plan* plan, int n_iters, uint32_t iter0, float* means_copy, void* stream, uint32_t* tag_out) {
     if (!plan) return mpb_fail(MPB_E_INVALID, "mpb_stomp_plan_launch: null plan");
-    return stomp_run(plan->call, plan->workspace, plan->workspace_bytes, plan->status, {n_iters, iter0, means_copy, (hipStream_t)stream, nullptr}, tag_out);
+    if (plan->image && !plan->image_built)
+        if (const int rc = mpb_stomp_plan_refresh(plan, stream)) return rc;
+    return stomp_run(plan->call, plan->workspace, plan->workspace_bytes, plan->status, {n_iters, iter0, means_copy, (hipStream_t)stream, nullptr}, tag_out,
+                     plan->image);
 }
 
 extern "C" int mpb_stomp_plan_destroy(mpb_stomp_plan* plan) {
+    if (plan && plan->image) (void)hipFree(plan->image);
     free(plan);
     return MPB_OK;
+}
+
+static int stomp_run_timed(const char* who, const StompCall& c, float* workspace, size_t workspace_bytes, uint32_t* status, int n_iters,
+                           uint32_t iter0, float* means_copy, void* stream, uint32_t* tag_out, float* kernel_ms, const void* image) {
+    if (!kernel_ms) return mpb_failf(MPB_E_INVALID, "%s: null pointer", who);
+    *kernel_ms = 0.f;
+    StompEvents ev = {nullptr, nullptr};
+    if (hipEventCreate(&ev.start) != hipSuccess || hipEventCreate(&ev.stop) != hipSuccess) {
+        if (ev.start) (void)hipEventDestroy(ev.start);
+        return mpb_failf(MPB_E_HIP, "%s: hipEventCreate failed", who);
+    }
+    uint32_t tag = 0;
+    int rc = stomp_run(c, workspace, workspace_bytes, status, {n_iters, iter0, means_copy, (hipStream_t)stream, &ev}, &tag, image);
+    if (tag_out) *tag_out = tag;
+    if (rc == MPB_OK && hipStreamSynchronize((hipStream_t)stream) != hipSuccess) rc = mpb_failf(MPB_E_HIP, "%s: synchronize failed", who);
+    if (rc == MPB_OK && tag != 0u && hipEventElapsedTime(kernel_ms, ev.start, ev.stop) != hipSuccess) {
+        (void)hipGetLastError();
+        rc = mpb_failf(MPB_E_HIP, "%s: hipEventElapsedTime failed", who);
+    }
+    (void)hipEventDestroy(ev.start);
+    (void)hipEventDestroy(ev.stop);
+    return rc;
 }
 
 extern "C" int mpb_stomp_run_timed(float* means, const float* eps, float* samples, float* costs, float* weights,
@@ -283,26 +335,18 @@
                                    size_t workspace_bytes, int P, int S, int H, int d, int D, float k_sigma, float weight, float lr,
                                    float temperature, int n_iters, uint64_t seed, uint32_t iter0, uint32_t particle_offset,
                                    uint32_t* status, uint32_t* tag_out, float* means_copy, void* stream, float* kernel_ms) {
-    if (!kernel_ms) return mpb_failf(MPB_E_INVALID, "%s: null pointer", __func__);
-    *kernel_ms = 0.f;
-    StompEvents ev = {nullptr, nullptr};
-    if (hipEventCreate(&ev.start) != hipSuccess || hipEventCreate(&ev.stop) != hipSuccess) {
-        if (ev.start) (void)hipEventDestroy(ev.start);
-        return mpb_failf(MPB_E_HIP, "%s: hipEventCreate failed", __func__);
-    }
     const StompCall c = {means, eps, samples, costs, weights, L, Sigma, geom, geom_flags, P, S, H, d, D,
                          k_sigma, weight, lr, temperature, seed, particle_offset};
-    uint32_t tag = 0;
-    int rc = stomp_run(c, workspace, workspace_bytes, status, {n_iters, iter0, means_copy, (hipStream_t)stream, &ev}, &tag);
-    if (tag_out) *tag_out = tag;
-    if (rc == MPB_OK && hipStreamSynchronize((hipStream_t)stream) != hipSuccess) rc = mpb_failf(MPB_E_HIP, "%s: synchronize failed", __func__);
-    if (rc == MPB_OK && tag != 0u && hipEventElapsedTime(kernel_ms, ev.start, ev.stop) != hipSuccess) {
-        (void)hipGetLastError();
-        rc = mpb_failf(MPB_E_HIP, "%s: hipEventElapsedTime failed", __func__);
-    }
-    (void)hipEventDestroy(ev.start);
-    (void)hipEventDestroy(ev.stop);
-    return rc;
+    return stomp_run_timed(__func__, c, workspace, workspace_bytes, status, n_iters, iter0, means_copy, stream, tag_out, kernel_ms, nullptr);
+}
+
+extern "C" int mpb_stomp_plan_launch_timed(mpb_stomp_plan* plan, int n_iters, uint32_t iter0, float* means_copy, void* stream,
+                                           uint32_t* tag_out, float* kernel_ms) {
+    if (!plan) return mpb_failf(MPB_E_INVALID, "%s: null plan", __func__);
+    if (plan->image && !plan->image_built)
+        if (const int rc = mpb_stomp_plan_refresh(plan, stream)) return rc;
+    return stomp_run_timed(__func__, plan->call, plan->workspace, plan->workspace_bytes, plan->status, n_iters, iter0, means_copy, stream, tag_out,
+                           kernel_ms, plan->image);
 }
 
 extern "C" int mpb_stomp_run_status(const float* workspace, void* stream, int* timed_out) {
diff --git a/motion_planning_baselines_amd/csrc/mpb_stomp_fused.hip b/motion_planning_baselines_amd/csrc/mpb_stomp_fused.hip
--- a/motion_planning_baselines_amd/csrc/mpb_stomp_fused.hip
+++ b/motion_planning_baselines_amd/csrc/mpb_stomp_fused.hip
@@ -7,6 +7,7 @@
 #include "mpb_geom.h"
 #include "mpb_stomp_noise.h"
 #include "mpb_stomp_fused.h"
+#include "mpb_stomp_image.h"
 
 static inline size_t fused_ws_floats(int P, int nc) { return FUSED_HDR_WORDS + 2 * 2 * (size_t)P * nc * FUSED_XCHG; }
 
@@ -53,10 +54,7 @@
 #endif
 template <int DCH, bool PRE>
 struct FusedSmem {
-    float4 otab[MPB_GRID_MAX_SPH + 1];
-    unsigned gridw[MPB_GRID_MAX_CELLS];
-    unsigned Limg[STOMP_LIMG_WORDS];
-    float sig_l[64 * FUSED_LD];
+    FusedImage img;
     float mean_l[64 * DCH];
     float delta[DCH * FUSED_LD];
     float cst[FUSED_WAVES];
@@ -68,13 +66,14 @@
     __attribute__((aligned(16))) granule_t premz[PRE ? FUSED_WAVES * 4 : 2];
 };
 
-template <int DCH, int MODEL, int NB, bool INJ, bool CHAIN>
-__global__ __launch_bounds__(FUSED_THREADS, 4) void stomp_fused_kernel(
+template <int DCH, int MODEL, int NB, bool INJ, bool CHAIN, bool IMG>
+__device__ __forceinline__ void stomp_fused_body(
     float* __restrict__ means, const float* __restrict__ eps, float* __restrict__ samples, float* __restrict__ costs,
     float* __restrict__ weights, const float* __restrict__ Lmat, const float* __restrict__ Sigma,
     const float* __restrict__ geom, float* __restrict__ ws, int P, int S, int nc, float k_sigma, float weight, float lr,
     float temperature, int n_iters, uint32_t seed_lo, uint32_t seed_hi, uint32_t iter0, uint32_t particle_offset,
-    uint32_t tag0, unsigned long long timeout_ticks, unsigned* __restrict__ status_host, float* __restrict__ means_copy) {
+    uint32_t tag0, unsigned long long timeout_ticks, unsigned* __restrict__ status_host, float* __restrict__ means_copy,
+    const FusedImage* __restrict__ image) {
     constexpr int H = 64;
     constexpr int N = H * DCH;
     static_assert(N <= FUSED_THREADS && N + 2 <= FUSED_XCHG, "one thread per trajectory element");
@@ -85,10 +84,11 @@
     constexpr bool PRE = NB == 1 && 2 * DCH > 16 && MODEL != 0 && !INJ;
 #endif
     __shared__ __attribute__((aligned(16))) FusedSmem<DCH, PRE> sm;
-    float4 (&otab)[MPB_GRID_MAX_SPH + 1] = sm.otab;
-    unsigned (&gridw)[MPB_GRID_MAX_CELLS] = sm.gridw;
-    unsigned (&Limg)[STOMP_LIMG_WORDS] = sm.Limg;
-    float (&sig_l)[64 * FUSED_LD] = sm.sig_l;
+    static_assert(__builtin_offsetof(FusedSmem<DCH, PRE>, img) == 0, "the image block is copied to LDS offset 0");
+    float4 (&otab)[MPB_GRID_MAX_SPH + 1] = sm.img.otab;
+    unsigned (&gridw)[MPB_GRID_MAX_CELLS] = sm.img.gridw;
+    unsigned (&Limg)[STOMP_LIMG_WORDS] = sm.img.Limg;
+    float (&sig_l)[64 * FUSED_LD] = sm.img.sig_l;
     float (&mean_l)[64 * DCH] = sm.mean_l;
     float (&delta)[DCH * FUSED_LD] = sm.delta;
     float (&cst)[FUSED_WAVES] = sm.cst;
@@ -98,6 +98,19 @@
 
     const int tid = threadIdx.x, lane = tid & 63, wave = __builtin_amdgcn_readfirstlane(tid >> 6);
     LSTAMP(0);
+    if constexpr (IMG) {
+        if (wave != 0) {
+            const char* src = reinterpret_cast<const char*>(image) + 16 * lane;
+            char* dst = reinterpret_cast<char*>(&sm.img);
+#pragma unroll
+            for (int k = 0; k < (FUSED_IMAGE_KB + FUSED_WAVES - 2) / (FUSED_WAVES - 1); ++k) {
+                const int c = wave - 1 + (FUSED_WAVES - 1) * k;
+                if (c < FUSED_IMAGE_KB)
+                    __builtin_amdgcn_global_load_lds((const __attribute__((address_space(1))) void*)(src + 1024 * c),
+                                                     (__attribute__((address_space(3))) void*)(dst + 1024 * c), 16, 0, 0);
+            }
+        }
+    }
     unsigned* wsu = reinterpret_cast<unsigned*>(ws);
     const bool exchange = NB == 1 && nc > 1;
     if (tid == 0) {
@@ -117,28 +130,8 @@
 
     GeomView G0 = geom_view(geom);
     if (!CHAIN && G0.next != 0) G0.model = 0;
-    {
-        const int g_rounds = (G0.n_cells + 4 * FUSED_THREADS - 1) / (4 * FUSED_THREADS);
-        const uint4* g4 = reinterpret_cast<const uint4*>(G0.grid);
-        const int n_pad16 = (G0.n_cells + MPB_GRID_PAD - 1) / MPB_GRID_PAD * (MPB_GRID_PAD / 4);
-        for (int u = 0; u < (MPB_GRID_MAX_CELLS / 4 + FUSED_THREADS - 1) / FUSED_THREADS; ++u) {
-            const int i = tid + FUSED_THREADS * u;
-            if (u < g_rounds && i < n_pad16) {
-                const uint4 gw = g4[i];
-                const unsigned ns = (unsigned)G0.n_sph;
-                reinterpret_cast<uint4*>(gridw)[i] = make_uint4(grid_offset_word(gw.x, ns), grid_offset_word(gw.y, ns),
-                                                                grid_offset_word(gw.z, ns), grid_offset_word(gw.w, ns));
-            }
-        }
-        for (int i = tid; i <= G0.n_sph && i <= MPB_GRID_MAX_SPH; i += FUSED_THREADS)
-            otab[i] = (i < G0.n_sph) ? reinterpret_cast<const float4*>(G0.sph)[i] : make_float4(-1.0e9f, -1.0e9f, -1.0e9f, 0.f);
-        const f32x4 lv = reinterpret_cast<const f32x4*>(Lmat)[tid];
-        const f32x4 sv = reinterpret_cast<const f32x4*>(Sigma)[tid];
-        const int row = tid >> 4, col0 = (tid & 15) << 2;
-        const bool edge_row = row == 0 || row == H - 1;
-        stomp_l_image_store(Limg, row, col0, edge_row ? f32x4{0.f, 0.f, 0.f, 0.f} : lv);
-        *reinterpret_cast<f32x4*>(sig_l + row * FUSED_LD + col0) = sv;
-    }
+    if constexpr (IMG) asm volatile("s_waitcnt vmcnt(0)" ::: "memory");
+    else fused_stage_image(otab, gridw, Limg, sig_l, G0, Lmat, Sigma, tid);
     __syncthreads();
     const int ticket = __builtin_amdgcn_readfirstlane((int)s_ticket);
     const int p = exchange ? ticket / nc : ticket;
@@ -546,7 +539,48 @@
     }
 }
 
+template <int DCH, int MODEL, int NB, bool INJ, bool CHAIN>
+__global__ __launch_bounds__(FUSED_THREADS, 4) void stomp_fused_kernel(
+    float* __restrict__ means, const float* __restrict__ eps, float* __restrict__ samples, float* __restrict__ costs,
+    float* __restrict__ weights, const float* __restrict__ Lmat, const float* __restrict__ Sigma,
+    const float* __restrict__ geom, float* __restrict__ ws, int P, int S, int nc, float k_sigma, float weight, float lr,
+    float temperature, int n_iters, uint32_t seed_lo, uint32_t seed_hi, uint32_t iter0, uint32_t particle_offset,
+    uint32_t tag0, unsigned long long timeout_ticks, unsigned* __restrict__ status_host, float* __restrict__ means_copy) {
+    stomp_fused_body<DCH, MODEL, NB, INJ, CHAIN, false>(means, eps, samples, costs, weights, Lmat, Sigma, geom, ws, P, S, nc, k_sigma, weight, lr,
+                                                        temperature, n_iters, seed_lo, seed_hi, iter0, particle_offset, tag0, timeout_ticks,
+                                                        status_host, means_copy, nullptr);
+}
+
+template <int DCH, int MODEL>
+__global__ __launch_bounds__(FUSED_THREADS, 4) void stomp_fused_img_kernel(
+    float* __restrict__ means, float* __restrict__ samples, float* __restrict__ costs, float* __restrict__ weights,
+    const float* __restrict__ geom, float* __restrict__ ws, int P, int S, int nc, float k_sigma, float weight, float lr,
+    float temperature, int n_iters, uint32_t seed_lo, uint32_t seed_hi, uint32_t iter0, uint32_t particle_offset,
+    uint32_t tag0, unsigned long long timeout_ticks, unsigned* __restrict__ status_host, float* __restrict__ means_copy,
+    const FusedImage* __restrict__ image) {
+    static_assert(MODEL != 0, "built where the exchange prefetch is: the compile-time robot models");
+    stomp_fused_body<DCH, MODEL, 1, false, false, true>(means, nullptr, samples, costs, weights, nullptr, nullptr, geom, ws, P, S, nc, k_sigma,
+                                                        weight, lr, temperature, n_iters, seed_lo, seed_hi, iter0, particle_offset, tag0,
+                                                        timeout_ticks, status_host, means_copy, image);
+}
+
+__global__ __launch_bounds__(FUSED_THREADS) void stomp_image_build_kernel(FusedImage* __restrict__ image, const float* __restrict__ Lmat,
+                                                                          const float* __restrict__ Sigma, const float* __restrict__ geom) {
+    const GeomView G0 = geom_view(geom);
+    fused_stage_image(image->otab, image->gridw, image->Limg, image->sig_l, G0, Lmat, Sigma, (int)threadIdx.x);
+}
+
 size_t mpb_fused_ws_floats(int P, int nc) { return fused_ws_floats(P, nc); }
+
+bool mpb_fused_takes_image(const StompCall& c) {
+    return !c.eps && mpb_flags_model_on_grids(c.geom_flags, PandaModel::ID) && mpb_flags_one_field(c.geom_flags) && (c.d == 7 || c.d == 14);
+}
+size_t mpb_fused_image_bytes() { return sizeof(FusedImage); }
+int mpb_fused_image_build(const StompCall& c, void* image, hipStream_t stream) {
+    if (hipMemsetAsync(image, 0, sizeof(FusedImage), stream) != hipSuccess) return mpb_fail(MPB_E_HIP, "mpb_stomp_plan: memset of the image block failed");
+    hipLaunchKernelGGL(stomp_image_build_kernel, dim3(1), dim3(FUSED_THREADS), 0, stream, static_cast<FusedImage*>(image), c.L, c.Sigma, c.geom);
+    return mpb_check_launch("mpb_stomp_plan");
+}
 
 int mpb_fused_launch(const StompCall& c, const StompLaunch& l, const StompFusedGrid& g) {
     const bool two_batches = g.nb == 2;
@@ -559,6 +593,16 @@
                c.weights, c.L, c.Sigma, c.geom, g.workspace, c.P, c.S, nc_k, c.k_sigma, c.weight, c.lr, c.temperature, l.n_iters, lo,   \
                hi, l.iter0, c.particle_offset, g.tag0, g.timeout, g.status_dev, l.means_copy)
     const bool one_field = mpb_flags_one_field(c.geom_flags);
+    if (g.image && !two_batches && mpb_fused_takes_image(c)) {
+#define MPB_F_LAUNCH_IMG(DCH)                                                                                                            \
+    MPB_LAUNCH(l.events, (stomp_fused_img_kernel<DCH, PandaModel::ID>), grid, block, 0, l.stream, c.means, c.samples, c.costs, c.weights, \
+               c.geom, g.workspace, c.P, c.S, nc_k, c.k_sigma, c.weight, c.lr, c.temperature, l.n_iters, lo, hi, l.iter0,                \
+               c.particle_offset, g.tag0, g.timeout, g.status_dev, l.means_copy, static_cast<const FusedImage*>(g.image))
+        if (d == 7) MPB_F_LAUNCH_IMG(7);
+        else MPB_F_LAUNCH_IMG(14);
+#undef MPB_F_LAUNCH_IMG
+        return mpb_check_launch("mpb_stomp_run");
+    }
 #define MPB_F_LAUNCH(DCH, MODEL, NB, INJ)                                              \
     do {                                                                               \
         if ((MODEL) != 0 && one_field) MPB_F_LAUNCH_(DCH, MODEL, NB, INJ, (MODEL) == 0); \
diff --git a/motion_planning_baselines_amd/csrc/mpb_stomp_host.h b/motion_planning_baselines_amd/csrc/mpb_stomp_host.h
--- a/motion_planning_baselines_amd/csrc/mpb_stomp_host.h
+++ b/motion_planning_baselines_amd/csrc/mpb_stomp_host.h
@@ -41,11 +41,15 @@
     uint32_t tag0;
     unsigned long long timeout;
     unsigned* status_dev;
+    const void* image;
 };
 
 void mpb_stomp_launch_sample(const StompCall& c, const float* eps_it, uint32_t iter, hipStream_t st, const StompEvents* ev);
 bool mpb_stomp_launch_update(const StompCall& c, hipStream_t st, const StompEvents* ev);
 size_t mpb_fused_ws_floats(int P, int nc);
 int mpb_fused_launch(const StompCall& c, const StompLaunch& l, const StompFusedGrid& g);
+bool mpb_fused_takes_image(const StompCall& c);
+size_t mpb_fused_image_bytes();
+int mpb_fused_image_build(const StompCall& c, void* image, hipStream_t stream);
 bool mpb_fused_hx_plan(int geom_flags, int n_cu, int P, int S, int H, int d, int* nc_out, int* nb_out, size_t* ws_bytes);
 int mpb_fused_hx_launch(const StompCall& c, const StompLaunch& l, const StompFusedGrid& g);
diff --git a/motion_planning_baselines_amd/csrc/mpb_stomp_image.h b/motion_planning_baselines_amd/csrc/mpb_stomp_image.h
--- /dev/null
+++ b/motion_planning_baselines_amd/csrc/mpb_stomp_image.h
@@ -0,0 +1,43 @@
+#pragma once
+#include <hip/hip_runtime.h>
+
+#include "mpb_geom.h"
+#include "mpb_stomp_noise.h"
+#include "mpb_stomp_fused.h"
+
+struct FusedImage {
+    float4 otab[MPB_GRID_MAX_SPH + 1];
+    unsigned gridw[MPB_GRID_MAX_CELLS];
+    unsigned Limg[STOMP_LIMG_WORDS];
+    float sig_l[64 * FUSED_LD];
+};
+#define FUSED_IMAGE_KB 52
+static_assert(sizeof(FusedImage) == FUSED_IMAGE_KB * 1024, "the image block is a whole number of kilobytes");
+static_assert(__builtin_offsetof(FusedImage, otab) == 0 && __builtin_offsetof(FusedImage, gridw) == 1024 &&
+              __builtin_offsetof(FusedImage, Limg) == 1024 + 16384 && __builtin_offsetof(FusedImage, sig_l) == 1024 + 16384 + 18432,
+              "the image block's layout is the LDS layout of the kernel's constants");
+
+__device__ __forceinline__ void fused_stage_image(float4* otab, unsigned* gridw, unsigned* Limg, float* sig_l, const GeomView& G0,
+                                                  const float* __restrict__ Lmat, const float* __restrict__ Sigma, int tid) {
+    constexpr int H = 64;
+    const int g_rounds = (G0.n_cells + 4 * FUSED_THREADS - 1) / (4 * FUSED_THREADS);
+    const uint4* g4 = reinterpret_cast<const uint4*>(G0.grid);
+    const int n_pad16 = (G0.n_cells + MPB_GRID_PAD - 1) / MPB_GRID_PAD * (MPB_GRID_PAD / 4);
+    for (int u = 0; u < (MPB_GRID_MAX_CELLS / 4 + FUSED_THREADS - 1) / FUSED_THREADS; ++u) {
+        const int i = tid + FUSED_THREADS * u;
+        if (u < g_rounds && i < n_pad16) {
+            const uint4 gw = g4[i];
+            const unsigned ns = (unsigned)G0.n_sph;
+            reinterpret_cast<uint4*>(gridw)[i] = make_uint4(grid_offset_word(gw.x, ns), grid_offset_word(gw.y, ns),
+                                                            grid_offset_word(gw.z, ns), grid_offset_word(gw.w, ns));
+        }
+    }
+    for (int i = tid; i <= G0.n_sph && i <= MPB_GRID_MAX_SPH; i += FUSED_THREADS)
+        otab[i] = (i < G0.n_sph) ? reinterpret_cast<const float4*>(G0.sph)[i] : make_float4(-1.0e9f, -1.0e9f, -1.0e9f, 0.f);
+    const f32x4 lv = reinterpret_cast<const f32x4*>(Lmat)[tid];
+    const f32x4 sv = reinterpret_cast<const f32x4*>(Sigma)[tid];
+    const int row = tid >> 4, col0 = (tid & 15) << 2;
+    const bool edge_row = row == 0 || row == H - 1;
+    stomp_l_image_store(Limg, row, col0, edge_row ? f32x4{0.f, 0.f, 0.f, 0.f} : lv);
+    *reinterpret_cast<f32x4*>(sig_l + row * FUSED_LD + col0) = sv;
+}
diff --git a/motion_planning_baselines_amd/ops.py b/motion_planning_baselines_amd/ops.py
--- a/motion_planning_baselines_amd/ops.py
+++ b/motion_planning_baselines_amd/ops.py
@@ -588,7 +588,23 @@
     return 0 if status is None else status.note_launch()
 
 
+STOMP_IMAGE_BYTES = 53248
+
+
+def debug_stomp_image(L, Sigma, geom):
+    out = torch.empty(STOMP_IMAGE_BYTES, dtype=torch.uint8, device=L.device)
+    with torch.cuda.device(L.device):
+        _lib.debug_check(_lib.debug_lib().mpb_debug_stomp_image(_ptr(out), _ptr(L), _ptr(Sigma), _ptr(geom.buf), _stream()), 'mpb_debug_stomp_image')
+    return out
+
+
 class StompRunPlan:
+
+    @staticmethod
+    def make_key(means, samples, costs, weights, L, Sigma, geom, workspace, S, D, k_sigma, weight, lr, temperature, seed, particle_offset):
+        return (means.data_ptr(), samples.data_ptr(), costs.data_ptr(), weights.data_ptr(), L.data_ptr(),
+                Sigma.data_ptr(), geom.buf.data_ptr(), workspace.data_ptr(), S, D, float(k_sigma), float(weight),
+                float(lr), float(temperature), int(seed), int(particle_offset), L._version, Sigma._version, geom.buf._version)
 
     def __init__(self, means, samples, costs, weights, L, Sigma, geom, S, D, k_sigma, weight, lr, temperature, workspace,
                  seed, particle_offset, status):
@@ -599,9 +615,8 @@
             raise ValueError(f'StompRunPlan: tensors live on different devices ({devs})')
         self.device = means.device
         self.shape = (P, H, d)
-        self.key = (means.data_ptr(), samples.data_ptr(), costs.data_ptr(), weights.data_ptr(), L.data_ptr(),
-                    Sigma.data_ptr(), geom.buf.data_ptr(), workspace.data_ptr(), S, D, float(k_sigma), float(weight),
-                    float(lr), float(temperature), int(seed), int(particle_offset))
+        self.key = self.make_key(means, samples, costs, weights, L, Sigma, geom, workspace, S, D, k_sigma, weight, lr, temperature,
+                                 seed, particle_offset)
         self._call = (means, samples, costs, weights, L, Sigma, geom, S, D, k_sigma, weight, lr, temperature, workspace)
         self._seed, self._poff = _seed64(seed), int(particle_offset)
         self._status = status
@@ -621,14 +636,27 @@
             self._destroy(h)
             self._handle = None
 
+    def refresh(self):
+        with torch.cuda.device(self.device):
+            _lib.check(_lib.lib().mpb_stomp_plan_refresh(self._handle, raw_stream(self.device.index)), 'mpb_stomp_plan_refresh')
+        means, samples, costs, weights, L, Sigma, geom, S, D, k_sigma, weight, lr, temperature, workspace = self._call
+        self.key = self.make_key(means, samples, costs, weights, L, Sigma, geom, workspace, S, D, k_sigma, weight, lr, temperature,
+                                 self._seed, self._poff)
+
+    def image(self):
+        out = torch.empty(STOMP_IMAGE_BYTES, dtype=torch.uint8, device=self.device)
+        with torch.cuda.device(self.device):
+            _lib.check(_lib.lib().mpb_stomp_plan_image_copy(self._handle, out.data_ptr(), out.numel(), raw_stream(self.device.index)),
+                       'mpb_stomp_plan_image_copy')
+        return out
+
     def launch_timed(self, n_iters, iter0, means_copy=None):
         ms = ctypes.c_float(0.0)
-        rc = _lib.lib().mpb_stomp_run_timed(*_stomp_head(None, *self._call), int(n_iters), self._seed,
-                                            int(iter0), self._poff, self._status_ptr,
-                                            self._tag_ref, None if means_copy is None else means_copy.data_ptr(),
-                                            torch.cuda.current_stream(self.device).cuda_stream, ctypes.byref(ms))
+        rc = _lib.lib().mpb_stomp_plan_launch_timed(self._handle, int(n_iters), int(iter0),
+                                                    None if means_copy is None else means_copy.data_ptr(),
+                                                    torch.cuda.current_stream(self.device).cuda_stream, self._tag_ref, ctypes.byref(ms))
         if rc != 0:
-            _lib.check(rc, 'mpb_stomp_run_timed')
+            _lib.check(rc, 'mpb_stomp_plan_launch_timed')
         self._status.note_launch()
         return float(ms.value)
 
diff --git a/motion_planning_baselines_amd/planners/stomp.py b/motion_planning_baselines_amd/planners/stomp.py
--- a/motion_planning_baselines_amd/planners/stomp.py
+++ b/motion_planning_baselines_amd/planners/stomp.py
@@ -88,6 +88,7 @@
 
     def set_noise_dist(self):
         self.scale_tril = precision_to_scale_tril(self.Sigma_inv.detach().cpu().float()).to(self.device).contiguous()
+        self._plan = None
 
     def const_vel_trajectory(self, start_state, goal_state):
         H, D = self.n_support_points, self.n_dof
@@ -132,6 +133,7 @@
         else:
             m = self.get_random_trajs()
         self._particle_means = m.to(device=self.device, dtype=torch.float32).contiguous()
+        self._plan = None
         self.state_particles = self.sample()
 
     def optimize(self, opt_iters=None, **observation):
@@ -199,10 +201,9 @@
                     copy = torch.empty_like(m)
             if (self.persistent and self.noise == 'philox' and self._particle_means.is_cuda
                     and _current_device() == self._particle_means.device.index):
-                key = (self._particle_means.data_ptr(), self.state_particles.data_ptr(), self.costs.data_ptr(),
-                       self._weights_buf.data_ptr(), self.scale_tril.data_ptr(), self.Sigma.data_ptr(), geom.buf.data_ptr(),
-                       self._run_ws.data_ptr(), self.num_samples, self.n_dof, float(cc.k_sigma), float(weight), float(self.lr),
-                       float(self.temperature), self.seed, self.particle_offset)
+                key = ops.StompRunPlan.make_key(self._particle_means, self.state_particles, self.costs, self._weights_buf, self.scale_tril,
+                                                self.Sigma, geom, self._run_ws, self.num_samples, self.n_dof, cc.k_sigma, weight, self.lr,
+                                                self.temperature, self.seed, self.particle_offset)
                 plan = self._plan
                 if plan is None or plan.key != key:
                     plan = self._plan = ops.StompRunPlan(
```

Result: no change. 88530 (-1.0%).
